# Academich/translation-transformer

Hardware: AMD Instinct MI355X
Metric: reactions/sec (SMILES decoded), greedy speculative (higher is better)
Workload: dtype f32

## Files before the change

### include/ttx.h

```cpp
#ifndef TTX_H
#define TTX_H

#include <stdint.h>

#ifdef __cplusplus
extern "C" {
#endif

#define TTX_ABI_VERSION 4

typedef enum ttx_status {
  TTX_OK = 0,
  TTX_ERR_INVALID = -1,
  TTX_ERR_HIP = -2,
  TTX_ERR_NO_DEVICE = -3,
  TTX_ERR_REFERENCE = -4,
  TTX_ERR_NOMEM = -5,
  TTX_ERR_ROW_REPLAY = -6,
  TTX_ERR_MAX_STEPS = -7
} ttx_status;

typedef struct ttx_config {
  int32_t vocab_size;
  int32_t src_vocab_size;
// ... 83 lines not shown
typedef struct ttx_gen_stats {
  int64_t model_calls;
  int64_t accepted_tokens;
  int64_t produced_tokens;
  int64_t verified_positions;
  int64_t kv_prefix_positions;
  int64_t src_positions;
  double  encode_ms, decode_ms;
  int64_t src_tokens_padded;
  int64_t status;
} ttx_gen_stats;

int ttx_greedy_speculative_generate(ttx_session* s, const int64_t* d_src, int B, int Ls,
                                    const ttx_gen_params* p, int64_t* d_out, ttx_gen_stats* stats,
                                    void* stream);

int ttx_greedy_generate(ttx_session* s, const int64_t* d_src, int B, int Ls, const ttx_gen_params* p,
                        int64_t* d_out, ttx_gen_stats* stats, void* stream);

int ttx_nucleus_mask(ttx_session* s, const float* d_logits, int rows, int V, float nucleus, int n_best, float fill,
                     float* d_out, void* stream);
int ttx_accepted_lengths(ttx_session* s, const float* d_logits, const int64_t* d_drafts, int R, int D, int V, float nucleus,
                         int n_best, int32_t* d_n_ok, void* stream);
int ttx_ragged_topk(ttx_session* s, const float* d_score, const int32_t* d_offsets, int G, int max_group, int k,
                    float* d_top, int64_t* d_idx, void* stream);
typedef struct ttx_beam_params {
  int32_t max_len;
  int32_t n_best;
  int32_t draft_len;
  int32_t n_drafts;
  int32_t smart_drafts_mode;
  int32_t pad_token, bos_token, eos_token, replace_token;
  int32_t max_steps;
} ttx_beam_params;

typedef struct ttx_beam_stats {
  int64_t model_calls;
  int64_t input_lines;
  int64_t running_rows;
  int64_t accepted_tokens;
  int64_t produced_non_pad_tokens;
  int64_t verified_positions;
  int64_t executed_positions;
  int64_t kv_prefix_positions;
  int64_t running_candidates;
  int64_t src_tokens_padded;
  double  encode_ms, decode_ms;
  int32_t out_width;
  int32_t status;
} ttx_beam_stats;

int ttx_beam_speculative_generate(ttx_session* s, const int64_t* d_src, int B, int Ls, const ttx_beam_params* p,
                                  int64_t* d_out, ttx_beam_stats* stats, void* stream);
int ttx_beam_speculative_generate_many(ttx_session** sessions, int n_sessions, int n_batches, const int64_t* const* d_src,
                                       const int* B, const int* Ls, const ttx_beam_params* p, int64_t* const* d_out,
                                       ttx_beam_stats* stats, void* stream);

int ttx_beam_speculative_generate_pool(ttx_session** sessions, int n_sessions, const int64_t* d_src, int R_total, int Ls_all,
                                       const int32_t* h_len, const int32_t* h_batch_of, int n_batches, const int32_t* h_given_ls,
                                       int capacity, const ttx_beam_params* p, int64_t* d_out, int16_t* d_trace_len,
                                       int32_t* d_summary, int trace_cap, ttx_beam_stats* stats, void* stream);

typedef struct ttx_beam_search_params {
  int32_t max_len, beam_size;
  int32_t pad_token, bos_token, eos_token;
} ttx_beam_search_params;
typedef struct ttx_beam_search_stats {
  int64_t model_calls;
  int64_t running_rows;
  int32_t out_width;
  int32_t pad_;
} ttx_beam_search_stats;
int ttx_beam_generate(ttx_session* s, const int64_t* d_src, int B, int Ls, const ttx_beam_search_params* p, int64_t* d_out,
                      ttx_beam_search_stats* stats, void* stream);

int ttx_greedy_speculative_generate_many(ttx_session** sessions, int n_sessions, int n_batches,
                                         const int64_t* const* d_src, const int* B, const int* Ls,
                                         const ttx_gen_params* p, int64_t* const* d_out, ttx_gen_stats* stats,
                                         void* stream);

int ttx_greedy_speculative_generate_rows(ttx_session** sessions, int n_sessions, int n_batches,
                                         const int64_t* const* d_src, const int* B, const int* Ls,
                                         const ttx_gen_params* p, int64_t* const* d_out, int16_t* const* d_traj,
                                         int32_t* const* d_fin_step, ttx_gen_stats* stats, void* stream);

int ttx_greedy_speculative_generate_pool(ttx_session** sessions, int n_sessions, const int64_t* d_src, int R_total, int Ls_all,
                                         const int32_t* h_len, int capacity, const ttx_gen_params* p, int64_t* d_out,
                                         int16_t* d_traj, int32_t* d_fin_step, ttx_gen_stats* stats, void* stream);

typedef struct ttx_tokenizer ttx_tokenizer;
int  ttx_tokenizer_create(const char* const* tokens, const int32_t* ids, int n, ttx_tokenizer** out);
void ttx_tokenizer_destroy(ttx_tokenizer* t);
int  ttx_tokenizer_encode(const ttx_tokenizer* t, const char* line, int32_t* out, int cap);
int  ttx_tokenizer_encode_batch(const ttx_tokenizer* t, const char* const* lines, int B, int64_t* out, int cap_cols);
int  ttx_tokenizer_decode(const ttx_tokenizer* t, const int64_t* ids, int n, char* out, int cap);

int ttx_debug_step_snapshot(ttx_session* s, int32_t* info, float* h_logits, int32_t* h_act, int32_t* h_front,
                            int32_t* h_gen);

int ttx_last_kernel_profile(ttx_session* s, double* gemm_ms, int64_t* gemm_launches, double* empty_pair_ms);

int ttx_debug_gemm_bench(ttx_session* s, int M, int N, int K, int splits, int variant, int reps, double* us_per_launch,
                         double* max_abs_diff);

int ttx_debug_gemm(ttx_session* s, const float* d_x, int ldx, const float* d_w, int ldw, const float* d_bias, float* d_y, int ldy,
                   const int32_t* d_m, int m_max, int N, int K, int relu, int splits, int64_t slab_stride, int variant, int tiling,
                   int32_t* kernel_id, void* stream);
int ttx_debug_gemm_act(ttx_session* s, const float* d_x, int ldx, const float* d_w, int ldw, const float* d_bias, float* d_y, int ldy,
                       const int32_t* d_m, int m_max, int N, int K, int activation, int splits, int64_t slab_stride, int variant,
                       int tiling, int32_t* kernel_id, void* stream);

int ttx_debug_finish_ln(ttx_session* s, const float* d_slabs, int n_slabs, int64_t slab_stride, const float* d_bias,
                        const float* d_resid, const float* d_g1, const float* d_b1, const float* d_g2, const float* d_b2,
                        const uint8_t* d_row_valid, float* d_y, const int32_t* d_m, int m_max, int d, float eps, void* stream);

int ttx_debug_attn(ttx_session* s, const float* d_q, int ldq, const float* d_k, const float* d_v, int ldkv, float* d_out, int H,
                   float scale, int L, int Lk, const int32_t* d_tok, int pad, const uint8_t* d_key_pad, const int32_t* d_mem_row,
                   const int32_t* d_act_idx, const int32_t* d_front, const int32_t* d_src_of, const int32_t* d_src_len,
                   const float* d_kcache, const float* d_vcache, int64_t cache_seq_stride, const int32_t* d_cache_slot, int gen_ld,
                   int N, int D, int mode, int groups, int n_active, int max_keys, int kernel, int32_t* kernel_id, void* stream);

int ttx_debug_attn_hd(ttx_session* s, const float* d_q, int ldq, const float* d_k, const float* d_v, int ldkv, float* d_out, int H,
                      int head_dim, float scale, int L, int Lk, const int32_t* d_tok, int pad, const uint8_t* d_key_pad,
                      const int32_t* d_mem_row, const int32_t* d_act_idx, const int32_t* d_front, const int32_t* d_src_of,
                      const int32_t* d_src_len, const float* d_kcache, const float* d_vcache, int64_t cache_seq_stride,
                      const int32_t* d_cache_slot, int gen_ld, int N, int D, int mode, int groups, int n_active, int max_keys,
                      int kernel, int32_t* kernel_id, void* stream);

int ttx_debug_attn_as(ttx_session* s, const float* d_q, int ldq, const float* d_k, const float* d_v, int ldkv, float* d_out, int H,
                      int head_dim, float scale, int L, int Lk, const int32_t* d_tok, int pad, const uint8_t* d_key_pad,
                      const int32_t* d_mem_row, const int32_t* d_act_idx, const int32_t* d_front, const int32_t* d_src_of,
                      const int32_t* d_src_len, const float* d_kcache, const float* d_vcache, int64_t cache_seq_stride,
                      const int32_t* d_cache_slot, int gen_ld, int N, int D, int mode, int groups, int n_active, int max_keys,
                      int kernel, int32_t* kernel_id, int sel_N, int sel_D, void* stream);

int ttx_debug_argmax(ttx_session* s, const float* d_logits, int V, int32_t* d_pred, const int32_t* d_m, int m_max, void* stream);

int ttx_debug_embed(ttx_session* s, const float* d_table, int V, const float* d_pe, int pe_rows, int d, float* d_x,
                    const int32_t* d_tok, int rows, int L, const int32_t* d_act_idx, const int32_t* d_front, const int32_t* d_gen,
                    int gen_ld, const int32_t* d_drafts, int B, int N, int D, int n_active, int step, void* stream);

typedef struct ttx_debug_accept_args {
  int32_t* d_act_idx; int32_t* d_front; int32_t* d_gen; const int32_t* d_drafts; const int32_t* d_pred; int32_t* d_rec;
  int64_t* d_out; int32_t* d_haspad;
  int16_t* d_traj; int32_t* d_fin_step;
  int32_t* d_rstep; int32_t* d_row_of; int64_t* d_pool_out; int16_t* d_pool_traj; int32_t* d_pool_fin_step;
  int32_t gen_ld, traj_ld, pool_rows, row_rule, pool;
  int32_t B, N, D, Ls, max_len, pad, bos, eos;
  int32_t greedy;
  int32_t threads;
} ttx_debug_accept_args;

int ttx_debug_accept(ttx_session* s, const ttx_debug_accept_args* a, int64_t* state, void* stream);

int ttx_debug_kvcopy(ttx_session* s, const int32_t* d_rec, int n_copy, const float* d_qkv, int64_t qkv_layer_stride, float* d_kcache,
                     float* d_vcache, int64_t cache_layer_stride, int64_t cache_seq_stride, int N, int D, int d, int B, int Ld,
                     void* stream);

int ttx_debug_kvcopy_split(ttx_session* s, const int32_t* d_rec, int n_copy, const float* d_qkv, int64_t qkv_layer_stride,
                           float* d_kcache, float* d_vcache, int64_t cache_layer_stride, int64_t cache_seq_stride, int N, int D, int d,
                           int B, int Ld, const int32_t* d_pos2, const float* d_qkv_probe, int64_t probe_layer_stride, void* stream);

int ttx_debug_probe_split(ttx_session* s, const int32_t* d_act_idx, const int32_t* d_pred_probe, const int32_t* d_drafts, int B, int N,
                          int D, int n_active, int32_t* d_act2, int32_t* d_pos2, int32_t* result, void* stream);

int ttx_debug_merge_pred(ttx_session* s, const int32_t* d_pos2, const int32_t* d_pred_probe, const int32_t* d_pred2, int32_t* d_pred,
                         int B, int N, int D, int n_active, void* stream);

int ttx_debug_probe_split_select(ttx_session* s, const int32_t* d_act_idx, const int32_t* d_pred_probe, const int32_t* d_drafts, int B,
                                 int N, int D, int n_active, int32_t* d_act2, int32_t* d_pos2, int32_t* d_draft_mask, int32_t* d_row_base,
                                 int32_t* d_row_map, int32_t* result, void* stream);
int ttx_debug_merge_pred_select(ttx_session* s, const int32_t* d_pos2, const int32_t* d_pred_probe, const int32_t* d_pred2,
                                int32_t* d_pred, int B, int N, int D, int n_active, const int32_t* d_row_base,
                                const int32_t* d_draft_mask, void* stream);
int ttx_debug_kvcopy_select(ttx_session* s, const int32_t* d_rec, int n_copy, const float* d_qkv, int64_t qkv_layer_stride,
                            float* d_kcache, float* d_vcache, int64_t cache_layer_stride, int64_t cache_seq_stride, int N, int D, int d,
                            int B, int Ld, const int32_t* d_pos2, const float* d_qkv_probe, int64_t probe_layer_stride,
                            const int32_t* d_row_base, const int32_t* d_draft_mask, void* stream);
int ttx_debug_embed_select(ttx_session* s, const float* d_table, int V, const float* d_pe, int pe_rows, int d, float* d_x,
                           const int32_t* d_act_idx, const int32_t* d_front, const int32_t* d_gen, int gen_ld, const int32_t* d_drafts,
                           int B, int N, int D, int n_active, const int32_t* d_row_map, int m_rows, void* stream);
int ttx_debug_attn_select(ttx_session* s, const float* d_q, int ldq, const float* d_k, const float* d_v, int ldkv, float* d_out, int H,
                          float scale, int Lk, const int32_t* d_tok, int pad, const uint8_t* d_key_pad, const int32_t* d_act_idx,
                          const int32_t* d_front, const int32_t* d_src_of, const int32_t* d_src_len, const float* d_kcache,
                          const float* d_vcache, int64_t cache_seq_stride, const int32_t* d_cache_slot, int gen_ld, int N, int D, int mode,
                          int groups, int n_active, int max_keys, int kernel, int32_t* kernel_id, const int32_t* d_row_base,
                          const int32_t* d_draft_mask, void* stream);

int ttx_pool_last_counters(ttx_session* s, int64_t* counters);

int ttx_attn_staged_key_limit(int head_dim, int q_per_group);

int ttx_debug_attn_kernels_seen(ttx_session* s);

int ttx_debug_attn_probs(ttx_session* s, const float* d_q, int ldq, const float* d_k, int ldkv, const uint8_t* d_key_pad,
                         const int32_t* d_mem_row, const int32_t* d_length, int R, int Rm, int H, int head_dim, int T, int Ls,
                         float scale, float* d_heads, float* d_mean, int32_t* d_align, void* stream);

#ifdef __cplusplus
}
#endif
#endif
```

### translation-transformer_amd/_native.py

```python
from __future__ import annotations

import ctypes as C
import os
import subprocess
from pathlib import Path

PKG_DIR = Path(__file__).resolve().parent
CSRC = PKG_DIR / "csrc"
INCLUDE = PKG_DIR.parent / "include"
LIB_PATH = PKG_DIR / "libttx_hip.so"
UNITS = [CSRC / "ttx_api.hip", CSRC / "ttx_gemm.hip", CSRC / "ttx_attn.hip"]
HEADERS = [CSRC / "ttx_internal.h", CSRC / "ttx_common.hip.h", CSRC / "ttx_loop_kernels.hip.h", CSRC / "ttx_metrics.hip.h",
           CSRC / "ttx_score.hip.h", CSRC / "ttx_alternatives.hip.h", CSRC / "ttx_attn_probs.hip.h", CSRC / "ttx_select.h",
           CSRC / "ttx_tokenizer.h", INCLUDE / "ttx.h"]
SOURCES = UNITS + HEADERS
OBJ_DIR = CSRC / "build"

TTX_OK, TTX_ERR_INVALID, TTX_ERR_HIP, TTX_ERR_NO_DEVICE, TTX_ERR_REFERENCE, TTX_ERR_NOMEM = 0, -1, -2, -3, -4, -5
TTX_ERR_ROW_REPLAY = -6
TTX_ERR_MAX_STEPS = -7
TTX_ACT_NONE, TTX_ACT_RELU, TTX_ACT_GELU = 0, 1, 2
ACTIVATIONS = {"relu": TTX_ACT_RELU, "gelu": TTX_ACT_GELU}


def activation_code(activation: str) -> int:
    if activation not in ACTIVATIONS:
        raise ValueError(f"activation must be 'relu' or 'gelu' (the exact erf GELU), got {activation!r}")
    return ACTIVATIONS[activation]


class TtxError(RuntimeError):
    def __init__(self, code: int, msg: str):
        super().__init__(f"libttx_hip error {code}: {msg}")
        self.code = code


class ReferenceError_(RuntimeError):
    """Raised where the reference implementation itself raises on the same input."""


class Config(C.Structure):
    _fields_ = [("vocab_size", C.c_int32), ("src_vocab_size", C.c_int32), ("embedding_dim", C.c_int32),
                ("num_heads", C.c_int32), ("feedforward_dim", C.c_int32), ("num_encoder_layers", C.c_int32),
                ("num_decoder_layers", C.c_int32), ("pad_token", C.c_int32), ("max_positions", C.c_int32),
                ("layer_norm_eps", C.c_float)]


class Tensor(C.Structure):
    _fields_ = [("name", C.c_char_p), ("data", C.POINTER(C.c_float)), ("numel", C.c_int64)]


class GenParams(C.Structure):
    _fields_ = [("max_len", C.c_int32), ("draft_len", C.c_int32), ("n_drafts", C.c_int32), ("pad_token", C.c_int32),
                ("bos_token", C.c_int32), ("eos_token", C.c_int32), ("replace_token", C.c_int32),
                ("want_logits", C.c_int32)]


class BeamParams(C.Structure):
    _fields_ = [("max_len", C.c_int32), ("n_best", C.c_int32), ("draft_len", C.c_int32), ("n_drafts", C.c_int32),
                ("smart_drafts_mode", C.c_int32), ("pad_token", C.c_int32), ("bos_token", C.c_int32),
                ("eos_token", C.c_int32), ("replace_token", C.c_int32), ("max_steps", C.c_int32)]


class BeamStats(C.Structure):
    _fields_ = [("model_calls", C.c_int64), ("input_lines", C.c_int64), ("running_rows", C.c_int64),
                ("accepted_tokens", C.c_int64), ("produced_non_pad_tokens", C.c_int64), ("verified_positions", C.c_int64),
                ("executed_positions", C.c_int64), ("kv_prefix_positions", C.c_int64), ("running_candidates", C.c_int64),
                ("src_tokens_padded", C.c_int64), ("encode_ms", C.c_double), ("decode_ms", C.c_double),
                ("out_width", C.c_int32), ("status", C.c_int32)]


class BeamSearchParams(C.Structure):
    _fields_ = [("max_len", C.c_int32), ("beam_size", C.c_int32), ("pad_token", C.c_int32), ("bos_token", C.c_int32),
                ("eos_token", C.c_int32)]


class BeamSearchStats(C.Structure):
    _fields_ = [("model_calls", C.c_int64), ("running_rows", C.c_int64), ("out_width", C.c_int32), ("pad_", C.c_int32)]


class GenStats(C.Structure):
    _fields_ = [("model_calls", C.c_int64), ("accepted_tokens", C.c_int64), ("produced_tokens", C.c_int64),
                ("verified_positions", C.c_int64), ("kv_prefix_positions", C.c_int64), ("src_positions", C.c_int64),
                ("encode_ms", C.c_double), ("decode_ms", C.c_double), ("src_tokens_padded", C.c_int64),
                ("status", C.c_int64)]


class DebugAcceptArgs(C.Structure):
    _fields_ = [(n, C.c_void_p) for n in ("d_act_idx", "d_front", "d_gen", "d_drafts", "d_pred", "d_rec", "d_out", "d_haspad",
                                          "d_traj", "d_fin_step", "d_rstep", "d_row_of", "d_pool_out", "d_pool_traj",
                                          "d_pool_fin_step")] + \
               [(n, C.c_int32) for n in ("gen_ld", "traj_ld", "pool_rows", "row_rule", "pool", "B", "N", "D", "Ls", "max_len",
                                         "pad", "bos", "eos", "greedy", "threads")]


DEBUG_ACCEPT_STATE_WORDS = 17


_VP, _I, _I64P = C.c_void_p, C.c_int, C.c_void_p
SYMBOLS = {
    "ttx_abi_version": (C.c_int, []),
    "ttx_last_error": (C.c_char_p, []),
    "ttx_device_count": (C.c_int, []),
    "ttx_model_create": (C.c_int, [C.POINTER(Config), C.POINTER(Tensor), _I, _I, C.POINTER(_VP)]),
    "ttx_model_destroy": (None, [_VP]),
    "ttx_model_create_empty": (C.c_int, [C.POINTER(Config), _I, C.POINTER(_VP)]),
    "ttx_model_blob": (C.c_int, [_VP, C.POINTER(_VP), C.POINTER(C.c_int64)]),
    "ttx_model_set_activation": (C.c_int, [_VP, _I]),
    "ttx_model_activation": (C.c_int, [_VP]),
    "ttx_session_create": (C.c_int, [_VP, C.POINTER(_VP)]),
    "ttx_session_destroy": (None, [_VP]),
    "ttx_encode_src": (C.c_int, [_VP, _VP, _I, _I, _VP, _VP]),
    "ttx_decode_tgt": (C.c_int, [_VP, _VP, _I, _I, _VP, _VP, _VP, _I, _I, _VP, _VP]),
    "ttx_forward": (C.c_int, [_VP, _VP, _I, _I, _VP, _I, _VP, _VP]),
    "ttx_token_metrics": (C.c_int, [_VP, _VP, _VP, _I, _I, _I, _I, _VP, _VP, _VP, _VP]),
    "ttx_teacher_forced_eval": (C.c_int, [_VP, _VP, _I, _I, _VP, _I, _I, _VP, _VP, _VP, _VP, _VP]),
    "ttx_hypothesis_logprobs": (C.c_int, [_VP, _VP, _VP, _I, _I, _I, _I, _I, _VP, _VP, _VP, _VP, _VP]),
    "ttx_score_hypotheses": (C.c_int, [_VP, _VP, _I, _I, _VP, _I, _I, _I, _I, _VP, _VP, _VP, _VP, _VP, _VP]),
    "ttx_hypothesis_alternatives": (C.c_int, [_VP, _VP, _VP, _I, _I, _I, _I, _I, _I, _VP, _VP, _VP, _VP, _VP, _VP, _VP]),
    "ttx_score_alternatives": (C.c_int, [_VP, _VP, _I, _I, _VP, _I, _I, _I, _I, _I, _VP, _VP, _VP, _VP, _VP, _VP, _VP, _VP]),
    "ttx_attention_maps": (C.c_int, [_VP, _VP, _I, _I, _VP, _I, _I, _I, _I, _I, _VP, _VP, _VP, _VP, _VP]),
    "ttx_attn_probs_key_limit": (C.c_int, [_I]),
    "ttx_debug_attn_probs": (C.c_int, [_VP, _VP, _I, _VP, _I, _VP, _VP, _VP, _I, _I, _I, _I, _I, _I, C.c_float, _VP, _VP, _VP, _VP]),
    "ttx_make_drafts": (C.c_int, [_VP, _VP, _I, _I, _I, _I, _I, _I, _I, _I, _I, _VP, _VP]),
    "ttx_greedy_speculative_generate": (C.c_int, [_VP, _VP, _I, _I, C.POINTER(GenParams), _VP, C.POINTER(GenStats), _VP]),
    "ttx_greedy_generate": (C.c_int, [_VP, _VP, _I, _I, C.POINTER(GenParams), _VP, C.POINTER(GenStats), _VP]),
    "ttx_greedy_speculative_generate_many": (C.c_int, [C.POINTER(_VP), _I, _I, C.POINTER(_VP), C.POINTER(C.c_int),
                                                      C.POINTER(C.c_int), C.POINTER(GenParams), C.POINTER(_VP),
                                                      C.POINTER(GenStats), _VP]),
    "ttx_greedy_speculative_generate_rows": (C.c_int, [C.POINTER(_VP), _I, _I, C.POINTER(_VP), C.POINTER(C.c_int),
                                                      C.POINTER(C.c_int), C.POINTER(GenParams), C.POINTER(_VP),
                                                      C.POINTER(_VP), C.POINTER(_VP), C.POINTER(GenStats), _VP]),
    "ttx_greedy_speculative_generate_pool": (C.c_int, [C.POINTER(_VP), _I, _VP, _I, _I, C.POINTER(C.c_int32), _I,
                                                      C.POINTER(GenParams), _VP, _VP, _VP, C.POINTER(GenStats), _VP]),
    "ttx_beam_speculative_generate": (C.c_int, [_VP, _VP, _I, _I, C.POINTER(BeamParams), _VP, C.POINTER(BeamStats), _VP]),
    "ttx_beam_speculative_generate_many": (C.c_int, [C.POINTER(_VP), _I, _I, C.POINTER(_VP), C.POINTER(C.c_int),
                                                    C.POINTER(C.c_int), C.POINTER(BeamParams), C.POINTER(_VP),
                                                    C.POINTER(BeamStats), _VP]),
    "ttx_beam_speculative_generate_pool": (C.c_int, [C.POINTER(_VP), _I, _VP, _I, _I, C.POINTER(C.c_int32), C.POINTER(C.c_int32), _I,
                                                    C.POINTER(C.c_int32), _I, C.POINTER(BeamParams), _VP, _VP, _VP, _I,
                                                    C.POINTER(BeamStats), _VP]),
    "ttx_beam_generate": (C.c_int, [_VP, _VP, _I, _I, C.POINTER(BeamSearchParams), _VP, C.POINTER(BeamSearchStats), _VP]),
    "ttx_nucleus_mask": (C.c_int, [_VP, _VP, _I, _I, C.c_float, _I, C.c_float, _VP, _VP]),
    "ttx_accepted_lengths": (C.c_int, [_VP, _VP, _VP, _I, _I, _I, C.c_float, _I, _VP, _VP]),
    "ttx_ragged_topk": (C.c_int, [_VP, _VP, _VP, _I, _I, _I, _VP, _VP, _VP]),
    "ttx_tokenizer_create": (C.c_int, [C.POINTER(C.c_char_p), C.POINTER(C.c_int32), _I, C.POINTER(_VP)]),
    "ttx_tokenizer_destroy": (None, [_VP]),
    "ttx_tokenizer_encode": (C.c_int, [_VP, C.c_char_p, _VP, _I]),
    "ttx_tokenizer_encode_batch": (C.c_int, [_VP, C.POINTER(C.c_char_p), _I, _VP, _I]),
    "ttx_tokenizer_decode": (C.c_int, [_VP, _VP, _I, _VP, _I]),
    "ttx_debug_step_snapshot": (C.c_int, [_VP, C.POINTER(C.c_int32), _VP, _VP, _VP, _VP]),
    "ttx_debug_gemm_bench": (C.c_int, [_VP, _I, _I, _I, _I, _I, _I, C.POINTER(C.c_double), C.POINTER(C.c_double)]),
    "ttx_debug_gemm": (C.c_int, [_VP, _VP, _I, _VP, _I, _VP, _VP, _I, _VP, _I, _I, _I, _I, _I, C.c_int64, _I, _I,
                                 C.POINTER(C.c_int32), _VP]),
    "ttx_debug_gemm_act": (C.c_int, [_VP, _VP, _I, _VP, _I, _VP, _VP, _I, _VP, _I, _I, _I, _I, _I, C.c_int64, _I, _I,
                                     C.POINTER(C.c_int32), _VP]),
    "ttx_debug_finish_ln": (C.c_int, [_VP, _VP, _I, C.c_int64, _VP, _VP, _VP, _VP, _VP, _VP, _VP, _VP, _VP, _I, _I, C.c_float, _VP]),
    "ttx_debug_attn": (C.c_int, [_VP, _VP, _I, _VP, _VP, _I, _VP, _I, C.c_float, _I, _I, _VP, _I, _VP, _VP, _VP, _VP, _VP, _VP, _VP, _VP,
                                 C.c_int64, _VP, _I, _I, _I, _I, _I, _I, _I, _I, C.POINTER(C.c_int32), _VP]),
    "ttx_debug_attn_hd": (C.c_int, [_VP, _VP, _I, _VP, _VP, _I, _VP, _I, _I, C.c_float, _I, _I, _VP, _I, _VP, _VP, _VP, _VP, _VP, _VP, _VP,
                                    _VP, C.c_int64, _VP, _I, _I, _I, _I, _I, _I, _I, _I, C.POINTER(C.c_int32), _VP]),
    "ttx_debug_attn_as": (C.c_int, [_VP, _VP, _I, _VP, _VP, _I, _VP, _I, _I, C.c_float, _I, _I, _VP, _I, _VP, _VP, _VP, _VP, _VP, _VP, _VP,
                                    _VP, C.c_int64, _VP, _I, _I, _I, _I, _I, _I, _I, _I, C.POINTER(C.c_int32), _I, _I, _VP]),
    "ttx_debug_argmax": (C.c_int, [_VP, _VP, _I, _VP, _VP, _I, _VP]),
    "ttx_debug_embed": (C.c_int, [_VP, _VP, _I, _VP, _I, _I, _VP, _VP, _I, _I, _VP, _VP, _VP, _I, _VP, _I, _I, _I, _I, _I, _VP]),
    "ttx_debug_accept": (C.c_int, [_VP, C.POINTER(DebugAcceptArgs), C.POINTER(C.c_int64), _VP]),
    "ttx_debug_kvcopy": (C.c_int, [_VP, _VP, _I, _VP, C.c_int64, _VP, _VP, C.c_int64, C.c_int64, _I, _I, _I, _I, _I, _VP]),
    "ttx_debug_kvcopy_split": (C.c_int, [_VP, _VP, _I, _VP, C.c_int64, _VP, _VP, C.c_int64, C.c_int64, _I, _I, _I, _I, _I, _VP, _VP,
                                         C.c_int64, _VP]),
    "ttx_debug_probe_split": (C.c_int, [_VP, _VP, _VP, _VP, _I, _I, _I, _I, _VP, _VP, C.POINTER(C.c_int32), _VP]),
    "ttx_debug_merge_pred": (C.c_int, [_VP, _VP, _VP, _VP, _VP, _I, _I, _I, _I, _VP]),
    "ttx_debug_probe_split_select": (C.c_int, [_VP, _VP, _VP, _VP, _I, _I, _I, _I, _VP, _VP, _VP, _VP, _VP, C.POINTER(C.c_int32), _VP]),
    "ttx_debug_merge_pred_select": (C.c_int, [_VP, _VP, _VP, _VP, _VP, _I, _I, _I, _I, _VP, _VP, _VP]),
    "ttx_debug_kvcopy_select": (C.c_int, [_VP, _VP, _I, _VP, C.c_int64, _VP, _VP, C.c_int64, C.c_int64, _I, _I, _I, _I, _I, _VP, _VP,
                                          C.c_int64, _VP, _VP, _VP]),
    "ttx_debug_embed_select": (C.c_int, [_VP, _VP, _I, _VP, _I, _I, _VP, _VP, _VP, _VP, _I, _VP, _I, _I, _I, _I, _VP, _I, _VP]),
    "ttx_debug_attn_select": (C.c_int, [_VP, _VP, _I, _VP, _VP, _I, _VP, _I, C.c_float, _I, _VP, _I, _VP, _VP, _VP, _VP, _VP, _VP, _VP,
                                        C.c_int64, _VP, _I, _I, _I, _I, _I, _I, _I, _I, C.POINTER(C.c_int32), _VP, _VP, _VP]),
    "ttx_pool_last_counters": (C.c_int, [_VP, C.POINTER(C.c_int64)]),
    "ttx_attn_staged_key_limit": (C.c_int, [_I, _I]),
    "ttx_debug_attn_kernels_seen": (C.c_int, [_VP]),
    "ttx_last_kernel_profile": (C.c_int, [_VP, C.POINTER(C.c_double), C.POINTER(C.c_int64), C.POINTER(C.c_double)]),
}

_lib = None


def hipcc_path() -> str:
    for cand in (os.environ.get("HIPCC"), "/opt/rocm/bin/hipcc", "hipcc"):
        if cand and (os.path.isabs(cand) and os.path.exists(cand) or not os.path.isabs(cand)):
            return cand
    return "hipcc"


def needs_build() -> bool:
    if not LIB_PATH.exists():
        return True
    t = LIB_PATH.stat().st_mtime
    return any(src.stat().st_mtime > t for src in SOURCES)


def build(force: bool = False, verbose: bool = False) -> Path:
    if not force and not needs_build():
        return LIB_PATH
    OBJ_DIR.mkdir(exist_ok=True)
    flags = ["--offload-arch=gfx950", "-O3", "-std=c++17", "-fPIC", f"-I{INCLUDE}"] + os.environ.get("TTX_HIPCC_FLAGS", "").split()
    newest_header = max(h.stat().st_mtime for h in HEADERS)
    jobs, objs = [], []
    for unit in UNITS:
        obj = OBJ_DIR / (unit.stem + ".o")
        objs.append(str(obj))
        if not force and obj.exists() and obj.stat().st_mtime > max(unit.stat().st_mtime, newest_header) \
                and not os.environ.get("TTX_HIPCC_FLAGS"):
            continue
        cmd = [hipcc_path(), *flags, "-c", str(unit), "-o", str(obj)]
        if verbose:
            print(" ".join(cmd))
        jobs.append((cmd, subprocess.Popen(cmd)))
    for cmd, proc in jobs:
        if proc.wait() != 0:
            raise subprocess.CalledProcessError(proc.returncode, cmd)
    cmd = [hipcc_path(), "--offload-arch=gfx950", "-shared", "-fPIC", "-o", str(LIB_PATH), *objs]
    if verbose:
        print(" ".join(cmd))
    subprocess.run(cmd, check=True)
    return LIB_PATH


def lib():
    global _lib
    if _lib is not None:
        return _lib
    if needs_build():
        build()
    handle = C.CDLL(str(LIB_PATH))
    for name, (res, args) in SYMBOLS.items():
        fn = getattr(handle, name)
        fn.restype = res
        fn.argtypes = args
    if handle.ttx_abi_version() != 4:
        raise RuntimeError("libttx_hip.so ABI version mismatch")
    _lib = handle
    return _lib


def check(code: int) -> None:
    if code == TTX_OK:
        return
    msg = lib().ttx_last_error().decode("utf-8", "replace")
    if code == TTX_ERR_REFERENCE:
        raise ReferenceError_(msg)
    if code == TTX_ERR_MAX_STEPS:
        raise RuntimeError("beam-speculative loop exceeded max_steps (non-terminating input)")
    raise TtxError(code, msg)
```

### translation-transformer_amd/csrc/ttx_api.hip

```cpp
#include "ttx_internal.h"
#include "ttx_loop_kernels.hip.h"
#include "ttx_metrics.hip.h"
#include "ttx_score.hip.h"
#include "ttx_alternatives.hip.h"
#include "ttx_attn_probs.hip.h"
#include "ttx_tokenizer.h"

#include <algorithm>
#include <chrono>
#include <cmath>
#include <cstdio>
#include <cstdlib>
#include <cstring>
#include <mutex>
#include <type_traits>

using namespace ttx;

static thread_local std::string g_err;

int ttx::fail(int code, const std::string& msg) {
  g_err = msg;
  return code;
}
// ... 131 lines not shown
  *bytes = (int64_t)(m->blob_floats * sizeof(float));
  return TTX_OK;
}

extern "C" int ttx_model_create(const ttx_config* cfg, const ttx_tensor* tensors, int n_tensors, int device,
                                ttx_model** out) {
  if (!tensors || n_tensors <= 0) return fail(TTX_ERR_INVALID, "no tensors given");
  ttx_model* m = nullptr;
  TTX_TRY(model_alloc(cfg, device, &m));
  std::vector<float> host(m->blob_floats, 0.f);
  std::map<std::string, const ttx_tensor*> given;
  for (int i = 0; i < n_tensors; ++i) {
    if (!tensors[i].name || !tensors[i].data) { ttx_model_destroy(m); return fail(TTX_ERR_INVALID, "tensor with null name/data"); }
    std::string nm = tensors[i].name;
    if (nm.rfind("model.", 0) == 0) nm = nm.substr(6);
    given[nm] = &tensors[i];
  }
  for (auto& kv : m->index) {
    const std::string& nm = kv.first;
    const bool derived = nm.rfind("derived.", 0) == 0;
    auto it = given.find(nm);
    if (it == given.end()) {
      if (derived || nm == "positional_encoding.pe") continue;
      ttx_model_destroy(m);
      return fail(TTX_ERR_INVALID, "missing tensor: " + nm);
    }
    if ((size_t)it->second->numel != kv.second.second) {
      ttx_model_destroy(m);
      return fail(TTX_ERR_INVALID, "tensor " + nm + " has " + std::to_string(it->second->numel) + " elements, expected " +
                                       std::to_string(kv.second.second));
    }
    std::memcpy(host.data() + kv.second.first, it->second->data, kv.second.second * sizeof(float));
  }
  const ttx_config& c = m->cfg;
  const size_t d = c.embedding_dim;
  if (given.find("positional_encoding.pe") == given.end()) {
    float* pe = host.data() + m->pe;
    const float cst = (float)(-std::log(10000.0) / (double)d);
    for (int p = 0; p < c.max_positions; ++p)
      for (size_t i = 0; i < d; i += 2) {
        const float div = expf((float)i * cst);
        const float arg = (float)p * div;
        pe[(size_t)(p + 1) * d + i] = sinf(arg);
        pe[(size_t)(p + 1) * d + i + 1] = cosf(arg);
      }
  }
  for (int l = 0; l < c.num_decoder_layers; ++l) {
    std::memcpy(host.data() + m->cross_kv_w + (size_t)l * 2 * d * d, host.data() + m->dec[l].ca_in_w + d * d, 2 * d * d * sizeof(float));
    std::memcpy(host.data() + m->cross_kv_b + (size_t)l * 2 * d, host.data() + m->dec[l].ca_in_b + d, 2 * d * sizeof(float));
  }
  if (hipMemcpy(m->blob, host.data(), host.size() * sizeof(float), hipMemcpyHostToDevice) != hipSuccess) {
    ttx_model_destroy(m);
    return fail(TTX_ERR_HIP, "hipMemcpy of the weight blob failed");
  }
  *out = m;
  return TTX_OK;
}

extern "C" void ttx_model_destroy(ttx_model* m) {
  if (!m) return;
  if (m->blob) (void)hipFree(m->blob);
  delete m;
}

static std::mutex g_retired_mu;
static std::vector<void*> g_retired;

static void release_retired() {
  std::vector<void*> v;
  {
    std::lock_guard<std::mutex> lk(g_retired_mu);
    v.swap(g_retired);
  }
  if (v.empty()) return;
  (void)hipDeviceSynchronize();
  for (void* p : v) (void)hipFree(p);
}

static std::mutex g_stream_mu;
static std::map<int, std::vector<std::pair<int, hipStream_t>>> g_free_streams;
static std::map<hipStream_t, int> g_stream_index;
static int g_streams_made = 0;

static int ensure_own_stream(ttx_session* s) {
  if (s->own_stream) return TTX_OK;
  std::lock_guard<std::mutex> lock(g_stream_mu);
  auto& idle = g_free_streams[s->m->device];
  if (!idle.empty()) {
    auto it = std::min_element(idle.begin(), idle.end());
    s->own_stream = it->second;
    idle.erase(it);
    return TTX_OK;
  }
  HIP_TRY(hipStreamCreateWithFlags(&s->own_stream, hipStreamNonBlocking));
  g_stream_index[s->own_stream] = g_streams_made++;
  return TTX_OK;
}

static void release_own_stream(ttx_session* s) {
  if (!s->own_stream) return;
  std::lock_guard<std::mutex> lock(g_stream_mu);
  g_free_streams[s->m->device].push_back({g_stream_index[s->own_stream], s->own_stream});
  s->own_stream = nullptr;
}

static int ensure(Buf& b, size_t bytes, hipStream_t st) {
  (void)st;
  if (bytes <= b.cap) return TTX_OK;
  if (b.owner_gen) ++*b.owner_gen;
  if (b.p) {
    std::lock_guard<std::mutex> lk(g_retired_mu);
    g_retired.push_back(b.p);
    b.p = nullptr;
    b.cap = 0;
  }
  size_t want = bytes + bytes / 8 + 256;
  if (hipMalloc(&b.p, want) != hipSuccess) return fail(TTX_ERR_NOMEM, "hipMalloc failed for " + std::to_string(want) + " bytes");
  b.cap = want;
  static const bool poison = getenv("TTX_POISON_WORKSPACES") != nullptr && atoi(getenv("TTX_POISON_WORKSPACES")) != 0;
  if (poison) {
    if (hipMemset(b.p, 0xFF, want) != hipSuccess) return fail(TTX_ERR_HIP, "hipMemset (poison) failed");
    (void)hipDeviceSynchronize();
  }
  return TTX_OK;
}

extern "C" int ttx_session_create(ttx_model* m, ttx_session** out) {
  if (!m || !out) return fail(TTX_ERR_INVALID, "null argument");
  HIP_TRY(hipSetDevice(m->device));
  ttx_session* s = new ttx_session();
  s->m = m;
  if (hipHostMalloc((void**)&s->host_info, sizeof(HostInfo), hipHostMallocMapped) != hipSuccess ||
      hipHostMalloc((void**)&s->probe_info, sizeof(ProbeInfo), hipHostMallocMapped) != hipSuccess ||
      hipHostMalloc((void**)&s->host_state, sizeof(DecState), hipHostMallocDefault) != hipSuccess) {
    if (s->host_info) (void)hipHostFree(s->host_info);
    if (s->probe_info) (void)hipHostFree(s->probe_info);
    if (s->host_state) (void)hipHostFree(s->host_state);
    delete s;
    return fail(TTX_ERR_NOMEM, "hipHostMalloc failed");
  }
  std::memset(s->host_info, 0, sizeof(HostInfo));
  std::memset(s->probe_info, 0, sizeof(ProbeInfo));
  HIP_TRY(hipEventCreate(&s->ev_a));
  HIP_TRY(hipEventCreate(&s->ev_b));
  HIP_TRY(hipEventCreate(&s->ev_c));
  HIP_TRY(hipEventCreateWithFlags(&s->ev_done, hipEventDisableTiming));
  s->use_graphs = getenv("TTX_NO_GRAPH") == nullptr;
  const char* pf = getenv("TTX_PROFILE_GEMM");
  s->profile = pf && pf[0] == '1';
  if (const char* e = getenv("TTX_SMALL_ROWS")) s->small_rows = std::max(0, atoi(e));
  if (const char* e = getenv("TTX_FFN2_SLAB_ROWS")) s->ffn2_slab_rows = std::max(0, atoi(e));
  if (const char* e = getenv("TTX_QKV_SMALL_ROWS")) s->qkv_small_rows = std::max(0, atoi(e));
  if (const char* e = getenv("TTX_ATTN_FALLBACK")) s->attn_fallback = atoi(e) != 0;
  if (const char* e = getenv("TTX_ATTN_ROW")) s->attn_row = atoi(e) != 0 ? 1 : 0;
  s->host_timing = getenv("TTX_HOST_TIMING") != nullptr;
  m->n_sessions++;
  *out = s;
  return TTX_OK;
}

extern "C" void ttx_session_destroy(ttx_session* s) {
  if (!s) return;
  if (s->host_timing && s->host_launches)
    fprintf(stderr, "[ttx host timing] hipGraphLaunch: %lld launches, %.1f us each\n", s->host_launches,
            s->host_launch_us / (double)s->host_launches);
  if (s->host_timing && s->host_captures)
    fprintf(stderr, "[ttx host timing] graphs captured: %lld, %.1f us each\n", s->host_captures,
            s->host_capture_us / (double)s->host_captures);
  if (s->dead) {
    delete s;
    return;
  }
  release_retired();
  (void)hipDeviceSynchronize();
  for (Buf* b : s->all)
    if (b->p) (void)hipFree(b->p);
  if (s->host_info) (void)hipHostFree(s->host_info);
  if (s->probe_info) (void)hipHostFree(s->probe_info);
  if (s->beam_host) (void)hipHostFree(s->beam_host);
  if (s->bp_host) (void)hipHostFree(s->bp_host);
  s->drop_graphs();
  release_own_stream(s);
  if (s->ev_done) (void)hipEventDestroy(s->ev_done);
  if (s->host_state) (void)hipHostFree(s->host_state);
  for (auto& e : s->ev_pool) { (void)hipEventDestroy(e.first); (void)hipEventDestroy(e.second); }
  if (s->ev_a) (void)hipEventDestroy(s->ev_a);
  if (s->ev_b) (void)hipEventDestroy(s->ev_b);
  if (s->ev_c) (void)hipEventDestroy(s->ev_c);
  delete s;
}

static int variant_for_rows(const ttx_session* s, long long rows, bool step) {
  if (!step) return GV_BIG;
  if (rows < s->qkv_small_rows) return GV_SMALL;
  if (rows < s->small_rows) return GV_MID;
  return rows < s->ffn2_slab_rows ? GV_BIG_FFN2_SLABS : GV_BIG;
}
static int variant_qkv(int v) { return v == GV_SMALL ? GV_SMALL : GV_BIG; }
static int variant_dd(int v) { return (v == GV_SMALL || v == GV_MID) ? GV_SMALL : GV_BIG; }
static int variant_ffn1(int v) { return v == GV_SMALL ? GV_SMALL : GV_BIG; }
static int variant_ffn2(int v) { return v == GV_BIG ? GV_BIG : GV_SMALL; }

static int gemm_ln(ttx_session* s, hipStream_t st, const float* X, int ldx, int K, const float* W, const float* bias,
                   const float* resid, const float* g1, const float* b1, const float* g2, const float* b2,
                   const uint8_t* row_valid, float* Y, const int* m_ptr, int Mmax, int variant) {
  const int d = s->m->cfg.embedding_dim;
  const int S = gemm_splits(d, K, m_ptr != nullptr, variant);
  const long long stride = (long long)Mmax * d;
  TTX_TRY(ensure(s->slab, sizeof(float) * (size_t)S * stride, st));
  TTX_TRY(launch_gemm(s, st, X, ldx, W, K, nullptr, s->slab.as<float>(), d, m_ptr, Mmax, d, K, false, S, stride, variant));
  return launch_finish(s, st, s->slab.as<float>(), S, stride, bias, resid, g1, b1, g2, b2, row_valid, Y, m_ptr, Mmax);
}

static int ffn_half(ttx_session* s, hipStream_t st, const LayerW& w, const float* x, size_t n_w, size_t n_b, const float* g2,
                    const float* b2, const uint8_t* row_valid, float* Y, const int* m_ptr, int Mmax, int v_ffn1, int v_ffn2) {
  const ttx_model* m = s->m;
  const int d = m->cfg.embedding_dim, F = m->cfg.feedforward_dim;
  float* hb = s->hbuf.as<float>();
  TTX_TRY(launch_gemm(s, st, x, d, m->p(w.l1_w), d, m->p(w.l1_b), hb, F, m_ptr, Mmax, F, d, m->activation, 0, 0, v_ffn1));
  return gemm_ln(s, st, hb, F, F, m->p(w.l2_w), m->p(w.l2_b), x, m->p(n_w), m->p(n_b), g2, b2, row_valid, Y, m_ptr, Mmax, v_ffn2);
}

static int ensure_acts(ttx_session* s, hipStream_t st, size_t M, int qkv_layers) {
  const ttx_config& c = s->m->cfg;
  const size_t d = c.embedding_dim, F = c.feedforward_dim;
  TTX_TRY(ensure(s->x, M * d * 4, st));
  TTX_TRY(ensure(s->x1, M * d * 4, st));
  TTX_TRY(ensure(s->x2, M * d * 4, st));
  TTX_TRY(ensure(s->xf, M * d * 4, st));
  TTX_TRY(ensure(s->ao, M * d * 4, st));
  TTX_TRY(ensure(s->q2, M * d * 4, st));
  TTX_TRY(ensure(s->hbuf, M * F * 4, st));
  TTX_TRY(ensure(s->qkv, (size_t)qkv_layers * M * 3 * d * 4, st));
  return TTX_OK;
}

static int run_encoder(ttx_session* s, hipStream_t st, const int* tok, const uint8_t* valid, int B, int Ls, float* memory,
                       float* qkv_buf = nullptr) {
  const ttx_model* m = s->m;
  const ttx_config& c = m->cfg;
  const int d = c.embedding_dim, H = c.num_heads;
  const int M = B * Ls;
  const int gv = variant_for_rows(s, M, false);
  TTX_TRY(ensure_acts(s, st, (size_t)M, 1));
  float* x = s->x.as<float>();
  float* x1 = s->x1.as<float>();
  float* qkv = qkv_buf ? qkv_buf : s->qkv.as<float>();
  float* ao = s->ao.as<float>();
  EmbedArgs e{};
  e.table = m->p(m->src_emb); e.pe = m->p(m->pe); e.X = x; e.d = d; e.V = c.src_vocab_size; e.tok = tok; e.rows = M; e.L = Ls;
  hipLaunchKernelGGL((k_embed<false>), dim3(cdiv(M, 4)), dim3(256), 0, st, e);
  HIP_TRY(hipGetLastError());
  for (int l = 0; l < c.num_encoder_layers; ++l) {
    const LayerW& w = m->enc[l];
    const bool last = (l == c.num_encoder_layers - 1);
    TTX_TRY(launch_gemm(s, st, x, d, m->p(w.sa_in_w), d, m->p(w.sa_in_b), qkv, 3 * d, nullptr, M, 3 * d, d, false, 0, 0, gv));
    AttnArgs a{};
    a.q = qkv; a.ldq = 3 * d; a.k = qkv + d; a.v = qkv + 2 * d; a.ldkv = 3 * d; a.out = ao; a.d = d;
    a.scale = 1.0f / sqrtf((float)(d / H)); a.L = Ls; a.tok = tok; a.pad = c.pad_token;
    TTX_TRY(launch_attn(ATT_ENC, s, st, a, B, H, Ls, Ls));
    TTX_TRY(gemm_ln(s, st, ao, d, d, m->p(w.sa_out_w), m->p(w.sa_out_b), x, m->p(w.n1_w), m->p(w.n1_b), nullptr, nullptr,
                    nullptr, x1, nullptr, M, gv));
    TTX_TRY(ffn_half(s, st, w, x1, w.n2_w, w.n2_b, last ? m->p(m->enc_norm_w) : nullptr, last ? m->p(m->enc_norm_b) : nullptr,
                     last ? valid : nullptr, last ? memory : x, nullptr, M, gv, gv));
  }
  return TTX_OK;
}

static int prepare_tokens(hipStream_t st, const int64_t* d_in, int* out, uint8_t* valid, int n, int pad) {
  hipLaunchKernelGGL(k_prepare_tokens, dim3(cdiv(n, 256)), dim3(256), 0, st, d_in, out, valid, n, pad);
  HIP_TRY(hipGetLastError());
  return TTX_OK;
}

extern "C" int ttx_encode_src(ttx_session* s, const int64_t* d_src, int B, int Ls, float* d_memory, void* stream) {
  if (!s || !d_src || !d_memory || B <= 0 || Ls <= 0) return fail(TTX_ERR_INVALID, "bad argument to ttx_encode_src");
  if (Ls > s->m->cfg.max_positions) return fail(TTX_ERR_INVALID, "source longer than the positional table");
  hipStream_t st = (hipStream_t)stream;
  HIP_TRY(hipSetDevice(s->m->device));
  TTX_TRY(ensure(s->tok_src, (size_t)B * Ls * 4, st));
  TTX_TRY(ensure(s->src_valid, (size_t)B * Ls, st));
  TTX_TRY(prepare_tokens(st, d_src, s->tok_src.as<int>(), s->src_valid.as<uint8_t>(), B * Ls, s->m->cfg.pad_token));
  return run_encoder(s, st, s->tok_src.as<int>(), s->src_valid.as<uint8_t>(), B, Ls, d_memory);
}

struct StackRows {
  const int* m_ptr;
  int Mmax;
  int v_qkv, v_dd, v_ffn1, v_ffn2;
  float* qkv;
  long long qkv_layer;
};

template <class SelfAttn, class CrossAttn>
static int run_decoder_stack(ttx_session* s, hipStream_t st, const StackRows& r, SelfAttn&& self_attn, CrossAttn&& cross_attn,
                             float* logits, int stop_layer = -1) {
  const ttx_model* m = s->m;
  const ttx_config& c = m->cfg;
  const int d = c.embedding_dim, V = c.vocab_size, Ld = c.num_decoder_layers;
  float* x = s->x.as<float>();
  float* x1 = s->x1.as<float>();
  float* x2 = s->x2.as<float>();
  float* xf = s->xf.as<float>();
  float* ao = s->ao.as<float>();
  float* q2 = s->q2.as<float>();
  for (int l = 0; l < Ld; ++l) {
// ... 385 lines not shown
                                  void* stream) {
  if (!s) return session_required("ttx_attention_maps");
  if (!d_src || !d_hyp || B <= 0 || N <= 0 || Ls <= 0) return fail(TTX_ERR_INVALID, "bad argument to ttx_attention_maps");
  if (!d_heads && !d_mean && !d_align) return fail(TTX_ERR_INVALID, "ttx_attention_maps: no output requested (heads, mean and alignment are all null)");
  if (ld_hyp < W) return fail(TTX_ERR_INVALID, "ttx_attention_maps: row stride ld_hyp smaller than W");
  const ttx_config& c = s->m->cfg;
  if (layer == -1) layer = c.num_decoder_layers - 1;
  if (layer < 0 || layer >= c.num_decoder_layers)
    return fail(TTX_ERR_INVALID, "ttx_attention_maps: layer must be -1 or in [0, " + std::to_string(c.num_decoder_layers) + ")");
  TTX_TRY(check_score_shapes(s, (long long)B * N, W, 1, "ttx_attention_maps"));
  if (Ls > c.max_positions) return fail(TTX_ERR_INVALID, "source longer than the positional table");
  const int limit = attn_probs_key_limit(c.embedding_dim / c.num_heads);
  if (Ls > limit)
    return fail(TTX_ERR_INVALID, "ttx_attention_maps: source longer than " + std::to_string(limit) + " keys (ttx_attn_probs_key_limit)");
  hipStream_t st = (hipStream_t)stream;
  HIP_TRY(hipSetDevice(s->m->device));
  const int R = B * N, T = W - 1, d = c.embedding_dim;
  if (!d_length) {
    TTX_TRY(ensure(s->am_length, (size_t)R * 4, st));
    d_length = s->am_length.as<int32_t>();
  }
  TTX_TRY(ensure(s->memory, (size_t)B * Ls * d * 4, st));
  TTX_TRY(ensure(s->mem_pad_tmp, (size_t)B * Ls, st));
  TTX_TRY(ensure(s->sc_src_of, (size_t)R * 4, st));
  TTX_TRY(ttx_encode_src(s, d_src, B, Ls, s->memory.as<float>(), stream));
  hipLaunchKernelGGL(k_invert_mask, dim3(cdiv(B * Ls, 256)), dim3(256), 0, st, s->src_valid.as<uint8_t>(),
                     s->mem_pad_tmp.as<uint8_t>(), B * Ls);
  HIP_TRY(hipGetLastError());
  hipLaunchKernelGGL(k_score_src_of, dim3(cdiv(R, 256)), dim3(256), 0, st, s->sc_src_of.as<int>(), R, N);
  HIP_TRY(hipGetLastError());
  TTX_TRY(ensure(s->tok_tgt, (size_t)R * T * 4, st));
  hipLaunchKernelGGL(k_prepare_tokens_2d, dim3(cdiv(R * T, 256)), dim3(256), 0, st, d_hyp, ld_hyp, s->tok_tgt.as<int>(),
                     (uint8_t*)nullptr, R, T, c.pad_token);
  HIP_TRY(hipGetLastError());
  hipLaunchKernelGGL(k_hyp_length, dim3(cdiv(R, 4)), dim3(256), 0, st, d_hyp, ld_hyp, R, W, c.pad_token, eos, d_length);
  HIP_TRY(hipGetLastError());
  const AttnTap tap{layer, d_length, d_heads, d_mean, d_align};
  return run_decoder_full(s, st, s->tok_tgt.as<int>(), R, T, s->memory.as<float>(), s->mem_pad_tmp.as<uint8_t>(),
                          s->sc_src_of.as<int>(), B, Ls, nullptr, &tap);
}

static int clamp_draft_len(int draft_len, int lo, int hi) { return std::min(std::max(lo, draft_len), hi); }

template <typename OutT>
static int launch_make_drafts(hipStream_t st, const int* src32, int src_ld, int off, int B, int L, int N, int D, int eos,
                              int pad, int repl, OutT* out) {
  const int need = N + D - 1;
  const int Lp = L > need ? L : need;
  const size_t lds = sizeof(int) * (size_t)(Lp + 1);
  if (lds > 60 * 1024) return fail(TTX_ERR_INVALID, "make_drafts: padded source row too long");
  hipLaunchKernelGGL((k_make_drafts<OutT>), dim3(B), dim3(64), lds, st, src32, src_ld, off, L, N, D, eos, pad, repl, out);
  HIP_TRY(hipGetLastError());
  return TTX_OK;
}

extern "C" int ttx_make_drafts(ttx_session* s, const int64_t* d_src, int B, int L, int draft_len, int n_drafts,
                               int min_draft_len, int max_draft_len, int eos_token, int pad_token, int replace_token,
                               int64_t* d_drafts, void* stream) {
  if (!s || !d_src || !d_drafts || B <= 0 || L <= 0) return fail(TTX_ERR_INVALID, "bad argument to ttx_make_drafts");
  if (n_drafts <= 0) return fail(TTX_ERR_REFERENCE, "The number of drafts must be greater than 0");
  if (min_draft_len > max_draft_len) return fail(TTX_ERR_REFERENCE, "The minimum draft length must not be greater than the maximum draft length");
  if (pad_token == replace_token || eos_token == replace_token || eos_token == pad_token)
    return fail(TTX_ERR_REFERENCE, "pad, eos and replace tokens must be pairwise different");
  hipStream_t st = (hipStream_t)stream;
  HIP_TRY(hipSetDevice(s->m->device));
  const int D = clamp_draft_len(draft_len, min_draft_len, max_draft_len);
  if (D <= 0) return fail(TTX_ERR_INVALID, "draft length must be positive");
  TTX_TRY(ensure(s->src32, (size_t)B * L * 4, st));
  TTX_TRY(prepare_tokens(st, d_src, s->src32.as<int>(), nullptr, B * L, pad_token));
  return launch_make_drafts<int64_t>(st, s->src32.as<int>(), L, 0, B, L, n_drafts, D, eos_token, pad_token, replace_token, d_drafts);
}

struct StepCtx {
  int B, Ls, N, D, Lc, gen_ld, max_len;
  ttx_gen_params p;
  const float* kcache = nullptr;
  const float* vcache = nullptr;
  const int* src_of = nullptr;
  const int* src_len = nullptr;
  const int* cache_slot = nullptr;
  bool want_argmax = true;
  int variant = GV_BIG;
  DecState* st_ov = nullptr;
  const int* act_ov = nullptr;
  float* qkv_ov = nullptr;
  int* pred_ov = nullptr;
  int sel_N = 0, sel_D = 0;
  const int* row_base = nullptr; const int* draft_mask = nullptr; const int* row_map = nullptr;
};

static int run_step(ttx_session* s, hipStream_t st, const StepCtx& k, int kcap) {
  const ttx_model* m = s->m;
  const ttx_config& c = m->cfg;
  const int d = c.embedding_dim, H = c.num_heads, V = c.vocab_size, Ld = c.num_decoder_layers;
  const int D1 = k.D + 1;
  const int RPS = step_rps(k.N, k.D);
  const int Mmax = k.B * RPS;
  DecState* dst = k.st_ov ? k.st_ov : s->state.as<DecState>();
  const int* act = k.act_ov ? k.act_ov : s->act_idx.as<int>();
  const int* m_ptr = &dst->m_rows;
  float* ao = s->ao.as<float>();
  float* logits = s->logits.as<float>();
  const float scale = 1.0f / sqrtf((float)(d / H));
  const long long cache_seq = (long long)k.Lc * d;
  const long long cache_layer = (long long)k.B * cache_seq;

  struct AttnSel {
    ttx_session* s;
    AttnSel(ttx_session* s_, int N, int D) : s(s_) { s->attn_sel_N = N; s->attn_sel_D = D; }
    ~AttnSel() { s->attn_sel_N = 0; s->attn_sel_D = 0; }
  } attn_sel(s, k.sel_N, k.sel_D);
  EmbedArgs e{};
  e.table = m->p(m->tgt_emb); e.pe = m->p(m->pe); e.X = s->x.as<float>(); e.d = d; e.V = c.vocab_size;
  e.st = dst; e.act_idx = act; e.front = s->front.as<int>(); e.gen = s->gen.as<int>(); e.gen_ld = k.gen_ld;
  e.drafts = s->drafts.as<int>(); e.N = k.N; e.D = k.D; e.row_map = k.row_map;
  hipLaunchKernelGGL((k_embed<true>), dim3(cdiv(Mmax, 4)), dim3(256), 0, st, e);
  HIP_TRY(hipGetLastError());

  const StackRows rows{m_ptr, Mmax, variant_qkv(k.variant), variant_dd(k.variant), variant_ffn1(k.variant), variant_ffn2(k.variant),
                       k.qkv_ov ? k.qkv_ov : s->qkv.as<float>(), (long long)Mmax * 3 * d};
  TTX_TRY(run_decoder_stack(s, st, rows,
      [&](int l, float* qkv) -> int {
        AttnArgs a{};
        a.q = qkv; a.ldq = 3 * d; a.k = qkv + d; a.v = qkv + 2 * d; a.ldkv = 3 * d; a.out = ao; a.d = d; a.scale = scale;
        a.tok = s->gen.as<int>(); a.pad = c.pad_token; a.st = dst; a.act_idx = act; a.front = s->front.as<int>();
        a.kcache = (k.kcache ? k.kcache : s->kcache.as<float>()) + (size_t)l * cache_layer;
        a.vcache = (k.vcache ? k.vcache : s->vcache.as<float>()) + (size_t)l * cache_layer;
        a.cache_seq_stride = cache_seq; a.gen_ld = k.gen_ld; a.N = k.N; a.D = k.D; a.cache_slot = k.cache_slot;
        a.row_base = k.row_base; a.draft_mask = k.draft_mask;
        return launch_attn(ATT_STEP_SELF, s, st, a, k.B, H, RPS, kcap, k.N, D1);
      },
      [&](int l) -> int {
        AttnArgs ca{};
        ca.q = s->q2.as<float>(); ca.ldq = d; ca.k = s->memkv.as<float>() + (size_t)l * 2 * d; ca.v = ca.k + d; ca.ldkv = Ld * 2 * d;
        ca.out = ao; ca.d = d; ca.scale = scale; ca.Lk = k.Ls; ca.key_pad = s->src_valid.as<uint8_t>();
        ca.st = dst; ca.act_idx = act; ca.front = s->front.as<int>(); ca.N = k.N; ca.D = k.D;
        ca.src_of = k.src_of; ca.src_len = k.src_len; ca.row_base = k.row_base; ca.draft_mask = k.draft_mask;
        return launch_attn(ATT_STEP_CROSS, s, st, ca, k.B, H, RPS, k.Ls, k.N, D1);
      },
      logits));
  if (k.want_argmax) {
    hipLaunchKernelGGL(k_argmax, dim3(cdiv(Mmax, 4)), dim3(256), 0, st, logits, V, k.pred_ov ? k.pred_ov : s->pred.as<int>(), m_ptr, Mmax);
    HIP_TRY(hipGetLastError());
  }
  return TTX_OK;
}

struct GenCtx {
  StepCtx k;
  LoopArgs la;
  KvCopyArgs kc;
};

static int launch_accept_and_commit(ttx_session* s, hipStream_t st, const GenCtx& g, bool greedy) {
  if (greedy) hipLaunchKernelGGL(k_greedy_accept, dim3(1), dim3(256), 0, st, g.la);
  else hipLaunchKernelGGL(k_accept, dim3(1), dim3(g.k.B > 256 ? ACCEPT_THREADS : 256), 0, st, g.la);
  HIP_TRY(hipGetLastError());
  hipLaunchKernelGGL(k_kvcopy, dim3(g.k.B, s->m->cfg.num_decoder_layers), dim3(256), 0, st, g.kc);
  HIP_TRY(hipGetLastError());
  return TTX_OK;
}

static bool watchdog_expired(std::chrono::steady_clock::time_point since) {
  static const int limit_s = [] { const char* e = getenv("TTX_WATCHDOG_SECONDS"); return e && atoi(e) > 0 ? atoi(e) : 120; }();
  return std::chrono::steady_clock::now() - since > std::chrono::seconds(limit_s);
}

static int session_hung(ttx_session* s) {
  s->dead = true;
  return fail(TTX_ERR_HIP, "verify step did not publish its result within the watchdog time; the session is unusable "
                           "(its stream was NOT synchronised) - exit the process or continue in a fresh child process");
}

static int session_alive(const ttx_session* s) {
  if (s && s->dead) return fail(TTX_ERR_HIP, "this session hung in an earlier call and is unusable");
  return TTX_OK;
}

struct Progress {
  unsigned idle_spins = 0;
  std::chrono::steady_clock::time_point last_progress = std::chrono::steady_clock::now();
  bool stalled() { return (++idle_spins & 0xffff) == 0 && watchdog_expired(last_progress); }
  void advanced() { idle_spins = 0; last_progress = std::chrono::steady_clock::now(); }
};

static int key_capacity(int width, int max_len) { return std::min(max_len, ((width + 63) / 64) * 64); }

template <class Enqueue>
static int graph_replay(ttx_session* s, hipStream_t st, GraphCache& cache, const GraphKey& key, Enqueue&& enqueue) {
  if (!s->use_graphs || s->profile) return enqueue();
  const auto now = [s] { return s->host_timing ? std::chrono::steady_clock::now() : std::chrono::steady_clock::time_point(); };
  const auto us_since = [&](std::chrono::steady_clock::time_point t0) { return std::chrono::duration<double, std::micro>(now() - t0).count(); };
  s->graphs_current();
  auto it = cache.map.find(key);
  if (it == cache.map.end()) {
    if (cache.warmed.insert(key).second) return enqueue();
    hipGraph_t graph = nullptr;
    hipGraphExec_t exec = nullptr;
    const auto t0 = now();
    HIP_TRY(hipStreamBeginCapture(st, hipStreamCaptureModeThreadLocal));
    const int rc = enqueue();
    hipError_t e = hipStreamEndCapture(st, &graph);
    if (rc != TTX_OK) { if (graph) (void)hipGraphDestroy(graph); return rc; }
    if (e != hipSuccess) return fail(TTX_ERR_HIP, std::string("hipStreamEndCapture: ") + hipGetErrorString(e));
    e = hipGraphInstantiate(&exec, graph, nullptr, nullptr, 0);
    (void)hipGraphDestroy(graph);
    if (e != hipSuccess) return fail(TTX_ERR_HIP, std::string("hipGraphInstantiate: ") + hipGetErrorString(e));
    if (cache.map.size() > cache.limit) s->drop_graphs();
    it = cache.map.emplace(key, exec).first;
    if (s->host_timing) { s->host_captures += 1; s->host_capture_us += us_since(t0); }
  }
  const auto t0 = now();
  HIP_TRY(hipGraphLaunch(it->second, st));
  if (s->host_timing) { s->host_launches += 1; s->host_launch_us += us_since(t0); }
  return TTX_OK;
}

struct EventGuard {
  hipEvent_t e = nullptr;
  ~EventGuard() { if (e) (void)hipEventDestroy(e); }
};

struct GenJob {
  ttx_session* s = nullptr;
  hipStream_t st = nullptr;
  GenCtx g{};
  bool greedy = false;
  int64_t* d_out = nullptr;
  int16_t* d_traj = nullptr;
  int32_t* d_fin = nullptr;
  ttx_gen_stats* stats = nullptr;
  int launched = 0;
  int phase = 0;
  int batch = -1;
  Progress progress;
};

static int gen_validate(const ttx_session* s, const int64_t* d_src, int B, int Ls, const ttx_gen_params* p, const int64_t* d_out,
                        bool greedy) {
  if (!s || !d_src || !p || !d_out || B <= 0 || Ls <= 1) return fail(TTX_ERR_INVALID, "bad argument to a generate call");
  const ttx_config& c = s->m->cfg;
  if (!greedy) {
    if (p->n_drafts <= 0) return fail(TTX_ERR_REFERENCE, "The number of drafts must be greater than 0");
    if (p->max_len < 1) return fail(TTX_ERR_REFERENCE, "The minimum draft length must not be greater than the maximum draft length");
    if (p->pad_token == p->replace_token || p->eos_token == p->replace_token || p->eos_token == p->pad_token)
      return fail(TTX_ERR_REFERENCE, "pad, eos and replace tokens must be pairwise different");
    if (p->draft_len <= 0) return fail(TTX_ERR_REFERENCE, "Number of speculative tokens must be a positive integer.");
    if (p->draft_len > p->max_len) return fail(TTX_ERR_REFERENCE, "draft_len beyond max_len: the reference's scatter shapes disagree");
  } else if (p->max_len < 1) {
    return fail(TTX_ERR_INVALID, "max_len must be positive");
  }
  if (p->pad_token != c.pad_token) return fail(TTX_ERR_INVALID, "generator pad token differs from the model's");
  const int D = greedy ? 0 : p->draft_len;
  if (p->max_len + D + 2 > c.max_positions) return fail(TTX_ERR_INVALID, "max_len + draft_len exceeds the positional table");
  return TTX_OK;
}

static int gen_start(GenJob& j, ttx_session* s, hipStream_t st, const int64_t* d_src, int B, int Ls, const ttx_gen_params* p,
                     int64_t* d_out, ttx_gen_stats* stats, bool greedy, int16_t* d_traj = nullptr, int32_t* d_fin = nullptr) {
  const ttx_model* m = s->m;
  const ttx_config& c = m->cfg;
  const int d = c.embedding_dim, Ld = c.num_decoder_layers, V = c.vocab_size;
  const int N = greedy ? 1 : p->n_drafts, D = greedy ? 0 : p->draft_len, D1 = D + 1;
  const int max_len = p->max_len;
  j.s = s; j.st = st; j.greedy = greedy; j.d_out = d_out; j.stats = stats; j.launched = 0;
  j.d_traj = d_traj; j.d_fin = d_fin;
  const bool row_rule = d_traj != nullptr;
  s->snap_step = 0;
  GenCtx& g = j.g;
  g = GenCtx{};
  g.k.B = B; g.k.Ls = Ls; g.k.N = N; g.k.D = D; g.k.max_len = max_len; g.k.p = *p;
  g.k.Lc = max_len + D1;
  g.k.gen_ld = max_len + D + 2;
  const size_t Mmax = (size_t)B * step_rps(N, D);

  TTX_TRY(ensure(s->tok_src, (size_t)B * Ls * 4, st));
  TTX_TRY(ensure(s->src_valid, (size_t)B * Ls, st));
  TTX_TRY(ensure(s->memory, (size_t)B * Ls * d * 4, st));
  TTX_TRY(ensure(s->memkv, (size_t)B * Ls * Ld * 2 * d * 4, st));
  TTX_TRY(ensure(s->drafts, (size_t)B * N * std::max(D, 1) * 4, st));
  TTX_TRY(ensure(s->gen, (size_t)B * g.k.gen_ld * 4, st));
  TTX_TRY(ensure(s->front, (size_t)B * 4, st));
  TTX_TRY(ensure(s->act_idx, (size_t)B * 4, st));
  TTX_TRY(ensure(s->haspad, (size_t)B * 4, st));
  if (row_rule) {
    TTX_TRY(ensure(s->traj, (size_t)B * (max_len + 1) * 2, st));
    TTX_TRY(ensure(s->fin_step, (size_t)B * 4, st));
  }
  TTX_TRY(ensure(s->rec, (size_t)B * sizeof(CopyRec), st));
  TTX_TRY(ensure(s->pred, Mmax * 4, st));
  TTX_TRY(ensure(s->state, sizeof(DecState), st));
  TTX_TRY(ensure(s->logits, Mmax * V * 4, st));
  TTX_TRY(ensure(s->outbuf, (size_t)B * max_len * 8, st));
  TTX_TRY(ensure(s->kcache, (size_t)Ld * B * g.k.Lc * d * 4, st));
  TTX_TRY(ensure(s->vcache, (size_t)Ld * B * g.k.Lc * d * 4, st));
  const size_t Macts = std::max(Mmax, (size_t)B * Ls);
  TTX_TRY(ensure_acts(s, st, Macts, 1));
  TTX_TRY(ensure(s->qkv, std::max((size_t)Ld * Mmax, (size_t)B * Ls) * 3 * d * 4, st));
  TTX_TRY(ensure(s->slab, sizeof(float) * 16 * Macts * d, st));
  s->graphs_current();

  s->ev_used = 0;
  HIP_TRY(hipEventRecord(s->ev_a, st));
  TTX_TRY(prepare_tokens(st, d_src, s->tok_src.as<int>(), s->src_valid.as<uint8_t>(), B * Ls, c.pad_token));
  TTX_TRY(run_encoder(s, st, s->tok_src.as<int>(), s->src_valid.as<uint8_t>(), B, Ls, s->memory.as<float>()));
  const int gv = variant_for_rows(s, (long long)B * Ls, false);
  TTX_TRY(launch_gemm(s, st, s->memory.as<float>(), d, m->p(m->cross_kv_w), d, m->p(m->cross_kv_b), s->memkv.as<float>(),
                      Ld * 2 * d, nullptr, B * Ls, Ld * 2 * d, d, false, 0, 0, gv));
  if (!greedy)
    TTX_TRY(launch_make_drafts<int>(st, s->tok_src.as<int>(), Ls, 1, B, Ls - 1, N, D, p->eos_token, p->pad_token,
                                    p->replace_token, s->drafts.as<int>()));

  g.la.st = s->state.as<DecState>(); g.la.act_idx = s->act_idx.as<int>(); g.la.front = s->front.as<int>();
  g.la.gen = s->gen.as<int>(); g.la.gen_ld = g.k.gen_ld; g.la.drafts = s->drafts.as<int>(); g.la.pred = s->pred.as<int>();
  g.la.rec = s->rec.as<CopyRec>(); g.la.out = s->outbuf.as<int64_t>(); g.la.haspad = s->haspad.as<int>();
  HostInfo* dev_info = nullptr;
  HIP_TRY(hipHostGetDevicePointer((void**)&dev_info, (void*)s->host_info, 0));
  g.la.host = dev_info;
  g.la.B = B; g.la.N = N; g.la.D = D; g.la.Ls = Ls; g.la.max_len = max_len; g.la.pad = p->pad_token; g.la.bos = p->bos_token;
  g.la.eos = p->eos_token;
  g.la.row_rule = row_rule ? 1 : 0; g.la.traj = row_rule ? s->traj.as<short>() : nullptr; g.la.traj_ld = max_len + 1;
  g.la.fin_step = row_rule ? s->fin_step.as<int>() : nullptr;
  g.kc.st = s->state.as<DecState>(); g.kc.rec = s->rec.as<CopyRec>(); g.kc.qkv = s->qkv.as<float>();
  g.kc.qkv_layer_stride = (long long)Mmax * 3 * d;
  g.kc.kcache = s->kcache.as<float>(); g.kc.vcache = s->vcache.as<float>();
  g.kc.cache_seq_stride = (long long)g.k.Lc * d; g.kc.cache_layer_stride = (long long)B * g.k.Lc * d;
  g.kc.N = N; g.kc.D = D; g.kc.d = d;

  s->host_info->stop = 0;
  s->host_info->steps_done = 0;
  s->host_info->width = 1;
  s->host_info->n_active = B;
  hipLaunchKernelGGL(k_loop_init, dim3(64), dim3(256), 0, st, g.la);
  HIP_TRY(hipGetLastError());
  HIP_TRY(hipEventRecord(s->ev_b, st));
  j.phase = 1;
  return TTX_OK;
}

static int gen_launch_step(GenJob& j, int width_bound) {
  ttx_session* s = j.s;
  StepCtx k = j.g.k;
  const int live = j.greedy ? k.B : std::max(1, (int)((volatile HostInfo*)s->host_info)->n_active);
  k.variant = variant_for_rows(s, (long long)live * step_rps(k.N, k.D), true);
  const int kcap = key_capacity(std::max(width_bound, 1), k.max_len);
  const auto enqueue = [&]() -> int {
    TTX_TRY(run_step(s, j.st, k, kcap));
    return launch_accept_and_commit(s, j.st, j.g, j.greedy);
  };
  if (k.p.want_logits > 0 && k.p.want_logits == j.launched + 1) {
    TTX_TRY(run_step(s, j.st, k, kcap));
    const ttx_config& c = s->m->cfg;
    const size_t Mmax = (size_t)k.B * step_rps(k.N, k.D);
    TTX_TRY(ensure(s->snap_logits, Mmax * c.vocab_size * 4, j.st));
    TTX_TRY(ensure(s->snap_act, (size_t)k.B * 4, j.st));
    TTX_TRY(ensure(s->snap_front, (size_t)k.B * 4, j.st));
    TTX_TRY(ensure(s->snap_gen, (size_t)k.B * k.gen_ld * 4, j.st));
    TTX_TRY(ensure(s->snap_state, sizeof(DecState), j.st));
    HIP_TRY(hipMemcpyAsync(s->snap_logits.p, s->logits.p, Mmax * c.vocab_size * 4, hipMemcpyDeviceToDevice, j.st));
    HIP_TRY(hipMemcpyAsync(s->snap_act.p, s->act_idx.p, (size_t)k.B * 4, hipMemcpyDeviceToDevice, j.st));
    HIP_TRY(hipMemcpyAsync(s->snap_front.p, s->front.p, (size_t)k.B * 4, hipMemcpyDeviceToDevice, j.st));
    HIP_TRY(hipMemcpyAsync(s->snap_gen.p, s->gen.p, (size_t)k.B * k.gen_ld * 4, hipMemcpyDeviceToDevice, j.st));
    HIP_TRY(hipMemcpyAsync(s->snap_state.p, s->state.p, sizeof(DecState), hipMemcpyDeviceToDevice, j.st));
    s->snap_B = k.B; s->snap_rps = step_rps(k.N, k.D); s->snap_gen_ld = k.gen_ld; s->snap_step = j.launched + 1;
    TTX_TRY(launch_accept_and_commit(s, j.st, j.g, j.greedy));
  } else {
    const int site = j.greedy ? GS_STEP_GREEDY : (j.g.la.row_rule ? GS_STEP_ROW_RULE : GS_STEP_SPECULATIVE);
    TTX_TRY(graph_replay(s, j.st, s->step_graphs, GraphKey{site, k.B, k.Ls, k.N, k.D, k.max_len, kcap, k.variant, 0}, enqueue));
  }
  ++j.launched;
  return TTX_OK;
}

static int gen_finish_enqueue(GenJob& j) {
  ttx_session* s = j.s;
  const StepCtx& k = j.g.k;
  if (j.greedy) {
    hipLaunchKernelGGL(k_gen_to_out, dim3(cdiv(k.B * k.max_len, 256)), dim3(256), 0, j.st, s->gen.as<int>(), k.gen_ld, j.d_out,
                       k.B, k.max_len);
    HIP_TRY(hipGetLastError());
  } else {
    HIP_TRY(hipMemcpyAsync(j.d_out, s->outbuf.as<int64_t>(), (size_t)k.B * k.max_len * 8, hipMemcpyDeviceToDevice, j.st));
    if (j.d_traj) {
      HIP_TRY(hipMemcpyAsync(j.d_traj, s->traj.p, (size_t)k.B * (k.max_len + 1) * 2, hipMemcpyDeviceToDevice, j.st));
      HIP_TRY(hipMemcpyAsync(j.d_fin, s->fin_step.p, (size_t)k.B * 4, hipMemcpyDeviceToDevice, j.st));
    }
  }
  HIP_TRY(hipEventRecord(s->ev_c, j.st));
  HIP_TRY(hipMemcpyAsync(s->host_state, s->state.as<DecState>(), sizeof(DecState), hipMemcpyDeviceToHost, j.st));
  HIP_TRY(hipEventRecord(s->ev_done, j.st));
  j.phase = 2;
  return TTX_OK;
}

static void collect_gemm_profile(ttx_session* s, hipStream_t st) {
  if (!s->profile) return;
  s->prof_launches += (long long)s->ev_used;
  for (size_t i = 0; i < s->ev_used; ++i) {
    float ms = 0.f;
    if (hipEventElapsedTime(&ms, s->ev_pool[i].first, s->ev_pool[i].second) == hipSuccess) s->prof_ms += ms;
  }
  s->ev_used = 0;
  if (s->prof_empty_pair_ms < 0 && s->ev_pool.size() >= 32) {
    unsigned long long* d_ticks = nullptr;
    if (hipMalloc(&d_ticks, 32 * sizeof(unsigned long long)) == hipSuccess) {
      for (int i = 0; i < 32; ++i) {
        (void)hipEventRecord(s->ev_pool[i].first, st);
        hipLaunchKernelGGL(k_spin, dim3(1), dim3(64), 0, st, d_ticks + i, 2000);
        (void)hipEventRecord(s->ev_pool[i].second, st);
      }
      (void)hipStreamSynchronize(st);
      unsigned long long h_ticks[32];
      std::vector<double> over;
      if (hipMemcpy(h_ticks, d_ticks, sizeof(h_ticks), hipMemcpyDeviceToHost) == hipSuccess)
        for (int i = 0; i < 32; ++i) {
          float ms = 0.f;
          if (hipEventElapsedTime(&ms, s->ev_pool[i].first, s->ev_pool[i].second) == hipSuccess)
            over.push_back((double)ms - (double)h_ticks[i] * 1e-5);
        }
      (void)hipFree(d_ticks);
      if (!over.empty()) {
        std::sort(over.begin(), over.end());
        s->prof_empty_pair_ms = std::max(0.0, over[over.size() / 2]);
      }
    }
  }
}

static int gen_finish_collect(GenJob& j) {
  ttx_session* s = j.s;
  const DecState& hs = *s->host_state;
  if (j.stats) {
    j.stats->model_calls = hs.steps;
    j.stats->accepted_tokens = hs.accepted;
    j.stats->produced_tokens = hs.produced;
    j.stats->verified_positions = hs.verified_positions;
    j.stats->kv_prefix_positions = hs.kv_prefix_positions;
    j.stats->src_positions = hs.src_positions;
    j.stats->src_tokens_padded = (long long)j.g.k.B * j.g.k.Ls;
    float ms = 0.f;
    HIP_TRY(hipEventElapsedTime(&ms, s->ev_a, s->ev_b));
    j.stats->encode_ms = ms;
    HIP_TRY(hipEventElapsedTime(&ms, s->ev_b, s->ev_c));
    j.stats->decode_ms = ms;
  }
  collect_gemm_profile(s, j.st);
  j.phase = 0;
  if (j.stats) j.stats->status = hs.error == 3 ? TTX_ERR_ROW_REPLAY : (hs.error ? TTX_ERR_REFERENCE : TTX_OK);
  if (hs.error == 3)
    return fail(TTX_ERR_ROW_REPLAY, "a row emitted PAD inside its sequence: what the reference does next depends on the other rows "
                                    "of its batch, so the batch must be decoded as given (ttx_greedy_speculative_generate_many)");
  if (hs.error == 2)
    return fail(TTX_ERR_REFERENCE, "the model emitted PAD inside a sequence and a whole column became PAD: the reference's draft "
                                   "scatter raises 'index out of range' here (speculative_decoding.py:97,111-115)");
  if (hs.error) return fail(TTX_ERR_REFERENCE, "a row finished at a width beyond max_len: shape mismatch in the reference (speculative_decoding.py:158)");
  return TTX_OK;
}

static int generate_common(ttx_session* s, const int64_t* d_src, int B, int Ls, const ttx_gen_params* p, int64_t* d_out,
                           ttx_gen_stats* stats, void* stream, bool greedy) {
  TTX_TRY(gen_validate(s, d_src, B, Ls, p, d_out, greedy));
  TTX_TRY(session_alive(s));
  HIP_TRY(hipSetDevice(s->m->device));
  release_retired();
  TTX_TRY(ensure_own_stream(s));
  HIP_TRY(hipEventRecord(s->ev_done, (hipStream_t)stream));
  HIP_TRY(hipStreamWaitEvent(s->own_stream, s->ev_done, 0));
  hipStream_t st = s->own_stream;
  GenJob j;
  TTX_TRY(gen_start(j, s, st, d_src, B, Ls, p, d_out, stats, greedy));
  const int D1 = j.g.k.D + 1;
  volatile HostInfo* hi = s->host_info;
  HIP_TRY(hipStreamSynchronize(st));
  while (!hi->stop) {
    if (j.launched > p->max_len + 2) return fail(TTX_ERR_HIP, "decode loop failed to terminate");
    TTX_TRY(gen_launch_step(j, hi->width + D1));
    const int want = j.launched;
    Progress wait;
    while (hi->steps_done < want && !hi->stop) {
      if (wait.stalled()) return session_hung(s);
      __builtin_ia32_pause();
    }
  }
  TTX_TRY(gen_finish_enqueue(j));
  HIP_TRY(hipStreamSynchronize(st));
  return gen_finish_collect(j);
}

extern "C" int ttx_greedy_speculative_generate(ttx_session* s, const int64_t* d_src, int B, int Ls,
                                               const ttx_gen_params* p, int64_t* d_out, ttx_gen_stats* stats,
                                               void* stream) {
  return generate_common(s, d_src, B, Ls, p, d_out, stats, stream, false);
}

extern "C" int ttx_greedy_generate(ttx_session* s, const int64_t* d_src, int B, int Ls, const ttx_gen_params* p,
                                   int64_t* d_out, ttx_gen_stats* stats, void* stream) {
  return generate_common(s, d_src, B, Ls, p, d_out, stats, stream, true);
}

struct PoolJob {
  ttx_session* s = nullptr;
  hipStream_t st = nullptr;
  GenCtx g{};
  int C = 0, Ls_cap = 0;
  int launched = 0;
  int phase = 0;
  int admits = 0;
  int quota_end = -1;
  PoolIo io{};
  Progress progress;
  long long admitted_rows = 0, src_tokens_padded = 0;
  bool two_phase = true;
  long long min_rows = 800;
  GenCtx g2{};
  ProbeInfo* dev_probe = nullptr;
  int probes = 0;
  bool probe_pending = false;
  long long slot_steps = 0, matched_slot_steps = 0, split_steps = 0, skipped_draft_passes = 0;
  bool draft_select = false;
  long long drafts_matched = 0;
  long long rows_executed = 0;
  long long unsplit_rows = 0;
};

static int pool_start(PoolJob& j, ttx_session* s, hipStream_t st, int C, int Ls_cap, const ttx_gen_params* p, int64_t* d_out,
                      int16_t* d_traj, int32_t* d_fin) {
  const ttx_model* m = s->m;
  const ttx_config& c = m->cfg;
  const int d = c.embedding_dim, Ld = c.num_decoder_layers, V = c.vocab_size;
  const int N = p->n_drafts, D = p->draft_len, D1 = D + 1, max_len = p->max_len;
  j.s = s; j.st = st; j.C = C; j.Ls_cap = Ls_cap; j.launched = 0; j.admits = 0; j.admitted_rows = 0; j.src_tokens_padded = 0;
  s->snap_step = 0;
  GenCtx& g = j.g;
  g = GenCtx{};
  g.k.B = C; g.k.Ls = Ls_cap; g.k.N = N; g.k.D = D; g.k.max_len = max_len; g.k.p = *p;
  g.k.Lc = max_len + D1;
  g.k.gen_ld = max_len + D + 2;
  const size_t Mmax = (size_t)C * step_rps(N, D);
  const size_t kv_row = (size_t)Ld * 2 * d;
  TTX_TRY(ensure(s->tok_src, (size_t)C * Ls_cap * 4, st));
  TTX_TRY(ensure(s->valid_new, (size_t)C * Ls_cap, st));
  TTX_TRY(ensure(s->src_valid, (size_t)C * Ls_cap, st));
  TTX_TRY(ensure(s->memory, (size_t)C * Ls_cap * d * 4, st));
  TTX_TRY(ensure(s->memkv_new, (size_t)C * Ls_cap * kv_row * 4, st));
  TTX_TRY(ensure(s->memkv, (size_t)C * Ls_cap * kv_row * 4, st));
  TTX_TRY(ensure(s->drafts, (size_t)C * N * D * 4, st));
  TTX_TRY(ensure(s->drafts_new, (size_t)C * N * D * 4, st));
  TTX_TRY(ensure(s->gen, (size_t)C * g.k.gen_ld * 4, st));
  for (Buf* b : {&s->front, &s->act_idx, &s->haspad, &s->rstep, &s->row_of, &s->src_len, &s->new_slot}) TTX_TRY(ensure(*b, (size_t)C * 4, st));
  TTX_TRY(ensure(s->rec, (size_t)C * sizeof(CopyRec), st));
  TTX_TRY(ensure(s->pred, Mmax * 4, st));
  TTX_TRY(ensure(s->state, sizeof(DecState), st));
  TTX_TRY(ensure(s->pool_io, sizeof(PoolIo), st));
  TTX_TRY(ensure(s->logits, Mmax * V * 4, st));
  TTX_TRY(ensure(s->kcache, (size_t)Ld * C * g.k.Lc * d * 4, st));
  TTX_TRY(ensure(s->vcache, (size_t)Ld * C * g.k.Lc * d * 4, st));
  const size_t Macts = std::max(Mmax, (size_t)C * Ls_cap);
  TTX_TRY(ensure_acts(s, st, Macts, 1));
  TTX_TRY(ensure(s->qkv, std::max((size_t)Ld * Mmax, (size_t)C * Ls_cap) * 3 * d * 4, st));
  TTX_TRY(ensure(s->slab, sizeof(float) * 16 * Macts * d, st));
  j.two_phase = true; j.min_rows = 800; j.probes = 0; j.probe_pending = false;
  j.slot_steps = j.matched_slot_steps = j.split_steps = j.skipped_draft_passes = 0;
  j.drafts_matched = j.rows_executed = j.unsplit_rows = 0;
  if (const char* e = getenv("TTX_TWO_PHASE")) j.two_phase = atoi(e) != 0;
  if (const char* e = getenv("TTX_TWO_PHASE_MIN_ROWS")) j.min_rows = std::max(0, atoi(e));
  j.draft_select = j.two_phase && d == c.num_heads * ATT_DH && c.num_heads % 4 == 0 && !s->attn_fallback && N <= 32 && D >= 1;
  if (const char* e = getenv("TTX_DRAFT_SELECT")) j.draft_select = j.draft_select && atoi(e) != 0;
  if (j.draft_select) {
    for (Buf* b : {&s->draft_mask, &s->row_base}) TTX_TRY(ensure(*b, (size_t)C * 4, st));
    TTX_TRY(ensure(s->row_map, Mmax * 4, st));
  }
  if (j.two_phase) {
    TTX_TRY(ensure(s->qkv_probe, (size_t)Ld * C * 3 * d * 4, st));
    for (Buf* b : {&s->pred_probe, &s->act2, &s->pos2}) TTX_TRY(ensure(*b, (size_t)C * 4, st));
    TTX_TRY(ensure(s->pred_draft, Mmax * 4, st));
    TTX_TRY(ensure(s->state2, 3 * sizeof(DecState), st));
  }
  s->graphs_current();

  s->ev_used = 0;
  HIP_TRY(hipEventRecord(s->ev_a, st));
  if (j.two_phase) {
    HIP_TRY(hipMemsetAsync(s->state2.p, 0, 3 * sizeof(DecState), st));
    s->probe_info->matches = 0; s->probe_info->probes_done = 0; s->probe_info->rows = 0;
    HIP_TRY(hipHostGetDevicePointer((void**)&j.dev_probe, (void*)s->probe_info, 0));
  }
  j.io = PoolIo{d_out, d_traj, d_fin, max_len + 1, 0};
  HIP_TRY(hipMemcpyAsync(s->pool_io.p, &j.io, sizeof(j.io), hipMemcpyHostToDevice, st));
  g.la.st = s->state.as<DecState>(); g.la.act_idx = s->act_idx.as<int>(); g.la.front = s->front.as<int>();
  g.la.gen = s->gen.as<int>(); g.la.gen_ld = g.k.gen_ld; g.la.drafts = s->drafts.as<int>(); g.la.pred = s->pred.as<int>();
  g.la.rec = s->rec.as<CopyRec>(); g.la.out = nullptr; g.la.haspad = s->haspad.as<int>();
  HostInfo* dev_info = nullptr;
  HIP_TRY(hipHostGetDevicePointer((void**)&dev_info, (void*)s->host_info, 0));
  g.la.host = dev_info;
  g.la.B = C; g.la.N = N; g.la.D = D; g.la.Ls = Ls_cap; g.la.max_len = max_len; g.la.pad = p->pad_token; g.la.bos = p->bos_token;
  g.la.eos = p->eos_token;
  g.la.row_rule = 1; g.la.traj = nullptr; g.la.traj_ld = max_len + 1; g.la.fin_step = nullptr;
  g.la.pool = 1; g.la.rstep = s->rstep.as<int>(); g.la.row_of = s->row_of.as<int>(); g.la.io = s->pool_io.as<PoolIo>();
  g.k.src_len = s->src_len.as<int>();
  g.kc.st = s->state.as<DecState>(); g.kc.rec = s->rec.as<CopyRec>(); g.kc.qkv = s->qkv.as<float>();
  g.kc.qkv_layer_stride = (long long)Mmax * 3 * d;
  g.kc.kcache = s->kcache.as<float>(); g.kc.vcache = s->vcache.as<float>();
  g.kc.cache_seq_stride = (long long)g.k.Lc * d; g.kc.cache_layer_stride = (long long)C * g.k.Lc * d;
  g.kc.N = N; g.kc.D = D; g.kc.d = d;
  j.g2 = g;
  if (j.two_phase) {
    j.g2.la.exec_rows = reinterpret_cast<const int*>(s->state2.as<DecState>() + 2);
    j.g2.kc.pos2 = s->pos2.as<int>(); j.g2.kc.qkv_probe = s->qkv_probe.as<float>(); j.g2.kc.probe_layer_stride = (long long)C * 3 * d;
    if (j.draft_select) { j.g2.kc.row_base = s->row_base.as<int>(); j.g2.kc.draft_mask = s->draft_mask.as<int>(); }
  }
  s->host_info->stop = 0; s->host_info->steps_done = 0; s->host_info->width = 1; s->host_info->n_active = 0;
  hipLaunchKernelGGL(k_pool_init, dim3(4), dim3(256), 0, st, g.la);
  HIP_TRY(hipGetLastError());
  j.phase = 1;
  return TTX_OK;
}

static int pool_admit(PoolJob& j, const int64_t* d_src_rows, int ld_src, int R, int Ls_new, int first_row, int64_t* d_out,
                      int16_t* d_traj, int32_t* d_fin) {
  ttx_session* s = j.s;
  hipStream_t st = j.st;
  const ttx_model* m = s->m;
  const ttx_config& c = m->cfg;
  const StepCtx& k = j.g.k;
  const int d = c.embedding_dim, Ld = c.num_decoder_layers;
  const int kv_row = Ld * 2 * d;
  hipLaunchKernelGGL(k_prepare_tokens_2d, dim3(cdiv(R * Ls_new, 256)), dim3(256), 0, st, d_src_rows, ld_src, s->tok_src.as<int>(),
                     s->valid_new.as<uint8_t>(), R, Ls_new, c.pad_token);
  HIP_TRY(hipGetLastError());
  TTX_TRY(run_encoder(s, st, s->tok_src.as<int>(), s->valid_new.as<uint8_t>(), R, Ls_new, s->memory.as<float>()));
  const int gv = variant_for_rows(s, (long long)R * Ls_new, false);
  TTX_TRY(launch_gemm(s, st, s->memory.as<float>(), d, m->p(m->cross_kv_w), d, m->p(m->cross_kv_b), s->memkv_new.as<float>(),
                      kv_row, nullptr, R * Ls_new, kv_row, d, false, 0, 0, gv));
  TTX_TRY(launch_make_drafts<int>(st, s->tok_src.as<int>(), Ls_new, 1, R, Ls_new - 1, k.N, k.D, k.p.eos_token, k.p.pad_token,
                                  k.p.replace_token, s->drafts_new.as<int>()));
  PoolAdmitArgs a{};
  a.st = s->state.as<DecState>(); a.act_idx = s->act_idx.as<int>(); a.front = s->front.as<int>(); a.haspad = s->haspad.as<int>();
  a.rstep = s->rstep.as<int>(); a.row_of = s->row_of.as<int>(); a.src_len = s->src_len.as<int>(); a.new_slot = s->new_slot.as<int>();
  a.host = j.g.la.host; a.B = j.C; a.N = k.N; a.D = k.D; a.R = R; a.first_row = first_row; a.Ls_new = Ls_new;
  hipLaunchKernelGGL(k_pool_admit, dim3(1), dim3(256), (size_t)j.C * 4, st, a);
  HIP_TRY(hipGetLastError());
  PoolFillArgs f{};
  f.new_slot = s->new_slot.as<int>(); f.R = R; f.gen = s->gen.as<int>(); f.gen_ld = k.gen_ld; f.bos = k.p.bos_token; f.pad = k.p.pad_token;
  f.drafts = s->drafts.as<int>(); f.drafts_new = s->drafts_new.as<int>(); f.nd = k.N * k.D;
  f.src_valid = s->src_valid.as<uint8_t>(); f.valid_new = s->valid_new.as<uint8_t>(); f.Ls_cap = j.Ls_cap; f.Ls_new = Ls_new;
  f.memkv = s->memkv.as<float>(); f.memkv_new = s->memkv_new.as<float>(); f.kv_row = kv_row;
  f.out_rows = d_out; f.traj_rows = d_traj; f.fin_rows = d_fin; f.max_len = k.max_len; f.traj_ld = k.max_len + 1; f.first_row = first_row;
  hipLaunchKernelGGL(k_pool_fill, dim3(R, 1 + Ls_new), dim3(256), 0, st, f);
  HIP_TRY(hipGetLastError());
  ++j.admits;
  j.admitted_rows += R;
  j.src_tokens_padded += (long long)R * Ls_new;
  return TTX_OK;
}

static GraphKey pool_key(const StepCtx& k, int variant, int phase) {
  return GraphKey{GS_STEP_POOL, k.B, k.Ls, k.N, k.D, k.max_len, k.max_len, variant, phase};
}

static int pool_launch_step(PoolJob& j, int n_live) {
  ttx_session* s = j.s;
  StepCtx k = j.g.k;
  const int kcap = k.max_len;
  const long long rows = (long long)n_live * step_rps(k.N, k.D);
  if (!j.two_phase || rows < j.min_rows) {
    k.variant = variant_for_rows(s, rows, true);
    TTX_TRY(graph_replay(s, j.st, s->step_graphs, pool_key(k, k.variant, 0), [&]() -> int {
      TTX_TRY(run_step(s, j.st, k, kcap));
      return launch_accept_and_commit(s, j.st, j.g, false);
    }));
    ++j.launched;
    j.rows_executed += rows; j.unsplit_rows += rows;
    return TTX_OK;
  }
  DecState* st2 = s->state2.as<DecState>();
  StepCtx kp = k;
  kp.N = 1; kp.D = 0; kp.sel_N = k.N; kp.sel_D = k.D;
  kp.st_ov = st2; kp.qkv_ov = s->qkv_probe.as<float>(); kp.pred_ov = s->pred_probe.as<int>();
  kp.variant = variant_for_rows(s, n_live, true);
  TTX_TRY(graph_replay(s, j.st, s->step_graphs, pool_key(k, kp.variant, j.draft_select ? 4 : 1), [&]() -> int {
    hipLaunchKernelGGL(k_probe_begin, dim3(1), dim3(64), 0, j.st, s->state.as<DecState>(), st2);
    HIP_TRY(hipGetLastError());
    TTX_TRY(run_step(s, j.st, kp, kcap));
    ProbeSplitArgs ps{};
    ps.st = s->state.as<DecState>(); ps.act_idx = s->act_idx.as<int>(); ps.pred_probe = s->pred_probe.as<int>();
    ps.drafts = s->drafts.as<int>(); ps.N = k.N; ps.D = k.D; ps.act2 = s->act2.as<int>(); ps.pos2 = s->pos2.as<int>();
    ps.st2 = st2 + 1; ps.exec_rows = reinterpret_cast<int*>(st2 + 2);
    ps.host = j.dev_probe;
    if (j.draft_select) { ps.draft_mask = s->draft_mask.as<int>(); ps.row_base = s->row_base.as<int>(); ps.row_map = s->row_map.as<int>(); }
    hipLaunchKernelGGL(k_probe_split, dim3(1), dim3(k.B > 256 ? ACCEPT_THREADS : 256), 0, j.st, ps);
    HIP_TRY(hipGetLastError());
    return TTX_OK;
  }));
  ++j.probes;
  j.probe_pending = true;
  j.split_steps += 1; j.slot_steps += n_live; j.rows_executed += n_live;
  return TTX_OK;
}

static int pool_launch_drafts(PoolJob& j) {
  ttx_session* s = j.s;
  StepCtx k = j.g.k;
  const int kcap = k.max_len;
  const int matches = ((volatile ProbeInfo*)s->probe_info)->matches;
  if (matches < 0 || matches > k.B) return fail(TTX_ERR_HIP, "slot pool: the probe published a match count outside the pool");
  const int RPS = step_rps(k.N, k.D);
  const long long rows = j.draft_select ? ((volatile ProbeInfo*)s->probe_info)->rows : (long long)matches * RPS;
  if (rows < (long long)matches * (matches ? 1 + k.D : 0) || rows > (long long)matches * RPS)
    return fail(TTX_ERR_HIP, "slot pool: the probe published a row count outside its matches' rows");
  DecState* st2 = s->state2.as<DecState>();
  k.st_ov = st2 + 1; k.act_ov = s->act2.as<int>(); k.pred_ov = s->pred_draft.as<int>();
  if (j.draft_select) { k.row_base = s->row_base.as<int>(); k.draft_mask = s->draft_mask.as<int>(); k.row_map = s->row_map.as<int>(); }
  k.variant = matches ? variant_for_rows(s, rows, true) : 0;
  j.matched_slot_steps += matches; j.skipped_draft_passes += matches ? 0 : 1;
  j.rows_executed += rows; j.drafts_matched += (rows - matches) / k.D;
  const int phase = j.draft_select ? (matches ? 5 : 6) : (matches ? 2 : 3);
  TTX_TRY(graph_replay(s, j.st, s->step_graphs, pool_key(k, k.variant, phase), [&]() -> int {
    if (matches) TTX_TRY(run_step(s, j.st, k, kcap));
    MergePredArgs mp{};
    mp.st = s->state.as<DecState>(); mp.pos2 = s->pos2.as<int>(); mp.pred_probe = s->pred_probe.as<int>();
    mp.pred2 = s->pred_draft.as<int>(); mp.pred = s->pred.as<int>(); mp.RPS = RPS;
    mp.row_base = k.row_base; mp.draft_mask = k.draft_mask; mp.D = k.D;
    hipLaunchKernelGGL(k_merge_pred, dim3(cdiv(k.B * RPS, 256)), dim3(256), 0, j.st, mp);
    HIP_TRY(hipGetLastError());
    return launch_accept_and_commit(s, j.st, j.g2, false);
  }));
  j.probe_pending = false;
  ++j.launched;
  return TTX_OK;
}

extern "C" int ttx_greedy_speculative_generate_pool(ttx_session** sessions, int n_sessions, const int64_t* d_src, int R_total,
                                                    int Ls_all, const int32_t* h_len, int capacity, const ttx_gen_params* p,
                                                    int64_t* d_out, int16_t* d_traj, int32_t* d_fin_step, ttx_gen_stats* stats,
                                                    void* stream) {
  if (!sessions || n_sessions <= 0 || !d_src || R_total < 0 || !h_len || capacity <= 0 || capacity > 4096 || !p || !d_out || !d_traj ||
      !d_fin_step)
    return fail(TTX_ERR_INVALID, "bad argument to ttx_greedy_speculative_generate_pool");
  if (R_total == 0) return TTX_OK;
  if (p->max_len > 32000) return fail(TTX_ERR_INVALID, "max_len too large for the int16 trace");
  int len_max = 0;
  for (int i = 0; i < R_total; ++i) len_max = std::max(len_max, (int)h_len[i]);
  if (len_max > Ls_all) return fail(TTX_ERR_INVALID, "row length beyond the source matrix width");
  int Ls_cap = std::min(std::max(192, ((len_max + 63) / 64) * 64), sessions[0]->m->cfg.max_positions);
  Ls_cap = std::max(Ls_cap, std::max(2, len_max));
  TTX_TRY(gen_validate(sessions[0], d_src, capacity, Ls_cap, p, d_out, false));
  HIP_TRY(hipSetDevice(sessions[0]->m->device));
  release_retired();
  for (int i = 0; i < n_sessions; ++i) TTX_TRY(session_alive(sessions[i]));
  EventGuard ready_guard;
  HIP_TRY(hipEventCreateWithFlags(&ready_guard.e, hipEventDisableTiming));
  hipEvent_t ready = ready_guard.e;
  HIP_TRY(hipEventRecord(ready, (hipStream_t)stream));
  bool hung = false;
  const int n_jobs = std::min(n_sessions, cdiv(R_total, std::max(1, std::min(capacity / 2, 32))));
  const int C = std::min(capacity, std::max(1, cdiv(R_total, n_jobs)));
  std::vector<PoolJob> jobs(n_jobs);
  int rc_final = TTX_OK;
  std::fill(std::begin(sessions[0]->pool_counters), std::end(sessions[0]->pool_counters), 0LL);
  for (int i = 0; i < n_jobs && rc_final == TTX_OK; ++i) {
    ttx_session* s = sessions[i];
    TTX_TRY(ensure_own_stream(s));
    HIP_TRY(hipStreamWaitEvent(s->own_stream, ready, 0));
    rc_final = pool_start(jobs[i], s, s->own_stream, C, Ls_cap, p, d_out, d_traj, d_fin_step);
  }
  sessions[0]->pool_counters[6] = jobs[0].draft_select ? 1 : 0;
  const int min_admit = std::max(1, C / 4);
  const bool serial = sessions[0]->profile;
  int cursor = 0, done = 0;
  while (done < n_jobs && rc_final == TTX_OK) {
    bool progressed = false;
    int only = -1;
    if (serial)
      for (int i = n_jobs - 1; i >= 0; --i)
        if (jobs[i].phase != 3) only = i;
    for (int i = 0; i < n_jobs && rc_final == TTX_OK; ++i) {
      if (serial && i != only) continue;
      PoolJob& j = jobs[i];
      ttx_session* s = j.s;
      volatile HostInfo* hi = s->host_info;
      if (j.phase == 1) {
        if (j.probe_pending) {
          if (((volatile ProbeInfo*)s->probe_info)->probes_done < j.probes) {
            if (j.progress.stalled()) {
              rc_final = session_hung(s);
              hung = true;
              break;
            }
            continue;
          }
          j.progress.advanced();
          rc_final = pool_launch_drafts(j);
          progressed = true;
          continue;
        }
        if (j.launched > 0 && hi->steps_done < j.launched) {
          if (j.progress.stalled()) {
            rc_final = session_hung(s);
            hung = true;
            break;
          }
          continue;
        }
        j.progress.advanced();
        int n_act = (j.launched == 0) ? 0 : hi->n_active;
        const int free_slots = C - n_act;
        if (serial && j.quota_end < 0) j.quota_end = cursor + cdiv(R_total - cursor, n_jobs - i);
        const int list_end = serial ? j.quota_end : R_total;
        if (cursor < list_end && (n_act == 0 || free_slots >= min_admit)) {
          int n_running = 0;
          for (const PoolJob& o : jobs) n_running += (o.phase == 1);
          const int remaining = list_end - cursor;
          int share = std::max(1, cdiv(remaining, std::max(1, serial ? 1 : n_running)));
          if (!serial && j.launched == 0 && (long long)n_jobs * C >= R_total) share = std::max(1, cdiv(remaining, n_jobs - i));
          const int take = std::min({free_slots, remaining, share});
          int Ls_new = 2;
          for (int r = cursor; r < cursor + take; ++r) Ls_new = std::max(Ls_new, (int)h_len[r]);
          rc_final = pool_admit(j, d_src + (size_t)cursor * Ls_all, Ls_all, take, Ls_new, cursor, d_out, d_traj, d_fin_step);
          if (rc_final != TTX_OK) break;
          cursor += take;
          n_act += take;
        }
        if (n_act == 0) {
          if (hipEventRecord(s->ev_c, j.st) != hipSuccess ||
              hipMemcpyAsync(s->host_state, s->state.as<DecState>(), sizeof(DecState), hipMemcpyDeviceToHost, j.st) != hipSuccess ||
              hipEventRecord(s->ev_done, j.st) != hipSuccess) {
            rc_final = fail(TTX_ERR_HIP, "slot pool: enqueueing the final state read-back failed");
            break;
          }
          j.phase = 2;
        } else {
          if (j.launched > (long long)(p->max_len + 2) * (R_total + 1)) { rc_final = fail(TTX_ERR_HIP, "decode loop failed to terminate"); break; }
          rc_final = pool_launch_step(j, n_act);
        }
        progressed = true;
      } else if (j.phase == 2) {
        if (hipEventQuery(s->ev_done) == hipSuccess) {
          const DecState& hs = *s->host_state;
          if (stats) {
            stats->model_calls += hs.steps;
            stats->accepted_tokens += hs.accepted;
            stats->produced_tokens += hs.produced;
            stats->verified_positions += hs.verified_positions;
            stats->kv_prefix_positions += hs.kv_prefix_positions;
            stats->src_positions += hs.src_positions;
            stats->src_tokens_padded += j.src_tokens_padded;
            collect_gemm_profile(s, j.st);
            float ms = 0.f;
            if (hipEventElapsedTime(&ms, s->ev_a, s->ev_c) == hipSuccess) stats->decode_ms += ms;
          }
          if (getenv("TTX_TWO_PHASE_STATS"))
            fprintf(stderr, "[ttx two-phase] pool %d: %d steps, %lld split (%lld without a draft pass), %lld slot-steps probed, %lld matched, "
                            "%lld draft rows executed, %lld drafts matched\n",
                    i, j.launched, j.split_steps, j.skipped_draft_passes, j.slot_steps, j.matched_slot_steps,
                    j.rows_executed - j.slot_steps - j.unsplit_rows, j.drafts_matched);
          {
            long long* pc = sessions[0]->pool_counters;
            pc[0] += j.launched; pc[1] += j.split_steps; pc[2] += j.slot_steps; pc[3] += j.matched_slot_steps;
            pc[4] += j.drafts_matched; pc[5] += j.rows_executed;
          }
          if (hs.error == 3 && rc_final == TTX_OK)
            rc_final = fail(TTX_ERR_ROW_REPLAY, "a row emitted PAD inside its sequence: decode the batches as given");
          else if (hs.error && rc_final == TTX_OK)
            rc_final = fail(TTX_ERR_HIP, "slot pool bookkeeping failed (admitted more rows than free slots)");
          j.phase = 3;
          ++done;
          progressed = true;
        }
      }
    }
    if (!progressed) __builtin_ia32_pause();
  }
  if (hung) {
    for (int i = 0; i < n_jobs; ++i) jobs[i].s->dead = true;
  } else {
    for (int i = 0; i < n_jobs; ++i)
      if (jobs[i].s && jobs[i].s->own_stream) (void)hipStreamSynchronize(jobs[i].s->own_stream);
  }
  if (stats) stats->status = rc_final;
  return rc_final;
}

static int generate_many_impl(ttx_session** sessions, int n_sessions, int n_batches, const int64_t* const* d_src, const int* B,
                              const int* Ls, const ttx_gen_params* p, int64_t* const* d_out, int16_t* const* d_traj,
                              int32_t* const* d_fin, ttx_gen_stats* stats, void* stream) {
  if (!sessions || n_sessions <= 0 || n_batches < 0 || !d_src || !B || !Ls || !p || !d_out)
    return fail(TTX_ERR_INVALID, "bad argument to ttx_greedy_speculative_generate_many");
  if (d_traj)
    for (int i = 0; i < n_batches; ++i)
      if (!d_traj[i] || !d_fin || !d_fin[i]) return fail(TTX_ERR_INVALID, "missing trace buffer for a batch");
  for (int i = 0; i < n_batches; ++i) TTX_TRY(gen_validate(sessions[0], d_src[i], B[i], Ls[i], p, d_out[i], false));
  if (sessions[0]->profile) n_sessions = 1;
  HIP_TRY(hipSetDevice(sessions[0]->m->device));
  release_retired();
  hipStream_t caller = (hipStream_t)stream;
  for (int i = 0; i < n_sessions; ++i) TTX_TRY(session_alive(sessions[i]));
  EventGuard ready_guard;
  HIP_TRY(hipEventCreateWithFlags(&ready_guard.e, hipEventDisableTiming));
  hipEvent_t ready = ready_guard.e;
  HIP_TRY(hipEventRecord(ready, caller));
  bool hung = false;
  std::vector<GenJob> jobs(n_sessions);
  for (int i = 0; i < n_sessions; ++i) {
    TTX_TRY(ensure_own_stream(sessions[i]));
    HIP_TRY(hipStreamWaitEvent(sessions[i]->own_stream, ready, 0));
  }
  const int D1 = p->draft_len + 1;
  int next = 0, done = 0, rc_final = TTX_OK;
  while (done < n_batches) {
    bool progressed = false;
    for (int i = 0; i < n_sessions; ++i) {
      GenJob& j = jobs[i];
      ttx_session* s = sessions[i];
      if (j.phase == 0) {
        if (next < n_batches) {
          j.batch = next++;
          int rc = gen_start(j, s, s->own_stream, d_src[j.batch], B[j.batch], Ls[j.batch], p, d_out[j.batch],
                             stats ? &stats[j.batch] : nullptr, false, d_traj ? d_traj[j.batch] : nullptr,
                             d_traj ? d_fin[j.batch] : nullptr);
          if (rc != TTX_OK) { rc_final = rc; done = n_batches; break; }
          progressed = true;
        }
        continue;
      }
      volatile HostInfo* hi = s->host_info;
      if (j.phase == 1) {
        if (hi->stop) {
          if (j.launched == 0 && hipStreamQuery(s->own_stream) != hipSuccess) continue;
          int rc = gen_finish_enqueue(j);
          if (rc != TTX_OK) { rc_final = rc; done = n_batches; break; }
          progressed = true;
        } else if (hi->steps_done >= j.launched && (j.launched > 0 || hipStreamQuery(s->own_stream) == hipSuccess)) {
          if (j.launched > p->max_len + 2) { rc_final = fail(TTX_ERR_HIP, "decode loop failed to terminate"); done = n_batches; break; }
          int rc = gen_launch_step(j, hi->width + D1);
          if (rc != TTX_OK) { rc_final = rc; done = n_batches; break; }
          progressed = true;
          j.progress.advanced();
        } else if (j.launched > 0 && j.progress.stalled()) {
          rc_final = session_hung(s);
          hung = true;
          done = n_batches;
          break;
        }
      } else if (j.phase == 2) {
        if (hipEventQuery(s->ev_done) == hipSuccess) {
          int rc = gen_finish_collect(j);
          if (rc != TTX_OK && rc_final == TTX_OK) rc_final = rc;
          ++done;
          progressed = true;
        }
      }
    }
    if (!progressed) __builtin_ia32_pause();
  }
  if (hung) {
    for (int i = 0; i < n_sessions; ++i) sessions[i]->dead = true;
  } else {
    for (int i = 0; i < n_sessions; ++i) (void)hipStreamSynchronize(sessions[i]->own_stream);
  }
  return rc_final;
}

extern "C" int ttx_greedy_speculative_generate_many(ttx_session** sessions, int n_sessions, int n_batches,
                                                    const int64_t* const* d_src, const int* B, const int* Ls,
                                                    const ttx_gen_params* p, int64_t* const* d_out, ttx_gen_stats* stats,
                                                    void* stream) {
  return generate_many_impl(sessions, n_sessions, n_batches, d_src, B, Ls, p, d_out, nullptr, nullptr, stats, stream);
}

extern "C" int ttx_greedy_speculative_generate_rows(ttx_session** sessions, int n_sessions, int n_batches,
                                                    const int64_t* const* d_src, const int* B, const int* Ls,
// ... 1117 lines not shown
  HIP_TRY(hipSetDevice(s->m->device));
  if (d_m) {
    int32_t m = -1;
    HIP_TRY(hipStreamSynchronize(st));
    HIP_TRY(hipMemcpy(&m, d_m, 4, hipMemcpyDeviceToHost));
    if (m < 0 || m > m_max) return fail(TTX_ERR_INVALID, "ttx_debug_argmax: the live row count on the device is outside [0, m_max]");
  }
  hipLaunchKernelGGL(k_argmax, dim3(cdiv(m_max, 4)), dim3(256), 0, st, d_logits, V, d_pred, d_m, m_max);
  HIP_TRY(hipGetLastError());
  return TTX_OK;
}

static int embed_debug(ttx_session* s, const float* d_table, int V, const float* d_pe, int pe_rows, int d, float* d_x,
                       const int32_t* d_tok, int rows, int L, const int32_t* d_act_idx, const int32_t* d_front,
                       const int32_t* d_gen, int gen_ld, const int32_t* d_drafts, int B, int N, int D, int n_active, int step,
                       const int32_t* d_row_map, int m_rows, void* stream) {
  hipStream_t st = reinterpret_cast<hipStream_t>(stream);
  if (!s || !d_table || !d_pe || !d_x) return fail(TTX_ERR_INVALID, "null argument to ttx_debug_embed");
  if (!dbg_model_d(d)) return fail(TTX_ERR_INVALID, "ttx_debug_embed: d must be 64, 128, 256, 512 or 1024");
  if (V < 1 || pe_rows < 1) return fail(TTX_ERR_INVALID, "ttx_debug_embed: V and pe_rows must be positive");
  if (!dbg_aligned16(d_table) || !dbg_aligned16(d_pe) || !dbg_aligned16(d_x))
    return fail(TTX_ERR_INVALID, "ttx_debug_embed: float operands must be 16-byte aligned");
  HIP_TRY(hipSetDevice(s->m->device));
  EmbedArgs e{};
  e.table = d_table; e.pe = d_pe; e.X = d_x; e.d = d; e.V = V;
  if (!step) {
    if (!d_tok || rows < 1 || L < 1) return fail(TTX_ERR_INVALID, "ttx_debug_embed: full mode needs tokens, rows >= 1 and L >= 1");
    if (pe_rows < L + 1) return fail(TTX_ERR_INVALID, "ttx_debug_embed: the positional table must have L + 1 rows");
    e.tok = d_tok; e.rows = rows; e.L = L;
    hipLaunchKernelGGL((k_embed<false>), dim3(cdiv(rows, 4)), dim3(256), 0, st, e);
    HIP_TRY(hipGetLastError());
    return TTX_OK;
  }
  if (!d_act_idx || !d_front || !d_gen || !d_drafts) return fail(TTX_ERR_INVALID, "ttx_debug_embed: step mode needs act_idx, front, gen and drafts");
  if (B < 1 || N < 1 || D < 1 || gen_ld < 1) return fail(TTX_ERR_INVALID, "ttx_debug_embed: step mode needs B, N, D and gen_ld >= 1");
  if (n_active < 0 || n_active > B) return fail(TTX_ERR_INVALID, "ttx_debug_embed: n_active must lie in [0, B]");
  int max_front = 0;
  TTX_TRY(dbg_check_slots("ttx_debug_embed", d_act_idx, d_front, B, n_active, gen_ld, D, st, &max_front));
  if (n_active > 0 && pe_rows < max_front + D + 2) return fail(TTX_ERR_INVALID, "ttx_debug_embed: the positional table must have front + D + 2 rows");
  const int RPS = step_rps(N, D);
  if (d_row_map) {
    if (m_rows < 0 || m_rows > n_active * RPS) return fail(TTX_ERR_INVALID, "ttx_debug_embed_select: m_rows must lie in [0, n_active * (1 + N*D)]");
    std::vector<int32_t> map((size_t)std::max(m_rows, 1));
    HIP_TRY(hipStreamSynchronize(st));
    if (m_rows > 0) HIP_TRY(hipMemcpy(map.data(), d_row_map, (size_t)m_rows * 4, hipMemcpyDeviceToHost));
    for (int i = 0; i < m_rows; ++i)
      if (map[i] < 0 || map[i] >= n_active * RPS) return fail(TTX_ERR_INVALID, "ttx_debug_embed_select: row_map must hold layout rows of the live slots");
  }
  DecState* dst = nullptr;
  HIP_TRY(hipMalloc((void**)&dst, sizeof(DecState)));
  DecState* hs = reinterpret_cast<DecState*>(s->host_state);
  *hs = DecState{};
  hs->n_active = n_active; hs->r_rows = n_active * N; hs->m_rows = d_row_map ? m_rows : n_active * RPS;
  hipError_t err = hipMemcpyAsync(dst, hs, sizeof(DecState), hipMemcpyHostToDevice, st);
  if (err == hipSuccess) {
    e.st = dst; e.act_idx = d_act_idx; e.front = d_front; e.gen = d_gen; e.gen_ld = gen_ld; e.drafts = d_drafts; e.N = N; e.D = D;
    e.row_map = d_row_map;
    hipLaunchKernelGGL((k_embed<true>), dim3(cdiv(B * RPS, 4)), dim3(256), 0, st, e);
    err = hipGetLastError();
  }
  const hipError_t esync = hipStreamSynchronize(st);
  (void)hipFree(dst);
  HIP_TRY(err);
  HIP_TRY(esync);
  return TTX_OK;
}

extern "C" int ttx_debug_embed(ttx_session* s, const float* d_table, int V, const float* d_pe, int pe_rows, int d, float* d_x,
                               const int32_t* d_tok, int rows, int L, const int32_t* d_act_idx, const int32_t* d_front,
                               const int32_t* d_gen, int gen_ld, const int32_t* d_drafts, int B, int N, int D, int n_active, int step,
                               void* stream) {
  return embed_debug(s, d_table, V, d_pe, pe_rows, d, d_x, d_tok, rows, L, d_act_idx, d_front, d_gen, gen_ld, d_drafts, B, N, D, n_active,
                     step, nullptr, 0, stream);
}

extern "C" int ttx_debug_embed_select(ttx_session* s, const float* d_table, int V, const float* d_pe, int pe_rows, int d, float* d_x,
                                      const int32_t* d_act_idx, const int32_t* d_front, const int32_t* d_gen, int gen_ld,
                                      const int32_t* d_drafts, int B, int N, int D, int n_active, const int32_t* d_row_map, int m_rows,
                                      void* stream) {
  return embed_debug(s, d_table, V, d_pe, pe_rows, d, d_x, nullptr, 0, 0, d_act_idx, d_front, d_gen, gen_ld, d_drafts, B, N, D, n_active, 1,
                     d_row_map, m_rows, stream);
}

extern "C" int ttx_debug_accept(ttx_session* s, const ttx_debug_accept_args* a, int64_t* state, void* stream) {
  hipStream_t st = reinterpret_cast<hipStream_t>(stream);
  if (!s || !a || !state) return fail(TTX_ERR_INVALID, "null argument to ttx_debug_accept");
  if (!a->d_act_idx || !a->d_front || !a->d_gen || !a->d_pred || !a->d_rec)
    return fail(TTX_ERR_INVALID, "ttx_debug_accept: act_idx, front, gen, pred and rec are required");
  const bool greedy = a->greedy != 0;
  if (greedy && (a->row_rule || a->pool || a->N != 1 || a->D != 0))
    return fail(TTX_ERR_INVALID, "ttx_debug_accept: plain greedy runs with N = 1, D = 0 and neither row_rule nor pool");
  if (!greedy && (!a->d_drafts || !a->d_haspad || a->N < 1 || a->D < 1))
    return fail(TTX_ERR_INVALID, "ttx_debug_accept: the speculative step needs drafts, haspad, N >= 1 and D >= 1");
  if (a->pool && !a->row_rule) return fail(TTX_ERR_INVALID, "ttx_debug_accept: pool implies row_rule");
  if (!greedy && !a->pool && !a->d_out) return fail(TTX_ERR_INVALID, "ttx_debug_accept: out is required outside pool mode");
  if (a->row_rule && !a->pool && (!a->d_traj || !a->d_fin_step)) return fail(TTX_ERR_INVALID, "ttx_debug_accept: row_rule needs traj and fin_step");
  if (a->pool && (!a->d_rstep || !a->d_row_of || !a->d_pool_out || !a->d_pool_traj || !a->d_pool_fin_step || a->pool_rows < 1))
    return fail(TTX_ERR_INVALID, "ttx_debug_accept: pool mode needs rstep, row_of and the caller-side out, traj and fin_step rows");
  if (a->row_rule && a->traj_ld < 1) return fail(TTX_ERR_INVALID, "ttx_debug_accept: traj_ld must be positive");
  if (a->B < 1 || a->max_len < 1 || a->gen_ld < 1 || a->Ls < 0) return fail(TTX_ERR_INVALID, "ttx_debug_accept: B, max_len and gen_ld must be positive");
  if (a->threads != 0 && a->threads != 256 && a->threads != ACCEPT_THREADS) return fail(TTX_ERR_INVALID, "ttx_debug_accept: threads is 0, 256 or 1024");
  if (a->threads == 256 && a->B > 256) return fail(TTX_ERR_INVALID, "ttx_debug_accept: 256 threads are never launched for B > 256");
  if (greedy && a->threads == ACCEPT_THREADS) return fail(TTX_ERR_INVALID, "ttx_debug_accept: plain greedy always runs with 256 threads");
  const int n_active = (int)state[0];
  if (state[0] < 0 || state[0] > a->B) return fail(TTX_ERR_INVALID, "ttx_debug_accept: n_active must lie in [0, B]");
  if (a->gen_ld < a->max_len) return fail(TTX_ERR_INVALID, "ttx_debug_accept: gen_ld must cover max_len (finished rows are copied from gen)");
  HIP_TRY(hipSetDevice(s->m->device));
  int max_front = 0;
  if (greedy) {
    if (n_active > 0) {
      int32_t f0 = -1;
      HIP_TRY(hipStreamSynchronize(st));
      HIP_TRY(hipMemcpy(&f0, a->d_front, 4, hipMemcpyDeviceToHost));
      if (f0 < 0 || (long long)f0 + 2 > a->gen_ld) return fail(TTX_ERR_INVALID, "ttx_debug_accept: gen_ld is too small for front + D + 2");
    }
  } else {
    TTX_TRY(dbg_check_slots("ttx_debug_accept", a->d_act_idx, a->d_front, a->B, n_active, a->gen_ld, a->D, st, &max_front));
    if (a->pool && n_active > 0) {
      std::vector<int32_t> row_of((size_t)a->B);
      HIP_TRY(hipMemcpy(row_of.data(), a->d_row_of, (size_t)a->B * 4, hipMemcpyDeviceToHost));
      std::vector<int32_t> act((size_t)n_active);
      HIP_TRY(hipMemcpy(act.data(), a->d_act_idx, (size_t)n_active * 4, hipMemcpyDeviceToHost));
      for (int i = 0; i < n_active; ++i)
        if (row_of[act[i]] < 0 || row_of[act[i]] >= a->pool_rows) return fail(TTX_ERR_INVALID, "ttx_debug_accept: row_of must lie in [0, pool_rows)");
    }
  }
  HostInfo* hinfo = nullptr;
  HostInfo* dev_info = nullptr;
  DecState* dst = nullptr;
  PoolIo* dio = nullptr;
  hipError_t err = hipHostMalloc((void**)&hinfo, sizeof(HostInfo), hipHostMallocMapped);
  if (err == hipSuccess) err = hipHostGetDevicePointer((void**)&dev_info, (void*)hinfo, 0);
  if (err == hipSuccess) err = hipMalloc((void**)&dst, sizeof(DecState));
  if (err == hipSuccess && a->pool) err = hipMalloc((void**)&dio, sizeof(PoolIo));
  DecState* hs = reinterpret_cast<DecState*>(s->host_state);
  PoolIo hio{a->d_pool_out, a->d_pool_traj, a->d_pool_fin_step, a->traj_ld, 0};
  if (err == hipSuccess) {
    *hinfo = HostInfo{-1, -1, -1, -1};
    hs->n_active = n_active; hs->r_rows = (int)state[1]; hs->m_rows = (int)state[2]; hs->stop = (int)state[3];
    hs->width = (int)state[4]; hs->steps = (int)state[5]; hs->error = (int)state[6]; hs->n_copy = (int)state[7];
    hs->accepted = state[8]; hs->produced = state[9]; hs->verified_positions = state[10]; hs->kv_prefix_positions = state[11];
    hs->src_positions = state[12];
    err = hipMemcpyAsync(dst, hs, sizeof(DecState), hipMemcpyHostToDevice, st);
  }
  if (err == hipSuccess && a->pool) err = hipMemcpyAsync(dio, &hio, sizeof(PoolIo), hipMemcpyHostToDevice, st);
  if (err == hipSuccess) {
    LoopArgs la{};
    la.st = dst; la.act_idx = a->d_act_idx; la.front = a->d_front; la.gen = a->d_gen; la.gen_ld = a->gen_ld;
    la.drafts = a->d_drafts; la.pred = a->d_pred; la.rec = reinterpret_cast<CopyRec*>(a->d_rec); la.out = a->d_out;
    la.host = dev_info; la.haspad = a->d_haspad;
    la.row_rule = a->row_rule ? 1 : 0; la.traj = a->d_traj; la.traj_ld = a->traj_ld; la.fin_step = a->d_fin_step;
    la.pool = a->pool ? 1 : 0; la.rstep = a->d_rstep; la.row_of = a->d_row_of; la.io = dio;
    la.B = a->B; la.N = a->N; la.D = a->D; la.Ls = a->Ls; la.max_len = a->max_len; la.pad = a->pad; la.bos = a->bos; la.eos = a->eos;
    if (greedy) hipLaunchKernelGGL(k_greedy_accept, dim3(1), dim3(256), 0, st, la);
    else hipLaunchKernelGGL(k_accept, dim3(1), dim3(a->threads ? a->threads : (a->B > 256 ? ACCEPT_THREADS : 256)), 0, st, la);
    err = hipGetLastError();
  }
  if (err == hipSuccess) err = hipMemcpyAsync(hs, dst, sizeof(DecState), hipMemcpyDeviceToHost, st);
  const hipError_t esync = hipStreamSynchronize(st);
  if (err == hipSuccess && esync == hipSuccess) {
    state[0] = hs->n_active; state[1] = hs->r_rows; state[2] = hs->m_rows; state[3] = hs->stop; state[4] = hs->width;
    state[5] = hs->steps; state[6] = hs->error; state[7] = hs->n_copy;
    state[8] = hs->accepted; state[9] = hs->produced; state[10] = hs->verified_positions; state[11] = hs->kv_prefix_positions;
    state[12] = hs->src_positions;
    state[13] = hinfo->stop; state[14] = hinfo->steps_done; state[15] = hinfo->width; state[16] = hinfo->n_active;
  }
  if (dio) (void)hipFree(dio);
  if (dst) (void)hipFree(dst);
  if (hinfo) (void)hipHostFree(hinfo);
  HIP_TRY(err);
  HIP_TRY(esync);
  return TTX_OK;
}

static int kvcopy_debug(const char* who, ttx_session* s, const int32_t* d_rec, int n_copy, const float* d_qkv, int64_t qkv_layer_stride,
                        float* d_kcache, float* d_vcache, int64_t cache_layer_stride, int64_t cache_seq_stride, int N, int D, int d, int B,
                        int Ld, const int32_t* d_pos2, const float* d_qkv_probe, int64_t probe_layer_stride, hipStream_t st,
                        const int32_t* d_row_base = nullptr, const int32_t* d_draft_mask = nullptr) {
  const std::string w(who);
  if ((d_row_base || d_draft_mask) && !d_pos2) return fail(TTX_ERR_INVALID, w + ": row_base and draft_mask need pos2");
  if (!s || !d_rec || !d_qkv || !d_kcache || !d_vcache) return fail(TTX_ERR_INVALID, "null argument to " + w);
  if (!dbg_model_d(d)) return fail(TTX_ERR_INVALID, w + ": d must be 64, 128, 256, 512 or 1024");
  if (B < 1 || Ld < 1 || N < 1 || D < 0) return fail(TTX_ERR_INVALID, w + ": B, Ld and N must be positive, D >= 0");
  if (n_copy < 0 || n_copy > B) return fail(TTX_ERR_INVALID, w + ": n_copy must lie in [0, B]");
  if (!dbg_aligned16(d_qkv) || !dbg_aligned16(d_kcache) || !dbg_aligned16(d_vcache))
    return fail(TTX_ERR_INVALID, w + ": float operands must be 16-byte aligned");
  const int RPS = step_rps(N, D);
  if ((qkv_layer_stride & 3) || qkv_layer_stride < (int64_t)B * RPS * 3 * d)
    return fail(TTX_ERR_INVALID, w + ": qkv_layer_stride must be a multiple of 4 covering B * (1 + N*D) rows of 3d");
  if ((cache_seq_stride & 3) || cache_seq_stride < d || (cache_layer_stride & 3) || cache_layer_stride < (int64_t)B * cache_seq_stride)
    return fail(TTX_ERR_INVALID, w + ": the cache strides must be multiples of 4, a row's covering d and a layer's B rows");
  if ((d_pos2 != nullptr) != (d_qkv_probe != nullptr)) return fail(TTX_ERR_INVALID, w + ": pos2 and qkv_probe come together");
  if (d_pos2 && (!dbg_aligned16(d_qkv_probe) || (probe_layer_stride & 3) || probe_layer_stride < (int64_t)B * 3 * d))
    return fail(TTX_ERR_INVALID, w + ": qkv_probe must be 16-byte aligned and its layer stride a multiple of 4 covering B rows of 3d");
  HIP_TRY(hipSetDevice(s->m->device));
  if (n_copy > 0) {
    std::vector<CopyRec> rec((size_t)n_copy);
    std::vector<int> pos((size_t)n_copy, 0);
    HIP_TRY(hipStreamSynchronize(st));
    HIP_TRY(hipMemcpy(rec.data(), d_rec, (size_t)n_copy * sizeof(CopyRec), hipMemcpyDeviceToHost));
    if (d_pos2) HIP_TRY(hipMemcpy(pos.data(), d_pos2, (size_t)n_copy * sizeof(int), hipMemcpyDeviceToHost));
    for (int i = 0; i < n_copy; ++i) {
      const CopyRec& r = rec[i];
      if (r.b < 0 || r.b >= B || r.best < 0 || r.best >= N || r.nacc < 0 || r.nacc > D || r.front_old < 0 ||
          ((int64_t)r.front_old + r.nacc + 1) * d > cache_seq_stride)
        return fail(TTX_ERR_INVALID, w + ": a record is outside the operands (b, best, nacc or front_old + nacc + 1 positions)");
      if (d_pos2 && (pos[i] < -1 || pos[i] >= B || (pos[i] < 0 && r.nacc != 0)))
        return fail(TTX_ERR_INVALID, w + ": pos2 must lie in [-1, B), and a slot without a draft pass (-1) accepts nothing");
    }
    if (d_row_base || d_draft_mask) {
      int n_pos = 0, total = 0;
      for (int i = 0; i < n_copy; ++i) n_pos = std::max(n_pos, pos[i] + 1);
      std::vector<int32_t> mask;
      TTX_TRY(dbg_check_select(w, d_row_base, d_draft_mask, n_pos, N, D, st, &mask, &total));
      for (int i = 0; i < n_copy; ++i)
        if (pos[i] >= 0 && rec[i].nacc > 0 && !(((unsigned)mask[pos[i]] >> rec[i].best) & 1u))
          return fail(TTX_ERR_INVALID, w + ": the best draft of a slot that accepted tokens must be a present one");
    }
  }
  DecState* dst = nullptr;
  HIP_TRY(hipMalloc((void**)&dst, sizeof(DecState)));
  DecState* hs = reinterpret_cast<DecState*>(s->host_state);
  *hs = DecState{};
  hs->n_copy = n_copy;
  hipError_t err = hipMemcpyAsync(dst, hs, sizeof(DecState), hipMemcpyHostToDevice, st);
  if (err == hipSuccess) {
    KvCopyArgs kc{};
    kc.st = dst; kc.rec = reinterpret_cast<const CopyRec*>(d_rec); kc.qkv = d_qkv; kc.qkv_layer_stride = (long long)qkv_layer_stride;
    kc.kcache = d_kcache; kc.vcache = d_vcache; kc.cache_layer_stride = (long long)cache_layer_stride;
    kc.cache_seq_stride = (long long)cache_seq_stride; kc.N = N; kc.D = D; kc.d = d;
    kc.pos2 = d_pos2; kc.qkv_probe = d_qkv_probe; kc.probe_layer_stride = (long long)probe_layer_stride;
    kc.row_base = d_row_base; kc.draft_mask = d_draft_mask;
    hipLaunchKernelGGL(k_kvcopy, dim3(B, Ld), dim3(256), 0, st, kc);
    err = hipGetLastError();
  }
  const hipError_t esync = hipStreamSynchronize(st);
  (void)hipFree(dst);
  HIP_TRY(err);
  HIP_TRY(esync);
  return TTX_OK;
}

extern "C" int ttx_debug_kvcopy(ttx_session* s, const int32_t* d_rec, int n_copy, const float* d_qkv, int64_t qkv_layer_stride,
                                float* d_kcache, float* d_vcache, int64_t cache_layer_stride, int64_t cache_seq_stride, int N, int D,
                                int d, int B, int Ld, void* stream) {
  return kvcopy_debug("ttx_debug_kvcopy", s, d_rec, n_copy, d_qkv, qkv_layer_stride, d_kcache, d_vcache, cache_layer_stride,
                      cache_seq_stride, N, D, d, B, Ld, nullptr, nullptr, 0, reinterpret_cast<hipStream_t>(stream));
}

extern "C" int ttx_debug_kvcopy_split(ttx_session* s, const int32_t* d_rec, int n_copy, const float* d_qkv, int64_t qkv_layer_stride,
                                      float* d_kcache, float* d_vcache, int64_t cache_layer_stride, int64_t cache_seq_stride, int N,
                                      int D, int d, int B, int Ld, const int32_t* d_pos2, const float* d_qkv_probe,
                                      int64_t probe_layer_stride, void* stream) {
  return kvcopy_debug("ttx_debug_kvcopy_split", s, d_rec, n_copy, d_qkv, qkv_layer_stride, d_kcache, d_vcache, cache_layer_stride,
                      cache_seq_stride, N, D, d, B, Ld, d_pos2, d_qkv_probe, probe_layer_stride, reinterpret_cast<hipStream_t>(stream));
}

extern "C" int ttx_debug_kvcopy_select(ttx_session* s, const int32_t* d_rec, int n_copy, const float* d_qkv, int64_t qkv_layer_stride,
                                       float* d_kcache, float* d_vcache, int64_t cache_layer_stride, int64_t cache_seq_stride, int N,
                                       int D, int d, int B, int Ld, const int32_t* d_pos2, const float* d_qkv_probe,
                                       int64_t probe_layer_stride, const int32_t* d_row_base, const int32_t* d_draft_mask, void* stream) {
  if ((d_row_base != nullptr) != (d_draft_mask != nullptr))
    return fail(TTX_ERR_INVALID, "ttx_debug_kvcopy_select: row_base and draft_mask come together");
  return kvcopy_debug("ttx_debug_kvcopy_select", s, d_rec, n_copy, d_qkv, qkv_layer_stride, d_kcache, d_vcache, cache_layer_stride,
                      cache_seq_stride, N, D, d, B, Ld, d_pos2, d_qkv_probe, probe_layer_stride, reinterpret_cast<hipStream_t>(stream),
                      d_row_base, d_draft_mask);
}

static int dbg_state_with(hipStream_t st, int n_active, int steps, DecState** out) {
  DecState* dst = nullptr;
  HIP_TRY(hipMalloc((void**)&dst, 2 * sizeof(DecState)));
  DecState h[2] = {};
  h[0].n_active = n_active;
  h[1].steps = steps;
  const hipError_t e = hipMemcpy(dst, h, sizeof(h), hipMemcpyHostToDevice);
  (void)st;
  if (e != hipSuccess) { (void)hipFree(dst); HIP_TRY(e); }
  *out = dst;
  return TTX_OK;
}

static int probe_split_debug(ttx_session* s, const int32_t* d_act_idx, const int32_t* d_pred_probe, const int32_t* d_drafts,
                             int B, int N, int D, int n_active, int32_t* d_act2, int32_t* d_pos2, int32_t* result,
                             int32_t* d_draft_mask, int32_t* d_row_base, int32_t* d_row_map, void* stream) {
  hipStream_t st = reinterpret_cast<hipStream_t>(stream);
  if (!s || !d_act_idx || !d_pred_probe || !d_drafts || !d_act2 || !d_pos2 || !result)
    return fail(TTX_ERR_INVALID, "null argument to ttx_debug_probe_split");
  if (B < 1 || N < 1 || D < 1) return fail(TTX_ERR_INVALID, "ttx_debug_probe_split: B, N and D must be positive");
  if (n_active < 0 || n_active > B) return fail(TTX_ERR_INVALID, "ttx_debug_probe_split: n_active must lie in [0, B]");
  HIP_TRY(hipSetDevice(s->m->device));
  HIP_TRY(hipStreamSynchronize(st));
  if (n_active > 0) {
    std::vector<int> act((size_t)n_active);
    HIP_TRY(hipMemcpy(act.data(), d_act_idx, (size_t)n_active * 4, hipMemcpyDeviceToHost));
    std::vector<char> seen((size_t)B, 0);
    for (int b : act) {
      if (b < 0 || b >= B || seen[b]) return fail(TTX_ERR_INVALID, "ttx_debug_probe_split: act_idx must be distinct rows of [0, B)");
      seen[b] = 1;
    }
  }
  ProbeInfo* hinfo = nullptr;
  if (hipHostMalloc((void**)&hinfo, sizeof(ProbeInfo), hipHostMallocMapped) != hipSuccess) return fail(TTX_ERR_NOMEM, "hipHostMalloc failed");
  hinfo->matches = -1; hinfo->probes_done = -1; hinfo->rows = -1;
  DecState* dst = nullptr;
  int rc = dbg_state_with(st, n_active, result[4], &dst);
  int* d_exec = nullptr;
  hipError_t err = hipSuccess;
  if (rc == TTX_OK) err = hipMalloc((void**)&d_exec, 4);
  if (rc == TTX_OK && err == hipSuccess) {
    ProbeSplitArgs ps{};
    ps.st = dst; ps.act_idx = d_act_idx; ps.pred_probe = d_pred_probe; ps.drafts = d_drafts; ps.N = N; ps.D = D;
    ps.act2 = d_act2; ps.pos2 = d_pos2; ps.st2 = dst + 1; ps.exec_rows = d_exec;
    ps.draft_mask = d_draft_mask; ps.row_base = d_row_base; ps.row_map = d_row_map;
    err = hipHostGetDevicePointer((void**)&ps.host, (void*)hinfo, 0);
    if (err == hipSuccess) {
      hipLaunchKernelGGL(k_probe_split, dim3(1), dim3(B > 256 ? ACCEPT_THREADS : 256), 0, st, ps);
      err = hipGetLastError();
    }
    if (err == hipSuccess) err = hipStreamSynchronize(st);
    DecState h2{};
    int exec = 0;
    if (err == hipSuccess) err = hipMemcpy(&h2, dst + 1, sizeof(DecState), hipMemcpyDeviceToHost);
    if (err == hipSuccess) err = hipMemcpy(&exec, d_exec, 4, hipMemcpyDeviceToHost);
    if (err == hipSuccess) {
// ... 99 lines not shown
```

### translation-transformer_amd/csrc/ttx_internal.h

```cpp
#pragma once
#include "ttx.h"
#include "ttx_common.hip.h"

#include <map>
#include <set>
#include <string>
#include <utility>
#include <vector>

namespace ttx {
struct BeamHost;
struct BeamPoolHost;
}

struct LayerW {
  size_t sa_in_w, sa_in_b, sa_out_w, sa_out_b;
  size_t ca_in_w, ca_in_b, ca_out_w, ca_out_b;
  size_t l1_w, l1_b, l2_w, l2_b;
  size_t n1_w, n1_b, n2_w, n2_b, n3_w, n3_b;
};

struct ttx_model {
  ttx_config cfg;
  int device;
  int activation = TTX_ACT_RELU;
  int n_sessions = 0;

  int n_cu = 256;
  float* blob = nullptr;
  size_t blob_floats = 0;
  std::map<std::string, std::pair<size_t, size_t>> index;
  std::vector<LayerW> enc, dec;
  size_t src_emb, tgt_emb, enc_norm_w, enc_norm_b, dec_norm_w, dec_norm_b, cls_w, cls_b, pe;
  size_t cross_kv_w, cross_kv_b;
  const float* p(size_t off) const { return blob + off; }
};

struct Buf {
  void* p = nullptr;
  size_t cap = 0;
  uint64_t* owner_gen = nullptr;
  template <typename T> T* as() const { return reinterpret_cast<T*>(p); }
};

enum GemmVariant { GV_BIG = 0, GV_SMALL = 1, GV_BIG_FFN2_SLABS = 2, GV_MID = 3 };

enum GemmKernelId { GK_GEMM3 = 1, GK_GEMM_TN = 2, GK_GEMM24_4 = 3, GK_GEMM24_0 = 4, GK_GEMM2_1 = 5, GK_GEMM2_2 = 6, GK_GEMM2_4 = 7,
                    GK_GEMM2_0 = 8, GK_BODY_128x64 = 16 };

enum AttnKernelId { AK_ATTN = 1, AK_ATTN2 = 2, AK_ATTN3 = 3, AK_ATTN3S = 4, AK_ATTN1 = 5 };

enum GraphSite { GS_STEP_SPECULATIVE = 0, GS_STEP_GREEDY = 1, GS_STEP_ROW_RULE = 2, GS_STEP_POOL = 3, GS_BEAM_ITER = 4, GS_BEAM_POOL_ITER = 5 };
typedef std::vector<int> GraphKey;

struct GraphCache {
  std::map<GraphKey, hipGraphExec_t> map;
  std::set<GraphKey> warmed;
  size_t limit;
  explicit GraphCache(size_t limit_) : limit(limit_) {}
  void clear() {
    for (auto& kv : map) (void)hipGraphExecDestroy(kv.second);
    map.clear(); warmed.clear();
  }
};

#define TTX_SESSION_BUFS(X)                                                                                                      \
                                                                      \
  X(x) X(x1) X(x2) X(xf) X(ao) X(q2) X(hbuf) X(slab) X(qkv) X(logits) X(ckv)                                                      \
                                                                                                                    \
  X(tok_src) X(src_valid) X(memory) X(memkv)                                                                                     \
                                                                                                               \
  X(tok_tgt) X(mem_pad_tmp)                                                                                                      \
   \
  X(ev_logits) X(ev_pred) X(ev_nll)                                                                                              \
   \
                                                                                                      \
  X(sc_src_of) X(am_length)                                                                                                                   \
                                                                                                                       \
  X(drafts) X(gen) X(front) X(act_idx) X(rec) X(pred) X(state) X(kcache) X(vcache) X(src32) X(outbuf) X(haspad) X(traj)           \
  X(fin_step)                                                                                                                    \
                                                                                            \
  X(rstep) X(row_of) X(src_len) X(new_slot) X(pool_io) X(memkv_new) X(valid_new) X(drafts_new)                                    \
       \
            \
  X(qkv_probe) X(pred_probe) X(pred_draft) X(act2) X(pos2) X(state2)                                                             \
         \
  X(draft_mask) X(row_base) X(row_map)                                                                                           \
                                        \
  X(snap_logits) X(snap_act) X(snap_front) X(snap_gen) X(snap_state)                                                             \
  X(leaf_score) X(leaf_tok) X(leaf_cnt) X(beam_summary)                                                                          \
                                                                                               \
  X(bs_cand_next) X(bs_len_next) X(bs_fin_next) X(bs_logp_next) X(bs_len) X(bs_fin) X(bs_active) X(bs_logp) X(bs_per_cand)        \
  X(bs_best_n) X(bs_best_slot) X(bs_chosen) X(bs_parent) X(bs_parent_draft) X(bs_mark) X(bs_drafts_src) X(bs_cnt) X(bs_hit)       \
                                                                                 \
  X(t_prev_len) X(t_slot_of) X(t_src_of)                                                                                         \
                                            \
  X(bp_row_of) X(bp_batch) X(bp_cand) X(bp_cand_len) X(bp_tok) X(bp_new_slot) X(bp_io) X(bp_grp) X(bp_src_acc) X(bp_enc_qkv)
#define TTX_DECLARE_BUF(name) Buf name;
#define TTX_REGISTER_BUF(name) all.push_back(&name);

#ifndef TTX_BIG_MIN_TILES
#define TTX_BIG_MIN_TILES 400
#endif
struct ttx_session {
  ttx_model* m;
  std::vector<Buf*> all;
  TTX_SESSION_BUFS(TTX_DECLARE_BUF)
  Buf tk[2], tv[2];
  int snap_B = 0, snap_rps = 0, snap_gen_ld = 0, snap_step = 0;
  ttx::ProbeInfo* probe_info = nullptr;
  long long pool_counters[7] = {};
  ttx::BeamHost* beam_host = nullptr;
  ttx::BeamPoolHost* bp_host = nullptr;
  ttx::HostInfo* host_info = nullptr;
  hipStream_t own_stream = nullptr;
  uint64_t alloc_generation = 0;
  uint64_t graphs_generation = 0;
  bool dead = false;
  bool use_graphs = true;
  GraphCache step_graphs{512};
  GraphCache iter_graphs{256};
  hipEvent_t ev_done = nullptr;
  void drop_graphs() { step_graphs.clear(); iter_graphs.clear(); }
  void graphs_current() { if (graphs_generation != alloc_generation) { drop_graphs(); graphs_generation = alloc_generation; } }
  ttx::DecState* host_state = nullptr;
  bool attr_attn2[2][8] = {};
  bool attr_select = false, attr_step = false, attr_topk = false, attr_pool_select = false;
  bool attr_attn_probs[8] = {};
  int qkv_small_rows = 800;
  int small_rows = 2000;
  int ffn2_slab_rows = 5600;
  int big_min_tiles = TTX_BIG_MIN_TILES;
  int last_gemm_kernel = 0, last_gemm_big_min_tiles = 0;
  int attn_split = -1;
  int attn_row = -1;
  bool attn_fallback = false;
  int attn_force = 0;
  int attn_sel_N = 0, attn_sel_D = 0;
  int last_attn_kernel = 0;
  unsigned attn_kernels_seen = 0;
  bool profile = false;
  std::vector<std::pair<hipEvent_t, hipEvent_t>> ev_pool;
  size_t ev_used = 0;
  double prof_ms = 0;
  double prof_empty_pair_ms = -1;
  long long prof_launches = 0;
  bool host_timing = false;
  double host_launch_us = 0;
  long long host_captures = 0;
  double host_capture_us = 0;
  long long host_launches = 0;
  hipEvent_t ev_a = nullptr, ev_b = nullptr, ev_c = nullptr;
  ttx_session() {
    TTX_SESSION_BUFS(TTX_REGISTER_BUF)
    for (Buf* b : {&tk[0], &tk[1], &tv[0], &tv[1]}) all.push_back(b);
    for (Buf* b : all) b->owner_gen = &alloc_generation;
  }
};

namespace ttx {

int fail(int code, const std::string& msg);

#define HIP_TRY(expr)                                                                                  \
  do {                                                                                                 \
    hipError_t _e = (expr);                                                                            \
    if (_e != hipSuccess)                                                                              \
      return ttx::fail(TTX_ERR_HIP, std::string(#expr) + ": " + hipGetErrorString(_e) + " (" __FILE__ ":" + \
                                        std::to_string(__LINE__) + ")");                               \
  } while (0)

#define TTX_TRY(expr)        \
  do {                       \
    int _r = (expr);         \
    if (_r != TTX_OK) return _r; \
  } while (0)

static inline int cdiv(int a, int b) { return (a + b - 1) / b; }

int gemm_slice_k(int K);
int gemm_splits(int N, int K, bool step, int variant);
int launch_gemm(ttx_session* s, hipStream_t st, const float* X, int ldx, const float* W, int ldw, const float* bias,
                float* Y, int ldy, const int* m_ptr, int Mmax, int N, int K, int act, int splits, long long slab_stride,
                int variant);
int launch_finish(ttx_session* s, hipStream_t st, const float* slabs, int n_slabs, long long slab_stride, const float* bias,
                  const float* resid, const float* g1, const float* b1, const float* g2, const float* b2,
                  const uint8_t* row_valid, float* Y, const int* m_ptr, int Mmax);
int launch_finish_d(hipStream_t st, const float* slabs, int n_slabs, long long slab_stride, const float* bias, const float* resid,
                    const float* g1, const float* b1, const float* g2, const float* b2, const uint8_t* row_valid, float* Y,
                    const int* m_ptr, int Mmax, int d, float eps);
int gemm_debug(ttx_session* s, const float* d_x, int ldx, const float* d_w, int ldw, const float* d_bias, float* d_y, int ldy,
               const int32_t* d_m, int m_max, int N, int K, int act, int splits, long long slab_stride, int variant, int tiling,
               int32_t* kernel_id, hipStream_t st);
int finish_debug(ttx_session* s, const float* d_slabs, int n_slabs, long long slab_stride, const float* d_bias, const float* d_resid,
                 const float* d_g1, const float* d_b1, const float* d_g2, const float* d_b2, const uint8_t* d_row_valid, float* d_y,
                 const int32_t* d_m, int m_max, int d, float eps, hipStream_t st);
int gemm_bench(ttx_session* s, int M, int N, int K, int splits, int variant, int reps, double* us_per_launch, double* max_abs_diff);

int launch_attn(int mode, ttx_session* s, hipStream_t st, const AttnArgs& a, int groups, int H, int q_per_group, int max_keys,
                int N = 1, int D1 = 1);
int attn_debug(ttx_session* s, const AttnArgs& in, int H, int head_dim, int mode, int groups, int n_active, int max_keys, int kernel,
               int32_t* kernel_id, hipStream_t st);
int attn_staged_key_limit(int head_dim, int q_per_group);

}
```

### translation-transformer_amd/csrc/ttx_loop_kernels.hip.h

```cpp
#pragma once
#include "ttx_common.hip.h"
#include "ttx_select.h"

namespace ttx {

struct EmbedArgs {
  const float* table; const float* pe; float* X; int d;
  int V;
  const int* tok; int rows; int L;
  const DecState* st; const int* act_idx; const int* front; const int* gen; int gen_ld;
  const int* drafts; int N; int D;
  const int* row_map;
};

template <bool STEP>
__global__ __launch_bounds__(256) void k_embed(EmbedArgs a) {
  const int row = blockIdx.x * 4 + (threadIdx.x >> 6);
  const int lane = threadIdx.x & 63;
  int tok, pos;
  if constexpr (STEP) {
    if (row >= a.st->m_rows) return;
    const int RPS = step_rps(a.N, a.D);
    const int lrow = a.row_map ? a.row_map[row] : row;
    const int rs = lrow % RPS;
    const int b = a.act_idx[lrow / RPS];
    const int f = a.front[b];
    if (rs == 0) {
      tok = a.gen[(size_t)b * a.gen_ld + f];
      pos = f;
    } else {
      const int n = (rs - 1) / a.D, j = (rs - 1) % a.D;
      tok = a.drafts[((size_t)b * a.N + n) * a.D + j];
      pos = f + 1 + j;
    }
  } else {
    if (row >= a.rows) return;
    tok = a.tok[row];
    pos = row % a.L;
  }
  if ((unsigned)tok >= (unsigned)a.V) tok = 0;
  const float* e = a.table + (size_t)tok * a.d;
  const float* p = a.pe + (size_t)(pos + 1) * a.d;
  float* x = a.X + (size_t)row * a.d;
  for (int c = lane * 4; c < a.d; c += 256) {
    const float4 ev = *reinterpret_cast<const float4*>(e + c);
    const float4 pv = *reinterpret_cast<const float4*>(p + c);
    *reinterpret_cast<float4*>(x + c) = make_float4(ev.x + pv.x, ev.y + pv.y, ev.z + pv.z, ev.w + pv.w);
  }
}

__global__ void k_prepare_tokens(const int64_t* in, int* out, uint8_t* valid, int n, int pad) {
  const int i = blockIdx.x * blockDim.x + threadIdx.x;
  if (i < n) {
    const int t = (int)in[i];
    out[i] = t;
    if (valid) valid[i] = (t != pad) ? 1 : 0;
  }
}

__global__ __launch_bounds__(256) void k_argmax(const float* logits, int V, int* pred, const int* m_ptr, int M) {
  const int rows = m_ptr ? *m_ptr : M;
  const int row = blockIdx.x * 4 + (threadIdx.x >> 6);
  if (row >= rows) return;
  const int lane = threadIdx.x & 63;
  const float* p = logits + (size_t)row * V;
  float best = -INFINITY;
  int bi = 0x7fffffff;
  for (int c = lane; c < V; c += 64) {
    const float v = p[c];
    if (v > best) { best = v; bi = c; }
  }
#pragma unroll
  for (int o = 32; o > 0; o >>= 1) {
    const float ov = __shfl_xor(best, o, 64);
    const int oi = __shfl_xor(bi, o, 64);
    if (ov > best || (ov == best && oi < bi)) { best = ov; bi = oi; }
  }
  if (lane == 0) pred[row] = (bi < V) ? bi : 0;
}

template <typename OutT>
__global__ __launch_bounds__(64) void k_make_drafts(const int* src, int src_ld, int off, int L, int N, int D,
                                                    int eos, int pad, int repl, OutT* out) {
  extern __shared__ int pre[];
  const int b = blockIdx.x;
  const int need = N + D - 1;
  const int Lp = L > need ? L : need;
  const int W = Lp - D + 1;
  const int* s = src + (size_t)b * src_ld + off;
  __shared__ int n_clean;
  if (threadIdx.x == 0) {
    int c = 0;
    pre[0] = 0;
    for (int i = 0; i < Lp; ++i) {
      const int t = (i < L) ? s[i] : pad;
      c += (t == eos || t == pad) ? 1 : 0;
      pre[i + 1] = c;
    }
    int clean = 0;
    for (int w = 0; w < W; ++w) clean += (pre[w + D] - pre[w] == 0) ? 1 : 0;
    n_clean = clean;
  }
  __syncthreads();
  const int take = n_clean > N ? n_clean : N;
  const float ratio = __fdiv_rn((float)(take - 1), (float)(N - 1 > 1 ? N - 1 : 1));
  for (int e = threadIdx.x; e < N * D; e += blockDim.x) {
    const int i = e / D, j = e % D;
    int w = (int)__fmul_rn((float)i, ratio);
    if (w > W - 1) w = W - 1;
    const int p = w + j;
    int t = (p < L) ? s[p] : pad;
    if (t == eos || t == pad) t = repl;
    out[((size_t)b * N + i) * D + e % D] = (OutT)t;
  }
}

struct LoopArgs {
  DecState* st; int* act_idx; int* front; int* gen; int gen_ld;
  const int* drafts; const int* pred;
  CopyRec* rec; int64_t* out; HostInfo* host; int* haspad;
  int row_rule; short* traj; int traj_ld; int* fin_step;
  int pool; int* rstep; int* row_of; const struct PoolIo* io;
  int B, N, D, Ls, max_len, pad, bos, eos;
  const int* exec_rows;
};
struct PoolIo { int64_t* out; short* traj; int* fin_step; int traj_ld; int pad_; };

__global__ void k_loop_init(LoopArgs a) {
  const int tid = blockIdx.x * blockDim.x + threadIdx.x;
  const int total = a.B * a.gen_ld;
  for (int i = tid; i < total; i += gridDim.x * blockDim.x) a.gen[i] = (i % a.gen_ld == 0) ? a.bos : a.pad;
  for (int i = tid; i < a.B * a.max_len; i += gridDim.x * blockDim.x) a.out[i] = a.pad;
  for (int i = tid; i < a.B; i += gridDim.x * blockDim.x) {
    a.act_idx[i] = i; a.front[i] = 0; a.haspad[i] = 0;
    if (a.row_rule) a.fin_step[i] = 0;
  }
  if (a.row_rule)
    for (int i = tid; i < a.B * a.traj_ld; i += gridDim.x * blockDim.x) a.traj[i] = (i % a.traj_ld == 0) ? 0 : -1;
  if (tid == 0) {
    DecState s;
    s.n_active = a.B; s.r_rows = a.B * a.N; s.m_rows = a.B * step_rps(a.N, a.D);
    s.width = 1; s.steps = 0; s.error = 0; s.n_copy = 0;
    s.stop = (1 >= a.max_len) ? 1 : 0;
    if (s.stop) { s.n_active = 0; s.r_rows = 0; s.m_rows = 0; }
    s.accepted = s.produced = s.verified_positions = s.kv_prefix_positions = s.src_positions = 0;
    *a.st = s;
    a.host->width = 1;
    a.host->steps_done = 0;
    a.host->stop = s.stop;
    __threadfence_system();
  }
}

constexpr int ACCEPT_THREADS = 1024;
__global__ __launch_bounds__(ACCEPT_THREADS) void k_accept(LoopArgs a) {
  __shared__ int s_maxfront, s_anyfin, s_suspect, s_nn, s_maxf_new, s_nfin;
  __shared__ int s_finlist[256];
  __shared__ long long s_acc, s_prefix;
  __shared__ int s_scan[ACCEPT_THREADS];
  DecState* st = a.st;
  const int Bc = st->n_active;
  if (Bc == 0) return;
  const int D1 = a.D + 1, RPS = step_rps(a.N, a.D);
  if (threadIdx.x == 0) { s_maxfront = 0; s_anyfin = 0; s_acc = 0; s_prefix = 0; s_suspect = 0; s_nn = 0; s_maxf_new = 0; s_nfin = 0; }
  __syncthreads();
  for (int slot = threadIdx.x; slot < Bc; slot += blockDim.x) {
    const int b = a.act_idx[slot];
    const int f = a.front[b];
    const int* ps = a.pred + (size_t)slot * RPS;
    int best = 0, bacc = -1;
    for (int n = 0; n < a.N; ++n) {
      const int* dr = a.drafts + ((size_t)b * a.N + n) * a.D;
      const int* pr = ps + 1 + n * a.D - 1;
      int acc = a.D;
      for (int j = a.D - 1; j >= 0; --j)
        if (dr[j] != (j == 0 ? ps[0] : pr[j])) acc = j;
      if (acc > bacc) { bacc = acc; best = n; }
    }
    const int* pr = ps + 1 + best * a.D - 1;
    int* g = a.gen + (size_t)b * a.gen_ld;
    bool fin = false, sawpad = false;
    for (int j = 0; j <= bacc; ++j) {
      const int t = (j == 0) ? ps[0] : pr[j];
      g[f + 1 + j] = t;
      fin |= (t == a.eos);
      sawpad |= (t == a.pad);
    }
    if (sawpad) a.haspad[b] = 1;
    a.front[b] = f + bacc + 1;
    int flags = fin ? 1 : 0;
    if (a.row_rule) {
      int it = st->steps + 1;
      short* trow = a.traj + (size_t)b * a.traj_ld;
      int* finp = a.fin_step + b;
      if (a.pool) {
        it = a.rstep[b] + 1;
        a.rstep[b] = it;
        trow = a.io->traj + (size_t)a.row_of[b] * a.traj_ld;
        finp = a.io->fin_step + a.row_of[b];
      }
      if (it < a.traj_ld) trow[it] = (short)(f + bacc + 1);
      if (fin) *finp = it;
      else if (f + D1 + 1 >= a.max_len) flags = 2;
    }
    a.rec[slot] = CopyRec{b, best, bacc, f, flags};
    atomicMax(&s_maxfront, f);
    atomicAdd((unsigned long long*)&s_acc, (unsigned long long)bacc);
    atomicAdd((unsigned long long*)&s_prefix, (unsigned long long)f);
    if (fin) {
      s_anyfin = 1;
      const int k = atomicAdd(&s_nfin, 1);
      if (k < 256) s_finlist[k] = b;
    }
  }
  __syncthreads();
  const int width = s_maxfront + 1 + D1;
  const int wcopy = width < a.max_len ? width : a.max_len;
  int nn_before = 0;
  for (int base = 0; base < Bc; base += blockDim.x) {
    const int slot = base + threadIdx.x;
    const int code = slot < Bc ? a.rec[slot].b : -1;
    const int keep = (slot < Bc && a.rec[slot].flags == 0) ? 1 : 0;
    const unsigned long long mask = __ballot(keep);
    const int lane = threadIdx.x & 63, wave = threadIdx.x >> 6;
    if (lane == 0) s_scan[wave] = __popcll(mask);
    __syncthreads();
    int before = 0, total = 0;
    for (int w = 0; w < (int)(blockDim.x >> 6); ++w) {
      const int c = s_scan[w];
      before += (w < wave) ? c : 0;
      total += c;
    }
    if (keep) {
      a.act_idx[nn_before + before + __popcll(mask & ((1ull << lane) - 1ull))] = code;
      if (a.haspad[code]) s_suspect = 1;
      atomicMax(&s_maxf_new, a.front[code]);
    }
    nn_before += total;
    __syncthreads();
  }
  const int wout = a.row_rule ? a.max_len : wcopy;
  auto copy_row = [&](int b, int first, int stride) {
    const int* g = a.gen + (size_t)b * a.gen_ld;
    int64_t* orow = a.pool ? a.io->out + (size_t)a.row_of[b] * a.max_len : a.out + (size_t)b * a.max_len;
    for (int c = first; c < wout; c += stride) orow[c] = g[c];
  };
  if (s_nfin <= 256) {
    for (int k = threadIdx.x >> 6; k < s_nfin; k += (int)(blockDim.x >> 6)) copy_row(s_finlist[k], threadIdx.x & 63, 64);
  } else {
    for (int slot = 0; slot < Bc; ++slot)
      if (a.rec[slot].flags == 1) copy_row(a.rec[slot].b, threadIdx.x, blockDim.x);
  }
  __syncthreads();
  if (threadIdx.x == 0) {
    const int nn = nn_before;
    st->n_copy = Bc;
    st->steps += 1;
    st->accepted += s_acc;
    st->produced += s_acc + Bc;
    st->verified_positions += a.exec_rows ? (long long)*a.exec_rows : (long long)Bc * RPS;
    st->kv_prefix_positions += s_prefix;
    st->src_positions += (long long)Bc * a.Ls;
    st->width = width;
    if (s_anyfin && width > a.max_len && !a.row_rule) st->error = 1;
    int stop = (nn == 0 || (!a.row_rule && width >= a.max_len)) ? 1 : 0;
    if (a.row_rule && s_suspect) st->error = 3;
    if (!stop && s_suspect && !a.row_rule) {
      const int maxf = s_maxf_new;
      for (int c = 0; c <= maxf && !stop; ++c) {
        bool allpad = true;
        for (int i = 0; i < nn && allpad; ++i) {
          const int b = a.act_idx[i];
          if (a.front[b] >= c && a.gen[(size_t)b * a.gen_ld + c] != a.pad) allpad = false;
        }
        if (allpad) { st->error = 2; stop = 1; }
      }
    }
    st->stop = stop;
    st->n_active = stop ? 0 : nn;
    st->r_rows = stop ? 0 : nn * a.N;
    st->m_rows = stop ? 0 : nn * RPS;
    a.host->width = width;
    a.host->n_active = stop ? 0 : nn;
    a.host->stop = stop;
    __threadfence_system();
    a.host->steps_done = st->steps;
  }
}

__global__ void k_pool_init(LoopArgs a) {
  const int tid = blockIdx.x * blockDim.x + threadIdx.x;
  for (int i = tid; i < a.B; i += gridDim.x * blockDim.x) { a.act_idx[i] = 0; a.front[i] = 0; a.haspad[i] = 0; a.rstep[i] = 0; a.row_of[i] = 0; }
  if (tid == 0) {
    DecState s;
    s.n_active = 0; s.r_rows = 0; s.m_rows = 0; s.width = 1; s.steps = 0; s.error = 0; s.n_copy = 0; s.stop = 0;
    s.accepted = s.produced = s.verified_positions = s.kv_prefix_positions = s.src_positions = 0;
    *a.st = s;
    a.host->width = 1; a.host->steps_done = 0; a.host->stop = 0; a.host->n_active = 0;
    __threadfence_system();
  }
}

struct PoolAdmitArgs {
  DecState* st; int* act_idx; int* front; int* haspad; int* rstep; int* row_of; int* src_len; int* new_slot; HostInfo* host;
  int B, N, D, R, first_row, Ls_new;
};

__global__ __launch_bounds__(256) void k_pool_admit(PoolAdmitArgs a) {
  extern __shared__ int s_used[];
  DecState* st = a.st;
  const int n = st->n_active;
  for (int i = threadIdx.x; i < a.B; i += blockDim.x) s_used[i] = 0;
  __syncthreads();
  for (int i = threadIdx.x; i < n; i += blockDim.x) s_used[a.act_idx[i]] = 1;
  __syncthreads();
  if (threadIdx.x == 0) {
    int got = 0;
    for (int b = 0; b < a.B && got < a.R; ++b) {
      if (s_used[b]) continue;
      a.new_slot[got] = b;
      a.act_idx[n + got] = b;
      a.front[b] = 0; a.haspad[b] = 0; a.rstep[b] = 0;
      a.row_of[b] = a.first_row + got;
      a.src_len[b] = a.Ls_new;
      ++got;
    }
    const int nn = n + got;
    st->n_active = nn; st->r_rows = nn * a.N; st->m_rows = nn * step_rps(a.N, a.D);
    st->stop = 0;
    if (got != a.R) st->error = 4;
    a.host->stop = 0;
    a.host->n_active = nn;
    __threadfence_system();
  }
}

struct PoolFillArgs {
  const int* new_slot; int R;
  int* gen; int gen_ld; int bos; int pad;
  int* drafts; const int* drafts_new; int nd;
  uint8_t* src_valid; const uint8_t* valid_new; int Ls_cap; int Ls_new;
  float* memkv; const float* memkv_new; int kv_row;
  int64_t* out_rows; short* traj_rows; int* fin_rows; int max_len; int traj_ld; int first_row;
};

__global__ __launch_bounds__(256) void k_pool_fill(PoolFillArgs a) {
  const int i = blockIdx.x;
  const int b = a.new_slot[i];
  const int t = threadIdx.x;
  if (blockIdx.y == 0) {
    for (int c = t; c < a.gen_ld; c += blockDim.x) a.gen[(size_t)b * a.gen_ld + c] = (c == 0) ? a.bos : a.pad;
    for (int c = t; c < a.nd; c += blockDim.x) a.drafts[(size_t)b * a.nd + c] = a.drafts_new[(size_t)i * a.nd + c];
    for (int c = t; c < a.Ls_cap; c += blockDim.x)
      a.src_valid[(size_t)b * a.Ls_cap + c] = (c < a.Ls_new) ? a.valid_new[(size_t)i * a.Ls_new + c] : (uint8_t)0;
    const size_t row = (size_t)(a.first_row + i);
    for (int c = t; c < a.max_len; c += blockDim.x) a.out_rows[row * a.max_len + c] = a.pad;
    for (int c = t; c < a.traj_ld; c += blockDim.x) a.traj_rows[row * a.traj_ld + c] = (c == 0) ? 0 : -1;
    if (t == 0) a.fin_rows[row] = 0;
  } else {
    const int key = blockIdx.y - 1;
    const float4* src = reinterpret_cast<const float4*>(a.memkv_new + ((size_t)i * a.Ls_new + key) * a.kv_row);
    float4* dst = reinterpret_cast<float4*>(a.memkv + ((size_t)b * a.Ls_cap + key) * a.kv_row);
    for (int c = t; c < a.kv_row / 4; c += blockDim.x) dst[c] = src[c];
  }
}

__global__ void k_prepare_tokens_2d(const int64_t* in, int ld_in, int* out, uint8_t* valid, int rows, int cols, int pad) {
  const int i = blockIdx.x * blockDim.x + threadIdx.x;
  if (i < rows * cols) {
    const int r = i / cols, c = i - r * cols;
    const int tk = (int)in[(size_t)r * ld_in + c];
    out[i] = tk;
    if (valid) valid[i] = (tk != pad) ? 1 : 0;
  }
}

__global__ __launch_bounds__(256) void k_greedy_accept(LoopArgs a) {
  __shared__ int s_running;
  DecState* st = a.st;
  const int Bc = st->n_active;
  if (Bc == 0) return;
  if (threadIdx.x == 0) s_running = 0;
  __syncthreads();
  const int f = a.front[0];
  for (int b = threadIdx.x; b < Bc; b += blockDim.x) {
    const int t = a.pred[b];
    a.gen[(size_t)b * a.gen_ld + f + 1] = t;
    a.front[b] = f + 1;
    a.rec[b] = CopyRec{b, 0, 0, f, 0};
    if (t != a.eos && t != a.pad) s_running = 1;
  }
  __syncthreads();
  if (threadIdx.x == 0) {
    st->n_copy = Bc;
    st->steps += 1;
    st->produced += Bc;
    st->verified_positions += Bc;
    st->kv_prefix_positions += (long long)Bc * f;
    st->src_positions += (long long)Bc * a.Ls;
    st->width = f + 2;
    const int stop = (!s_running || f + 1 >= a.max_len - 1) ? 1 : 0;
    st->stop = stop;
    if (stop) { st->n_active = 0; st->r_rows = 0; st->m_rows = 0; }
    a.host->width = f + 2;
    a.host->steps_done = st->steps;
    a.host->stop = stop;
    __threadfence_system();
  }
}

__global__ void k_gen_to_out(const int* gen, int gen_ld, int64_t* out, int B, int max_len) {
  const int i = blockIdx.x * blockDim.x + threadIdx.x;
  if (i < B * max_len) out[i] = gen[(size_t)(i / max_len) * gen_ld + (i % max_len)];
}

struct KvCopyArgs {
  const DecState* st; const CopyRec* rec;
  const float* qkv; long long qkv_layer_stride;
  float* kcache; float* vcache; long long cache_layer_stride; long long cache_seq_stride;
  int N, D, d;
  const int* pos2; const float* qkv_probe; long long probe_layer_stride;
  const int* row_base; const int* draft_mask;
};

__global__ __launch_bounds__(256) void k_kvcopy(KvCopyArgs a) {
  const int slot = blockIdx.x, l = blockIdx.y;
  if (slot >= a.st->n_copy) return;
  const CopyRec r = a.rec[slot];
  const int RPS = step_rps(a.N, a.D);
  const float* src = a.qkv + (size_t)l * a.qkv_layer_stride + ((size_t)slot * RPS) * 3 * a.d;
  int nrows = r.nacc + 1;
  int best_row = 1 + r.best * a.D;
  if (a.pos2) {
    const int p = a.pos2[slot];
    if (p >= 0 && a.row_base) {
      src = a.qkv + (size_t)l * a.qkv_layer_stride + (size_t)a.row_base[p] * 3 * a.d;
      best_row = max(step_sel_row((unsigned)a.draft_mask[p], r.best, 0, a.D), 0);
    } else if (p >= 0) src = a.qkv + (size_t)l * a.qkv_layer_stride + ((size_t)p * RPS) * 3 * a.d;
    else { src = a.qkv_probe + (size_t)l * a.probe_layer_stride + (size_t)slot * 3 * a.d; nrows = 1; }
  }
  float* kc = a.kcache + (size_t)l * a.cache_layer_stride + (size_t)r.b * a.cache_seq_stride + (size_t)r.front_old * a.d;
  float* vc = a.vcache + (size_t)l * a.cache_layer_stride + (size_t)r.b * a.cache_seq_stride + (size_t)r.front_old * a.d;
  const int per_row = a.d / 4;
  const int total = nrows * per_row;
  for (int e = threadIdx.x; e < total; e += blockDim.x) {
// ... 1203 lines not shown
```

### translation-transformer_amd/model.py

```python
from __future__ import annotations

import ctypes as C
import os
import math
from typing import NamedTuple

import numpy as np
import torch

from . import _native as N


def reference_pe_table(emb: int, max_len: int = 5000) -> torch.Tensor:
    pe = torch.zeros(max_len, emb)
    position = torch.arange(0, max_len, dtype=torch.float).unsqueeze(1)
    div_term = torch.exp(torch.arange(0, emb, 2).float() * (-math.log(10000.0) / emb))
    pe[:, 0::2] = torch.sin(position * div_term)
    pe[:, 1::2] = torch.cos(position * div_term)
    return torch.vstack((torch.zeros(1, emb), pe)).contiguous()


def _strip(state: dict) -> dict:
    if any(k.startswith("model.") for k in state):
        return {k[len("model."):]: v for k, v in state.items() if k.startswith("model.")}
# ... 88 lines not shown
        arr = (N.Tensor * len(host))()
        keep = []
        for i, (k, v) in enumerate(host.items()):
            name = k.encode()
            keep.append((name, v))
            arr[i] = N.Tensor(name, C.cast(v.data_ptr(), C.POINTER(C.c_float)), v.numel())
        N.check(self._lib.ttx_model_create(C.byref(self.cfg), arr, len(host), dev.index or 0, C.byref(self._model)))
        N.check(self._lib.ttx_model_set_activation(self._model, act))
        N.check(self._lib.ttx_session_create(self._model, C.byref(self._session)))

    def blob_tensor(self) -> torch.Tensor:
        ptr, nbytes = C.c_void_p(), C.c_int64()
        N.check(self._lib.ttx_model_blob(self._model, C.byref(ptr), C.byref(nbytes)))
        with torch.cuda.device(self.device):
            t = torch.as_tensor(_DeviceSpan(int(ptr.value), int(nbytes.value)), device=self.device)
        t._ttx_owner = self
        return t

    def _stream(self) -> C.c_void_p:
        return C.c_void_p(torch.cuda.current_stream(self.device).cuda_stream)

    @property
    def session(self) -> C.c_void_p:
        return self._session

    def new_session(self) -> C.c_void_p:
        s = C.c_void_p()
        had = os.environ.get("TTX_PROFILE_GEMM")
        if self._profile_sessions:
            os.environ["TTX_PROFILE_GEMM"] = "1"
        try:
            N.check(self._lib.ttx_session_create(self._model, C.byref(s)))
        finally:
            if self._profile_sessions:
                if had is None:
                    os.environ.pop("TTX_PROFILE_GEMM", None)
                else:
                    os.environ["TTX_PROFILE_GEMM"] = had
        return s

    def session_pool(self, n: int) -> list:
        pool = getattr(self, "_pool", None)
        if pool is None:
            pool = self._pool = [self._session]
        while len(pool) < n:
            pool.append(self.new_session())
        return pool[:n]

    def kernel_profile(self) -> dict:
        ms, n, e = C.c_double(), C.c_int64(), C.c_double()
        tot_ms, tot_n, over = 0.0, 0, []
        for sess in (getattr(self, "_pool", None) or [self._session]):
            N.check(self._lib.ttx_last_kernel_profile(sess, C.byref(ms), C.byref(n), C.byref(e)))
            tot_ms += ms.value
            tot_n += n.value
            if n.value and e.value > 0:
                over.append(e.value)
        return {"gemm_ms": tot_ms, "launches": tot_n, "pair_overhead_ms": float(np.median(over)) if over else 0.0}

    @staticmethod
    def _ptr(t: torch.Tensor | None):
        return None if t is None else t.data_ptr()

    def debug_gemm(self, x: torch.Tensor, w: torch.Tensor, bias: torch.Tensor | None, y: torch.Tensor, n: int, k: int,
                   m_max: int, m_live: torch.Tensor | None = None, relu: bool = False, splits: int = 0, slab_stride: int = 0,
                   variant: int = 0, tiling: int = 0, activation: int | None = None) -> int:
        kid = C.c_int32(0)
        if activation is not None:
            N.check(self._lib.ttx_debug_gemm_act(self._session, x.data_ptr(), x.stride(0), w.data_ptr(), w.stride(0), self._ptr(bias),
                                                 y.data_ptr(), y.stride(0), self._ptr(m_live), int(m_max), int(n), int(k),
                                                 int(activation), int(splits), int(slab_stride), int(variant), int(tiling),
                                                 C.byref(kid), self._stream()))
            return int(kid.value)
        N.check(self._lib.ttx_debug_gemm(self._session, x.data_ptr(), x.stride(0), w.data_ptr(), w.stride(0), self._ptr(bias),
                                         y.data_ptr(), y.stride(0), self._ptr(m_live), int(m_max), int(n), int(k), int(relu),
                                         int(splits), int(slab_stride), int(variant), int(tiling), C.byref(kid), self._stream()))
        return int(kid.value)

    def debug_finish_ln(self, slabs: torch.Tensor, n_slabs: int, slab_stride: int, bias: torch.Tensor, resid: torch.Tensor,
                        g1: torch.Tensor, b1: torch.Tensor, g2: torch.Tensor | None, b2: torch.Tensor | None,
                        row_valid: torch.Tensor | None, y: torch.Tensor, m_max: int, d: int, eps: float = 1e-5,
                        m_live: torch.Tensor | None = None) -> None:
        N.check(self._lib.ttx_debug_finish_ln(self._session, slabs.data_ptr(), int(n_slabs), int(slab_stride), bias.data_ptr(),
                                              resid.data_ptr(), g1.data_ptr(), b1.data_ptr(), self._ptr(g2), self._ptr(b2),
                                              self._ptr(row_valid), y.data_ptr(), self._ptr(m_live), int(m_max), int(d),
                                              float(eps), self._stream()))

    def debug_attn(self, mode: int, q: torch.Tensor, k: torch.Tensor, v: torch.Tensor, out: torch.Tensor, heads: int, scale: float,
                   groups: int, max_keys: int, L: int = 0, Lk: int = 0, tok: torch.Tensor | None = None, pad: int = 0,
                   key_pad: torch.Tensor | None = None, mem_row: torch.Tensor | None = None, act_idx: torch.Tensor | None = None,
                   front: torch.Tensor | None = None, src_of: torch.Tensor | None = None, src_len: torch.Tensor | None = None,
                   kcache: torch.Tensor | None = None, vcache: torch.Tensor | None = None, cache_seq_stride: int = 0,
                   cache_slot: torch.Tensor | None = None, gen_ld: int = 0, n: int = 1, d: int = 0, n_active: int = 0,
                   kernel: int = 0, head_dim: int = 32, choose_as: tuple | None = None) -> int:
        kid = C.c_int32(0)
        assert k.stride(0) == v.stride(0)
        if choose_as is not None:
            N.check(self._lib.ttx_debug_attn_as(self._session, q.data_ptr(), q.stride(0), k.data_ptr(), v.data_ptr(), k.stride(0),
                                                out.data_ptr(), int(heads), int(head_dim), float(scale), int(L), int(Lk), self._ptr(tok),
                                                int(pad), self._ptr(key_pad), self._ptr(mem_row), self._ptr(act_idx), self._ptr(front),
                                                self._ptr(src_of), self._ptr(src_len), self._ptr(kcache), self._ptr(vcache),
                                                int(cache_seq_stride), self._ptr(cache_slot), int(gen_ld), int(n), int(d), int(mode),
                                                int(groups), int(n_active), int(max_keys), int(kernel), C.byref(kid),
                                                int(choose_as[0]), int(choose_as[1]), self._stream()))
            return int(kid.value)
        N.check(self._lib.ttx_debug_attn_hd(self._session, q.data_ptr(), q.stride(0), k.data_ptr(), v.data_ptr(), k.stride(0),
                                            out.data_ptr(), int(heads), int(head_dim), float(scale), int(L), int(Lk), self._ptr(tok),
                                            int(pad), self._ptr(key_pad), self._ptr(mem_row), self._ptr(act_idx), self._ptr(front),
                                            self._ptr(src_of), self._ptr(src_len), self._ptr(kcache), self._ptr(vcache),
                                            int(cache_seq_stride), self._ptr(cache_slot), int(gen_ld), int(n), int(d), int(mode),
                                            int(groups), int(n_active), int(max_keys), int(kernel), C.byref(kid), self._stream()))
        return int(kid.value)

    def debug_attn_probs(self, q: torch.Tensor, k: torch.Tensor, key_pad: torch.Tensor, length: torch.Tensor, heads: int,
                         head_dim: int, T: int, Ls: int, scale: float, mem_row: torch.Tensor | None = None,
                         out_heads: torch.Tensor | None = None, out_mean: torch.Tensor | None = None,
                         out_align: torch.Tensor | None = None) -> None:
        R, Rm = int(length.numel()), int(key_pad.numel()) // int(Ls)
        N.check(self._lib.ttx_debug_attn_probs(self._session, q.data_ptr(), q.stride(0), k.data_ptr(), k.stride(0), key_pad.data_ptr(),
                                               self._ptr(mem_row), length.data_ptr(), R, Rm, int(heads), int(head_dim), int(T), int(Ls),
                                               float(scale), self._ptr(out_heads), self._ptr(out_mean), self._ptr(out_align),
                                               self._stream()))

    @staticmethod
    def attn_probs_key_limit(head_dim: int) -> int:
        return int(N.lib().ttx_attn_probs_key_limit(int(head_dim)))

    def debug_argmax(self, logits: torch.Tensor, pred: torch.Tensor, m_max: int, m_live: torch.Tensor | None = None) -> None:
        N.check(self._lib.ttx_debug_argmax(self._session, logits.data_ptr(), int(logits.shape[1]), pred.data_ptr(),
                                           self._ptr(m_live), int(m_max), self._stream()))

    def debug_embed(self, table: torch.Tensor, pe: torch.Tensor, x: torch.Tensor, tok: torch.Tensor | None = None, rows: int = 0,
                    L: int = 0, act_idx: torch.Tensor | None = None, front: torch.Tensor | None = None,
                    gen: torch.Tensor | None = None, drafts: torch.Tensor | None = None, B: int = 0, n: int = 1, d: int = 0,
                    n_active: int = 0, step: bool = False) -> None:
        N.check(self._lib.ttx_debug_embed(self._session, table.data_ptr(), int(table.shape[0]), pe.data_ptr(), int(pe.shape[0]),
                                          int(table.shape[1]), x.data_ptr(), self._ptr(tok), int(rows), int(L), self._ptr(act_idx),
                                          self._ptr(front), self._ptr(gen), 0 if gen is None else int(gen.stride(0)),
                                          self._ptr(drafts), int(B), int(n), int(d), int(n_active), int(bool(step)), self._stream()))

    def debug_accept(self, state, *, B: int, n: int, d: int, Ls: int, max_len: int, pad: int, bos: int, eos: int, gen_ld: int,
                     greedy: bool = False, threads: int = 0, row_rule: bool = False, pool: bool = False, traj_ld: int = 0,
                     pool_rows: int = 0, **arrays) -> list:
        a = N.DebugAcceptArgs()
        for name, _ in N.DebugAcceptArgs._fields_[:15]:
            t = arrays.pop(name[2:], None)
            setattr(a, name, None if t is None else t.data_ptr())
        assert not arrays, f"unknown operands {sorted(arrays)}"
        a.gen_ld, a.traj_ld, a.pool_rows, a.row_rule, a.pool = int(gen_ld), int(traj_ld), int(pool_rows), int(row_rule), int(pool)
        a.B, a.N, a.D, a.Ls, a.max_len, a.pad, a.bos, a.eos = int(B), int(n), int(d), int(Ls), int(max_len), int(pad), int(bos), int(eos)
        a.greedy, a.threads = int(greedy), int(threads)
        words = (C.c_int64 * N.DEBUG_ACCEPT_STATE_WORDS)(*[int(v) for v in state], *([0] * (N.DEBUG_ACCEPT_STATE_WORDS - len(state))))
        N.check(self._lib.ttx_debug_accept(self._session, C.byref(a), words, self._stream()))
        return [int(v) for v in words]

    def debug_kvcopy(self, rec: torch.Tensor, n_copy: int, qkv: torch.Tensor, kcache: torch.Tensor, vcache: torch.Tensor,
                     n: int, d: int, width: int, B: int) -> None:
        assert kcache.stride() == vcache.stride()
        N.check(self._lib.ttx_debug_kvcopy(self._session, rec.data_ptr(), int(n_copy), qkv.data_ptr(), int(qkv.stride(0)),
                                           kcache.data_ptr(), vcache.data_ptr(), int(kcache.stride(0)), int(kcache.stride(1)),
                                           int(n), int(d), int(width), int(B), int(qkv.shape[0]), self._stream()))

    def debug_kvcopy_split(self, rec: torch.Tensor, n_copy: int, qkv: torch.Tensor, kcache: torch.Tensor, vcache: torch.Tensor,
                           n: int, d: int, width: int, B: int, pos2: torch.Tensor | None = None,
                           qkv_probe: torch.Tensor | None = None) -> None:
        assert kcache.stride() == vcache.stride()
        N.check(self._lib.ttx_debug_kvcopy_split(self._session, rec.data_ptr(), int(n_copy), qkv.data_ptr(), int(qkv.stride(0)),
                                                 kcache.data_ptr(), vcache.data_ptr(), int(kcache.stride(0)), int(kcache.stride(1)),
                                                 int(n), int(d), int(width), int(B), int(qkv.shape[0]), self._ptr(pos2),
                                                 self._ptr(qkv_probe), 0 if qkv_probe is None else int(qkv_probe.stride(0)),
                                                 self._stream()))

    def debug_probe_split(self, act_idx: torch.Tensor, pred_probe: torch.Tensor, drafts: torch.Tensor, n_active: int,
                          act2: torch.Tensor, pos2: torch.Tensor, probes_before: int = 0) -> list:
        B, n, d = drafts.shape
        words = (C.c_int32 * 7)(0, 0, 0, 0, int(probes_before), 0, 0)
        N.check(self._lib.ttx_debug_probe_split(self._session, act_idx.data_ptr(), pred_probe.data_ptr(), drafts.data_ptr(), int(B),
                                                int(n), int(d), int(n_active), act2.data_ptr(), pos2.data_ptr(), words,
                                                self._stream()))
        return [int(v) for v in words]

    def debug_merge_pred(self, pos2: torch.Tensor, pred_probe: torch.Tensor, pred2: torch.Tensor, pred: torch.Tensor, B: int,
                         n: int, d: int, n_active: int) -> None:
        N.check(self._lib.ttx_debug_merge_pred(self._session, pos2.data_ptr(), pred_probe.data_ptr(), pred2.data_ptr(),
                                               pred.data_ptr(), int(B), int(n), int(d), int(n_active), self._stream()))

    def debug_probe_split_select(self, act_idx: torch.Tensor, pred_probe: torch.Tensor, drafts: torch.Tensor, n_active: int,
                                 act2: torch.Tensor, pos2: torch.Tensor, draft_mask: torch.Tensor, row_base: torch.Tensor,
                                 row_map: torch.Tensor, probes_before: int = 0) -> list:
        B, n, d = drafts.shape
        words = (C.c_int32 * 8)(0, 0, 0, 0, int(probes_before), 0, 0, 0)
        N.check(self._lib.ttx_debug_probe_split_select(self._session, act_idx.data_ptr(), pred_probe.data_ptr(), drafts.data_ptr(),
                                                       int(B), int(n), int(d), int(n_active), act2.data_ptr(), pos2.data_ptr(),
                                                       self._ptr(draft_mask), self._ptr(row_base), self._ptr(row_map), words,
                                                       self._stream()))
        return [int(v) for v in words]

    def debug_merge_pred_select(self, pos2: torch.Tensor, pred_probe: torch.Tensor, pred2: torch.Tensor, pred: torch.Tensor, B: int,
                                n: int, d: int, n_active: int, row_base: torch.Tensor | None, draft_mask: torch.Tensor | None) -> None:
        N.check(self._lib.ttx_debug_merge_pred_select(self._session, pos2.data_ptr(), pred_probe.data_ptr(), pred2.data_ptr(),
                                                      pred.data_ptr(), int(B), int(n), int(d), int(n_active), self._ptr(row_base),
                                                      self._ptr(draft_mask), self._stream()))

    def debug_kvcopy_select(self, rec: torch.Tensor, n_copy: int, qkv: torch.Tensor, kcache: torch.Tensor, vcache: torch.Tensor,
                            n: int, d: int, width: int, B: int, pos2: torch.Tensor | None, qkv_probe: torch.Tensor | None,
                            row_base: torch.Tensor | None, draft_mask: torch.Tensor | None) -> None:
        assert kcache.stride() == vcache.stride()
        N.check(self._lib.ttx_debug_kvcopy_select(self._session, rec.data_ptr(), int(n_copy), qkv.data_ptr(), int(qkv.stride(0)),
                                                  kcache.data_ptr(), vcache.data_ptr(), int(kcache.stride(0)), int(kcache.stride(1)),
                                                  int(n), int(d), int(width), int(B), int(qkv.shape[0]), self._ptr(pos2),
                                                  self._ptr(qkv_probe), 0 if qkv_probe is None else int(qkv_probe.stride(0)),
                                                  self._ptr(row_base), self._ptr(draft_mask), self._stream()))

    def debug_embed_select(self, table: torch.Tensor, pe: torch.Tensor, x: torch.Tensor, act_idx: torch.Tensor, front: torch.Tensor,
                           gen: torch.Tensor, drafts: torch.Tensor, B: int, n: int, d: int, n_active: int,
                           row_map: torch.Tensor | None, m_rows: int) -> None:
        N.check(self._lib.ttx_debug_embed_select(self._session, table.data_ptr(), int(table.shape[0]), pe.data_ptr(), int(pe.shape[0]),
                                                 int(table.shape[1]), x.data_ptr(), act_idx.data_ptr(), front.data_ptr(),
                                                 gen.data_ptr(), int(gen.stride(0)), drafts.data_ptr(), int(B), int(n), int(d),
                                                 int(n_active), self._ptr(row_map), int(m_rows), self._stream()))

    def debug_attn_select(self, mode: int, q: torch.Tensor, k: torch.Tensor, v: torch.Tensor, out: torch.Tensor, heads: int,
                          scale: float, groups: int, max_keys: int, row_base: torch.Tensor | None, draft_mask: torch.Tensor | None,
                          Lk: int = 0, tok: torch.Tensor | None = None, pad: int = 0, key_pad: torch.Tensor | None = None,
                          act_idx: torch.Tensor | None = None, front: torch.Tensor | None = None, src_of: torch.Tensor | None = None,
                          src_len: torch.Tensor | None = None, kcache: torch.Tensor | None = None, vcache: torch.Tensor | None = None,
                          cache_seq_stride: int = 0, cache_slot: torch.Tensor | None = None, gen_ld: int = 0, n: int = 1, d: int = 0,
                          n_active: int = 0, kernel: int = 0, **unused) -> int:
        kid = C.c_int32(0)
        assert k.stride(0) == v.stride(0)
        N.check(self._lib.ttx_debug_attn_select(self._session, q.data_ptr(), q.stride(0), k.data_ptr(), v.data_ptr(), k.stride(0),
                                                out.data_ptr(), int(heads), float(scale), int(Lk), self._ptr(tok), int(pad),
                                                self._ptr(key_pad), self._ptr(act_idx), self._ptr(front), self._ptr(src_of),
                                                self._ptr(src_len), self._ptr(kcache), self._ptr(vcache), int(cache_seq_stride),
                                                self._ptr(cache_slot), int(gen_ld), int(n), int(d), int(mode), int(groups),
                                                int(n_active), int(max_keys), int(kernel), C.byref(kid), self._ptr(row_base),
                                                self._ptr(draft_mask), self._stream()))
        return int(kid.value)

    def attn_kernels_seen(self, session=None) -> set:
        mask = int(self._lib.ttx_debug_attn_kernels_seen(self._session if session is None else session))
        if mask < 0:
            N.check(mask)
        return {k for k in range(1, 32) if mask >> k & 1}

    POOL_COUNTERS = ("steps", "split_steps", "slot_steps_probed", "slots_matched", "drafts_matched", "rows_executed", "draft_select")

    def pool_last_counters(self, session=None) -> dict:
        words = (C.c_int64 * 7)()
        N.check(self._lib.ttx_pool_last_counters(self._session if session is None else session, words))
        return dict(zip(self.POOL_COUNTERS, (int(v) for v in words)))

    @staticmethod
    def attn_staged_key_limit(head_dim: int, q_per_group: int) -> int:
        return int(N.lib().ttx_attn_staged_key_limit(int(head_dim), int(q_per_group)))

    def close(self) -> None:
        if getattr(self, "_score_session", None):
            self._lib.ttx_session_destroy(self._score_session)
            self._score_session = None
        for extra in getattr(self, "_pool", [])[1:]:
            self._lib.ttx_session_destroy(extra)
        self._pool = None
        if getattr(self, "_session", None):
            self._lib.ttx_session_destroy(self._session)
            self._session = None
        if getattr(self, "_model", None):
            self._lib.ttx_model_destroy(self._model)
            self._model = None

    def __del__(self):
        try:
            self.close()
        except Exception:
            pass

    def _tokens(self, t: torch.Tensor) -> torch.Tensor:
        return t.to(self.device, torch.int64).contiguous()

    def check_tokens(self, t: torch.Tensor, vocab: int | None = None) -> None:
        if t.numel() == 0:
            return
        lo, hi = int(t.min()), int(t.max())
        if lo < 0 or hi >= (vocab or self.src_vocab_size):
            raise IndexError("index out of range in self")

    def encode_src(self, src: torch.Tensor, src_pad_mask: torch.Tensor | None = None) -> torch.Tensor:
        src = self._tokens(src)
        self.check_tokens(src)
        B, Ls = src.shape
        mem = torch.empty((B, Ls, self.emb_dim), dtype=torch.float32, device=self.device)
        N.check(self._lib.ttx_encode_src(self._session, src.data_ptr(), B, Ls, mem.data_ptr(), self._stream()))
        return mem

    def decode_tgt(self, tgt: torch.Tensor, memory: torch.Tensor, memory_pad_mask: torch.Tensor,
                   memory_row: torch.Tensor | None = None) -> torch.Tensor:
        tgt = self._tokens(tgt)
        R, Lt = tgt.shape
        memory = memory.to(self.device, torch.float32).contiguous()
        Rm, Ls, _ = memory.shape
        pad = memory_pad_mask.to(self.device, torch.uint8).contiguous()
        row_ptr = None
        if memory_row is not None:
            memory_row = memory_row.to(self.device, torch.int32).contiguous()
            row_ptr = memory_row.data_ptr()
        logits = torch.empty((R, Lt, self.tgt_vocab_size), dtype=torch.float32, device=self.device)
# ... 263 lines not shown
```

Baseline: 23080.

## Spread speculative accept across many blocks with wave-per-slot kernel and chunk pool admission

After: 23970, median of 6. +3.9%, better.

```diff
diff --git a/include/ttx.h b/include/ttx.h
--- a/include/ttx.h
+++ b/include/ttx.h
@@ -259,6 +259,8 @@
 } ttx_debug_accept_args;
 
 int ttx_debug_accept(ttx_session* s, const ttx_debug_accept_args* a, int64_t* state, void* stream);
+
+int ttx_debug_accept_block(ttx_session* s, int32_t* words, int n_words, void* stream);
 
 int ttx_debug_kvcopy(ttx_session* s, const int32_t* d_rec, int n_copy, const float* d_qkv, int64_t qkv_layer_stride, float* d_kcache,
                      float* d_vcache, int64_t cache_layer_stride, int64_t cache_seq_stride, int N, int D, int d, int B, int Ld,
diff --git a/translation-transformer_amd/_native.py b/translation-transformer_amd/_native.py
--- a/translation-transformer_amd/_native.py
+++ b/translation-transformer_amd/_native.py
@@ -94,6 +94,7 @@
                                          "pad", "bos", "eos", "greedy", "threads")]
 
 
+DEBUG_ACCEPT_BLOCK_WORDS = 264
 DEBUG_ACCEPT_STATE_WORDS = 17
 
 
@@ -165,6 +166,7 @@
     "ttx_debug_argmax": (C.c_int, [_VP, _VP, _I, _VP, _VP, _I, _VP]),
     "ttx_debug_embed": (C.c_int, [_VP, _VP, _I, _VP, _I, _I, _VP, _VP, _I, _I, _VP, _VP, _VP, _I, _VP, _I, _I, _I, _I, _I, _VP]),
     "ttx_debug_accept": (C.c_int, [_VP, C.POINTER(DebugAcceptArgs), C.POINTER(C.c_int64), _VP]),
+    "ttx_debug_accept_block": (C.c_int, [_VP, C.POINTER(C.c_int32), _I, _VP]),
     "ttx_debug_kvcopy": (C.c_int, [_VP, _VP, _I, _VP, C.c_int64, _VP, _VP, C.c_int64, C.c_int64, _I, _I, _I, _I, _I, _VP]),
     "ttx_debug_kvcopy_split": (C.c_int, [_VP, _VP, _I, _VP, C.c_int64, _VP, _VP, C.c_int64, C.c_int64, _I, _I, _I, _I, _I, _VP, _VP,
                                          C.c_int64, _VP]),
diff --git a/translation-transformer_amd/csrc/ttx_api.hip b/translation-transformer_amd/csrc/ttx_api.hip
--- a/translation-transformer_amd/csrc/ttx_api.hip
+++ b/translation-transformer_amd/csrc/ttx_api.hip
@@ -307,6 +307,7 @@
   if (const char* e = getenv("TTX_FFN2_SLAB_ROWS")) s->ffn2_slab_rows = std::max(0, atoi(e));
   if (const char* e = getenv("TTX_QKV_SMALL_ROWS")) s->qkv_small_rows = std::max(0, atoi(e));
   if (const char* e = getenv("TTX_ATTN_FALLBACK")) s->attn_fallback = atoi(e) != 0;
+  if (const char* e = getenv("TTX_ACCEPT_SPREAD")) s->accept_spread = atoi(e) != 0;
   if (const char* e = getenv("TTX_ATTN_ROW")) s->attn_row = atoi(e) != 0 ? 1 : 0;
   s->host_timing = getenv("TTX_HOST_TIMING") != nullptr;
   m->n_sessions++;
@@ -998,10 +999,35 @@
   KvCopyArgs kc;
 };
 
+static int launch_accept(hipStream_t st, const LoopArgs& la, int threads) {
+  if (la.blk) {
+    hipLaunchKernelGGL(k_accept_slots, dim3(cdiv(la.B, ACCEPT_SLOT_WAVES)), dim3(ACCEPT_SLOT_WAVES * 64), 0, st, la);
+    HIP_TRY(hipGetLastError());
+    hipLaunchKernelGGL(k_accept_finish, dim3(1), dim3(ACCEPT_THREADS), 0, st, la);
+  } else {
+    hipLaunchKernelGGL(k_accept, dim3(1), dim3(threads ? threads : (la.B > 256 ? ACCEPT_THREADS : 256)), 0, st, la);
+  }
+  HIP_TRY(hipGetLastError());
+  return TTX_OK;
+}
+
+static int accept_blk_for(ttx_session* s, hipStream_t st, int B, AcceptBlk** out) {
+  *out = nullptr;
+  if (!s->accept_spread || B <= 256) return TTX_OK;
+  const void* before = s->accept_blk.p;
+  TTX_TRY(ensure(s->accept_blk, sizeof(AcceptBlk), st));
+  if (s->accept_blk.p != before) HIP_TRY(hipMemsetAsync(s->accept_blk.p, 0, sizeof(AcceptBlk), st));
+  *out = s->accept_blk.as<AcceptBlk>();
+  return TTX_OK;
+}
+
 static int launch_accept_and_commit(ttx_session* s, hipStream_t st, const GenCtx& g, bool greedy) {
-  if (greedy) hipLaunchKernelGGL(k_greedy_accept, dim3(1), dim3(256), 0, st, g.la);
-  else hipLaunchKernelGGL(k_accept, dim3(1), dim3(g.k.B > 256 ? ACCEPT_THREADS : 256), 0, st, g.la);
-  HIP_TRY(hipGetLastError());
+  if (greedy) {
+    hipLaunchKernelGGL(k_greedy_accept, dim3(1), dim3(256), 0, st, g.la);
+    HIP_TRY(hipGetLastError());
+  } else {
+    TTX_TRY(launch_accept(st, g.la, 0));
+  }
   hipLaunchKernelGGL(k_kvcopy, dim3(g.k.B, s->m->cfg.num_decoder_layers), dim3(256), 0, st, g.kc);
   HIP_TRY(hipGetLastError());
   return TTX_OK;
@@ -1144,6 +1170,8 @@
   TTX_TRY(ensure_acts(s, st, Macts, 1));
   TTX_TRY(ensure(s->qkv, std::max((size_t)Ld * Mmax, (size_t)B * Ls) * 3 * d * 4, st));
   TTX_TRY(ensure(s->slab, sizeof(float) * 16 * Macts * d, st));
+  AcceptBlk* blk = nullptr;
+  if (!greedy) TTX_TRY(accept_blk_for(s, st, B, &blk));
   s->graphs_current();
 
   s->ev_used = 0;
@@ -1167,6 +1195,7 @@
   g.la.eos = p->eos_token;
   g.la.row_rule = row_rule ? 1 : 0; g.la.traj = row_rule ? s->traj.as<short>() : nullptr; g.la.traj_ld = max_len + 1;
   g.la.fin_step = row_rule ? s->fin_step.as<int>() : nullptr;
+  g.la.blk = blk;
   g.kc.st = s->state.as<DecState>(); g.kc.rec = s->rec.as<CopyRec>(); g.kc.qkv = s->qkv.as<float>();
   g.kc.qkv_layer_stride = (long long)Mmax * 3 * d;
   g.kc.kcache = s->kcache.as<float>(); g.kc.vcache = s->vcache.as<float>();
@@ -1344,6 +1373,29 @@
   return generate_common(s, d_src, B, Ls, p, d_out, stats, stream, true);
 }
 
+constexpr long long ADMIT_ROWS = 16384;
+static int chunk_width(const int32_t* len, int first, int end) {
+  int w = 2;
+  for (int r = first; r < end; ++r) w = std::max(w, (int)len[r]);
+  return w;
+}
+static void admit_chunks(const int32_t* len, int n, long long budget, std::vector<int>& ends) {
+  ends.clear();
+  if (budget > 0 && (long long)n * chunk_width(len, 0, n) >= budget) {
+    int first = 0, w = 2;
+    for (int r = 0; r < n; ++r) {
+      w = std::max(w, (int)len[r]);
+      if ((long long)(r + 1 - first) * w >= budget) { ends.push_back(r + 1); first = r + 1; w = 2; }
+    }
+    if (first < n) {
+      const bool merge = !ends.empty() && (long long)(n - first) * chunk_width(len, first, n) * 2 < budget;
+      if (merge) ends.back() = n; else ends.push_back(n);
+    }
+  } else {
+    ends.push_back(n);
+  }
+}
+
 struct PoolJob {
   ttx_session* s = nullptr;
   hipStream_t st = nullptr;
@@ -1356,6 +1408,7 @@
   PoolIo io{};
   Progress progress;
   long long admitted_rows = 0, src_tokens_padded = 0;
+  long long admit_rows = 0;
   bool two_phase = true;
   long long min_rows = 800;
   GenCtx g2{};
@@ -1408,6 +1461,8 @@
   j.two_phase = true; j.min_rows = 800; j.probes = 0; j.probe_pending = false;
   j.slot_steps = j.matched_slot_steps = j.split_steps = j.skipped_draft_passes = 0;
   j.drafts_matched = j.rows_executed = j.unsplit_rows = 0;
+  j.admit_rows = ADMIT_ROWS;
+  if (const char* e = getenv("TTX_ADMIT_ROWS")) j.admit_rows = std::max(0, atoi(e));
   if (const char* e = getenv("TTX_TWO_PHASE")) j.two_phase = atoi(e) != 0;
   if (const char* e = getenv("TTX_TWO_PHASE_MIN_ROWS")) j.min_rows = std::max(0, atoi(e));
   j.draft_select = j.two_phase && d == c.num_heads * ATT_DH && c.num_heads % 4 == 0 && !s->attn_fallback && N <= 32 && D >= 1;
@@ -1422,6 +1477,8 @@
     TTX_TRY(ensure(s->pred_draft, Mmax * 4, st));
     TTX_TRY(ensure(s->state2, 3 * sizeof(DecState), st));
   }
+  AcceptBlk* blk = nullptr;
+  TTX_TRY(accept_blk_for(s, st, C, &blk));
   s->graphs_current();
 
   s->ev_used = 0;
@@ -1443,6 +1500,7 @@
   g.la.eos = p->eos_token;
   g.la.row_rule = 1; g.la.traj = nullptr; g.la.traj_ld = max_len + 1; g.la.fin_step = nullptr;
   g.la.pool = 1; g.la.rstep = s->rstep.as<int>(); g.la.row_of = s->row_of.as<int>(); g.la.io = s->pool_io.as<PoolIo>();
+  g.la.blk = blk;
   g.k.src_len = s->src_len.as<int>();
   g.kc.st = s->state.as<DecState>(); g.kc.rec = s->rec.as<CopyRec>(); g.kc.qkv = s->qkv.as<float>();
   g.kc.qkv_layer_stride = (long long)Mmax * 3 * d;
@@ -1602,6 +1660,7 @@
   const int n_jobs = std::min(n_sessions, cdiv(R_total, std::max(1, std::min(capacity / 2, 32))));
   const int C = std::min(capacity, std::max(1, cdiv(R_total, n_jobs)));
   std::vector<PoolJob> jobs(n_jobs);
+  std::vector<int> chunk_ends;
   int rc_final = TTX_OK;
   std::fill(std::begin(sessions[0]->pool_counters), std::end(sessions[0]->pool_counters), 0LL);
   for (int i = 0; i < n_jobs && rc_final == TTX_OK; ++i) {
@@ -1660,9 +1719,14 @@
           int share = std::max(1, cdiv(remaining, std::max(1, serial ? 1 : n_running)));
           if (!serial && j.launched == 0 && (long long)n_jobs * C >= R_total) share = std::max(1, cdiv(remaining, n_jobs - i));
           const int take = std::min({free_slots, remaining, share});
-          int Ls_new = 2;
-          for (int r = cursor; r < cursor + take; ++r) Ls_new = std::max(Ls_new, (int)h_len[r]);
-          rc_final = pool_admit(j, d_src + (size_t)cursor * Ls_all, Ls_all, take, Ls_new, cursor, d_out, d_traj, d_fin_step);
+          admit_chunks(h_len + cursor, take, j.admit_rows, chunk_ends);
+          int r0 = cursor;
+          for (const int end : chunk_ends) {
+            const int r1 = cursor + end;
+            rc_final = pool_admit(j, d_src + (size_t)r0 * Ls_all, Ls_all, r1 - r0, chunk_width(h_len, r0, r1), r0, d_out, d_traj, d_fin_step);
+            if (rc_final != TTX_OK) break;
+            r0 = r1;
+          }
           if (rc_final != TTX_OK) break;
           cursor += take;
           n_act += take;
@@ -3086,9 +3150,11 @@
     la.row_rule = a->row_rule ? 1 : 0; la.traj = a->d_traj; la.traj_ld = a->traj_ld; la.fin_step = a->d_fin_step;
     la.pool = a->pool ? 1 : 0; la.rstep = a->d_rstep; la.row_of = a->d_row_of; la.io = dio;
     la.B = a->B; la.N = a->N; la.D = a->D; la.Ls = a->Ls; la.max_len = a->max_len; la.pad = a->pad; la.bos = a->bos; la.eos = a->eos;
-    if (greedy) hipLaunchKernelGGL(k_greedy_accept, dim3(1), dim3(256), 0, st, la);
-    else hipLaunchKernelGGL(k_accept, dim3(1), dim3(a->threads ? a->threads : (a->B > 256 ? ACCEPT_THREADS : 256)), 0, st, la);
-    err = hipGetLastError();
+    int rc_blk = TTX_OK;
+    if (!greedy && a->threads == 0) rc_blk = accept_blk_for(s, st, a->B, &la.blk);
+    if (rc_blk != TTX_OK) err = hipErrorOutOfMemory;
+    else if (greedy) { hipLaunchKernelGGL(k_greedy_accept, dim3(1), dim3(256), 0, st, la); err = hipGetLastError(); }
+    else if (launch_accept(st, la, a->threads) != TTX_OK) err = hipErrorLaunchFailure;
   }
   if (err == hipSuccess) err = hipMemcpyAsync(hs, dst, sizeof(DecState), hipMemcpyDeviceToHost, st);
   const hipError_t esync = hipStreamSynchronize(st);
@@ -3104,6 +3170,17 @@
   if (hinfo) (void)hipHostFree(hinfo);
   HIP_TRY(err);
   HIP_TRY(esync);
+  return TTX_OK;
+}
+
+extern "C" int ttx_debug_accept_block(ttx_session* s, int32_t* words, int n_words, void* stream) {
+  hipStream_t st = reinterpret_cast<hipStream_t>(stream);
+  if (!s || !words || n_words < 0 || (size_t)n_words * 4 > sizeof(AcceptBlk))
+    return fail(TTX_ERR_INVALID, "ttx_debug_accept_block: words must hold at most the block's int32 words");
+  if (!s->accept_blk.p) return fail(TTX_ERR_INVALID, "ttx_debug_accept_block: this session has not run the accept pair yet");
+  HIP_TRY(hipSetDevice(s->m->device));
+  HIP_TRY(hipStreamSynchronize(st));
+  HIP_TRY(hipMemcpy(words, s->accept_blk.p, (size_t)n_words * 4, hipMemcpyDeviceToHost));
   return TTX_OK;
 }
 
diff --git a/translation-transformer_amd/csrc/ttx_internal.h b/translation-transformer_amd/csrc/ttx_internal.h
--- a/translation-transformer_amd/csrc/ttx_internal.h
+++ b/translation-transformer_amd/csrc/ttx_internal.h
@@ -86,6 +86,8 @@
   X(qkv_probe) X(pred_probe) X(pred_draft) X(act2) X(pos2) X(state2)                                                             \
          \
   X(draft_mask) X(row_base) X(row_map)                                                                                           \
+                           \
+  X(accept_blk)                                                                                                                  \
                                         \
   X(snap_logits) X(snap_act) X(snap_front) X(snap_gen) X(snap_state)                                                             \
   X(leaf_score) X(leaf_tok) X(leaf_cnt) X(beam_summary)                                                                          \
@@ -134,6 +136,7 @@
   int last_gemm_kernel = 0, last_gemm_big_min_tiles = 0;
   int attn_split = -1;
   int attn_row = -1;
+  bool accept_spread = true;
   bool attn_fallback = false;
   int attn_force = 0;
   int attn_sel_N = 0, attn_sel_D = 0;
diff --git a/translation-transformer_amd/csrc/ttx_loop_kernels.hip.h b/translation-transformer_amd/csrc/ttx_loop_kernels.hip.h
--- a/translation-transformer_amd/csrc/ttx_loop_kernels.hip.h
+++ b/translation-transformer_amd/csrc/ttx_loop_kernels.hip.h
@@ -123,8 +123,16 @@
   int pool; int* rstep; int* row_of; const struct PoolIo* io;
   int B, N, D, Ls, max_len, pad, bos, eos;
   const int* exec_rows;
+  struct AcceptBlk* blk;
 };
 struct PoolIo { int64_t* out; short* traj; int* fin_step; int traj_ld; int pad_; };
+
+struct AcceptBlk { int maxfront, nfin, pad_[2]; unsigned long long acc, prefix; int finlist[256]; };
+
+__device__ __forceinline__ void accept_blk_clear(AcceptBlk* k, int t) {
+  if (t < 256) k->finlist[t] = 0;
+  if (t == 0) { k->maxfront = 0; k->nfin = 0; k->pad_[0] = k->pad_[1] = 0; k->acc = 0; k->prefix = 0; }
+}
 
 __global__ void k_loop_init(LoopArgs a) {
   const int tid = blockIdx.x * blockDim.x + threadIdx.x;
@@ -137,6 +145,7 @@
   }
   if (a.row_rule)
     for (int i = tid; i < a.B * a.traj_ld; i += gridDim.x * blockDim.x) a.traj[i] = (i % a.traj_ld == 0) ? 0 : -1;
+  if (a.blk && blockIdx.x == 0) accept_blk_clear(a.blk, threadIdx.x);
   if (tid == 0) {
     DecState s;
     s.n_active = a.B; s.r_rows = a.B * a.N; s.m_rows = a.B * step_rps(a.N, a.D);
@@ -152,69 +161,66 @@
   }
 }
 
+struct SlotStep { int b, f, bacc; bool fin; };
+__device__ __forceinline__ void accept_slot_commit(const LoopArgs& a, const DecState* st, int slot, int b, int f, int best, int bacc,
+                                                   bool fin, bool sawpad) {
+  const int D1 = a.D + 1;
+  if (sawpad) a.haspad[b] = 1;
+  a.front[b] = f + bacc + 1;
+  int flags = fin ? 1 : 0;
+  if (a.row_rule) {
+    int it = st->steps + 1;
+    short* trow = a.traj + (size_t)b * a.traj_ld;
+    int* finp = a.fin_step + b;
+    if (a.pool) {
+      it = a.rstep[b] + 1;
+      a.rstep[b] = it;
+      trow = a.io->traj + (size_t)a.row_of[b] * a.traj_ld;
+      finp = a.io->fin_step + a.row_of[b];
+    }
+    if (it < a.traj_ld) trow[it] = (short)(f + bacc + 1);
+    if (fin) *finp = it;
+    else if (f + D1 + 1 >= a.max_len) flags = 2;
+  }
+  a.rec[slot] = CopyRec{b, best, bacc, f, flags};
+}
+
+__device__ __forceinline__ SlotStep accept_slot(const LoopArgs& a, const DecState* st, int slot) {
+  const int RPS = step_rps(a.N, a.D);
+  const int b = a.act_idx[slot];
+  const int f = a.front[b];
+  const int* ps = a.pred + (size_t)slot * RPS;
+  int best = 0, bacc = -1;
+  for (int n = 0; n < a.N; ++n) {
+    const int* dr = a.drafts + ((size_t)b * a.N + n) * a.D;
+    const int* pr = ps + 1 + n * a.D - 1;
+    int acc = a.D;
+    for (int j = a.D - 1; j >= 0; --j)
+      if (dr[j] != (j == 0 ? ps[0] : pr[j])) acc = j;
+    if (acc > bacc) { bacc = acc; best = n; }
+  }
+  const int* pr = ps + 1 + best * a.D - 1;
+  int* g = a.gen + (size_t)b * a.gen_ld;
+  bool fin = false, sawpad = false;
+  for (int j = 0; j <= bacc; ++j) {
+    const int t = (j == 0) ? ps[0] : pr[j];
+    g[f + 1 + j] = t;
+    fin |= (t == a.eos);
+    sawpad |= (t == a.pad);
+  }
+  accept_slot_commit(a, st, slot, b, f, best, bacc, fin, sawpad);
+  return SlotStep{b, f, bacc, fin};
+}
+
 constexpr int ACCEPT_THREADS = 1024;
-__global__ __launch_bounds__(ACCEPT_THREADS) void k_accept(LoopArgs a) {
-  __shared__ int s_maxfront, s_anyfin, s_suspect, s_nn, s_maxf_new, s_nfin;
-  __shared__ int s_finlist[256];
-  __shared__ long long s_acc, s_prefix;
-  __shared__ int s_scan[ACCEPT_THREADS];
-  DecState* st = a.st;
-  const int Bc = st->n_active;
-  if (Bc == 0) return;
+__device__ __forceinline__ void accept_finish(const LoopArgs& a, DecState* st, int Bc, int maxfront, int nfin, const int* finlist,
+                                              long long acc, long long prefix) {
+  __shared__ int s_suspect, s_maxf_new;
+  __shared__ int s_scan[ACCEPT_THREADS / 64];
   const int D1 = a.D + 1, RPS = step_rps(a.N, a.D);
-  if (threadIdx.x == 0) { s_maxfront = 0; s_anyfin = 0; s_acc = 0; s_prefix = 0; s_suspect = 0; s_nn = 0; s_maxf_new = 0; s_nfin = 0; }
-  __syncthreads();
-  for (int slot = threadIdx.x; slot < Bc; slot += blockDim.x) {
-    const int b = a.act_idx[slot];
-    const int f = a.front[b];
-    const int* ps = a.pred + (size_t)slot * RPS;
-    int best = 0, bacc = -1;
-    for (int n = 0; n < a.N; ++n) {
-      const int* dr = a.drafts + ((size_t)b * a.N + n) * a.D;
-      const int* pr = ps + 1 + n * a.D - 1;
-      int acc = a.D;
-      for (int j = a.D - 1; j >= 0; --j)
-        if (dr[j] != (j == 0 ? ps[0] : pr[j])) acc = j;
-      if (acc > bacc) { bacc = acc; best = n; }
-    }
-    const int* pr = ps + 1 + best * a.D - 1;
-    int* g = a.gen + (size_t)b * a.gen_ld;
-    bool fin = false, sawpad = false;
-    for (int j = 0; j <= bacc; ++j) {
-      const int t = (j == 0) ? ps[0] : pr[j];
-      g[f + 1 + j] = t;
-      fin |= (t == a.eos);
-      sawpad |= (t == a.pad);
-    }
-    if (sawpad) a.haspad[b] = 1;
-    a.front[b] = f + bacc + 1;
-    int flags = fin ? 1 : 0;
-    if (a.row_rule) {
-      int it = st->steps + 1;
-      short* trow = a.traj + (size_t)b * a.traj_ld;
-      int* finp = a.fin_step + b;
-      if (a.pool) {
-        it = a.rstep[b] + 1;
-        a.rstep[b] = it;
-        trow = a.io->traj + (size_t)a.row_of[b] * a.traj_ld;
-        finp = a.io->fin_step + a.row_of[b];
-      }
-      if (it < a.traj_ld) trow[it] = (short)(f + bacc + 1);
-      if (fin) *finp = it;
-      else if (f + D1 + 1 >= a.max_len) flags = 2;
-    }
-    a.rec[slot] = CopyRec{b, best, bacc, f, flags};
-    atomicMax(&s_maxfront, f);
-    atomicAdd((unsigned long long*)&s_acc, (unsigned long long)bacc);
-    atomicAdd((unsigned long long*)&s_prefix, (unsigned long long)f);
-    if (fin) {
-      s_anyfin = 1;
-      const int k = atomicAdd(&s_nfin, 1);
-      if (k < 256) s_finlist[k] = b;
-    }
-  }
-  __syncthreads();
-  const int width = s_maxfront + 1 + D1;
+  if (threadIdx.x == 0) { s_suspect = 0; s_maxf_new = 0; }
+  __syncthreads();
+  const int width = maxfront + 1 + D1;
   const int wcopy = width < a.max_len ? width : a.max_len;
   int nn_before = 0;
   for (int base = 0; base < Bc; base += blockDim.x) {
@@ -245,8 +251,8 @@
     int64_t* orow = a.pool ? a.io->out + (size_t)a.row_of[b] * a.max_len : a.out + (size_t)b * a.max_len;
     for (int c = first; c < wout; c += stride) orow[c] = g[c];
   };
-  if (s_nfin <= 256) {
-    for (int k = threadIdx.x >> 6; k < s_nfin; k += (int)(blockDim.x >> 6)) copy_row(s_finlist[k], threadIdx.x & 63, 64);
+  if (nfin <= 256) {
+    for (int k = threadIdx.x >> 6; k < nfin; k += (int)(blockDim.x >> 6)) copy_row(finlist[k], threadIdx.x & 63, 64);
   } else {
     for (int slot = 0; slot < Bc; ++slot)
       if (a.rec[slot].flags == 1) copy_row(a.rec[slot].b, threadIdx.x, blockDim.x);
@@ -256,13 +262,13 @@
     const int nn = nn_before;
     st->n_copy = Bc;
     st->steps += 1;
-    st->accepted += s_acc;
-    st->produced += s_acc + Bc;
+    st->accepted += acc;
+    st->produced += acc + Bc;
     st->verified_positions += a.exec_rows ? (long long)*a.exec_rows : (long long)Bc * RPS;
-    st->kv_prefix_positions += s_prefix;
+    st->kv_prefix_positions += prefix;
     st->src_positions += (long long)Bc * a.Ls;
     st->width = width;
-    if (s_anyfin && width > a.max_len && !a.row_rule) st->error = 1;
+    if (nfin > 0 && width > a.max_len && !a.row_rule) st->error = 1;
     int stop = (nn == 0 || (!a.row_rule && width >= a.max_len)) ? 1 : 0;
     if (a.row_rule && s_suspect) st->error = 3;
     if (!stop && s_suspect && !a.row_rule) {
@@ -288,9 +294,106 @@
   }
 }
 
+__global__ __launch_bounds__(ACCEPT_THREADS) void k_accept(LoopArgs a) {
+  __shared__ int s_maxfront, s_nfin;
+  __shared__ int s_finlist[256];
+  __shared__ long long s_acc, s_prefix;
+  DecState* st = a.st;
+  const int Bc = st->n_active;
+  if (Bc == 0) return;
+  if (threadIdx.x == 0) { s_maxfront = 0; s_acc = 0; s_prefix = 0; s_nfin = 0; }
+  __syncthreads();
+  for (int slot = threadIdx.x; slot < Bc; slot += blockDim.x) {
+    const SlotStep r = accept_slot(a, st, slot);
+    atomicMax(&s_maxfront, r.f);
+    atomicAdd((unsigned long long*)&s_acc, (unsigned long long)r.bacc);
+    atomicAdd((unsigned long long*)&s_prefix, (unsigned long long)r.f);
+    if (r.fin) {
+      const int k = atomicAdd(&s_nfin, 1);
+      if (k < 256) s_finlist[k] = r.b;
+    }
+  }
+  __syncthreads();
+  accept_finish(a, st, Bc, s_maxfront, s_nfin, s_finlist, s_acc, s_prefix);
+}
+
+__device__ __forceinline__ SlotStep accept_slot_wave(const LoopArgs& a, const DecState* st, int slot, int lane) {
+  const int RPS = step_rps(a.N, a.D), ND = a.N * a.D;
+  const int b = a.act_idx[slot];
+  const int f = a.front[b];
+  const int* ps = a.pred + (size_t)slot * RPS;
+  const int* dr = a.drafts + (size_t)b * ND;
+  int best = 0, bacc = -1, open_acc = a.D;
+  for (int base = 0; base < ND; base += 64) {
+    const int e = base + lane;
+    bool miss = false;
+    if (e < ND) miss = dr[e] != ps[(e % a.D == 0) ? 0 : e];
+    const unsigned long long m = __ballot(miss);
+    for (int n = base / a.D; n < a.N && n * a.D < base + 64; ++n) {
+      const int start = n * a.D, end = start + a.D;
+      const int lo = max(start, base) - base, hi = min(end, base + 64) - base;
+      const unsigned long long bits = (m >> lo) & (hi - lo == 64 ? ~0ull : (1ull << (hi - lo)) - 1ull);
+      if (start >= base) open_acc = a.D;
+      if (bits && open_acc == a.D) open_acc = base + lo - start + (int)__ffsll((long long)bits) - 1;
+      if (end <= base + 64 && open_acc > bacc) { bacc = open_acc; best = n; }
+    }
+  }
+  int* g = a.gen + (size_t)b * a.gen_ld;
+  bool fin = false, sawpad = false;
+  for (int j0 = 0; j0 <= bacc; j0 += 64) {
+    const int j = j0 + lane;
+    int t = -1;
+    if (j <= bacc) { t = ps[j == 0 ? 0 : best * a.D + j]; g[f + 1 + j] = t; }
+    fin |= __ballot(j <= bacc && t == a.eos) != 0;
+    sawpad |= __ballot(j <= bacc && t == a.pad) != 0;
+  }
+  if (lane == 0) accept_slot_commit(a, st, slot, b, f, best, bacc, fin, sawpad);
+  return SlotStep{b, f, bacc, fin};
+}
+
+constexpr int ACCEPT_SLOT_WAVES = 4;
+__global__ __launch_bounds__(ACCEPT_SLOT_WAVES * 64) void k_accept_slots(LoopArgs a) {
+  __shared__ int s_maxfront;
+  __shared__ unsigned long long s_acc, s_prefix;
+  const DecState* st = a.st;
+  const int Bc = st->n_active;
+  if ((int)blockIdx.x * ACCEPT_SLOT_WAVES >= Bc) return;
+  if (threadIdx.x == 0) { s_maxfront = 0; s_acc = 0; s_prefix = 0; }
+  __syncthreads();
+  const int slot = blockIdx.x * ACCEPT_SLOT_WAVES + (threadIdx.x >> 6), lane = threadIdx.x & 63;
+  if (slot < Bc) {
+    const SlotStep r = accept_slot_wave(a, st, slot, lane);
+    if (lane == 0) {
+      atomicMax(&s_maxfront, r.f);
+      atomicAdd(&s_acc, (unsigned long long)r.bacc);
+      atomicAdd(&s_prefix, (unsigned long long)r.f);
+      if (r.fin) {
+        const int k = atomicAdd(&a.blk->nfin, 1);
+        if (k < 256) a.blk->finlist[k] = r.b;
+      }
+    }
+  }
+  __syncthreads();
+  if (threadIdx.x == 0) {
+    atomicMax(&a.blk->maxfront, s_maxfront);
+    atomicAdd(&a.blk->acc, s_acc);
+    atomicAdd(&a.blk->prefix, s_prefix);
+  }
+}
+
+__global__ __launch_bounds__(ACCEPT_THREADS) void k_accept_finish(LoopArgs a) {
+  DecState* st = a.st;
+  const int Bc = st->n_active;
+  if (Bc == 0) return;
+  AcceptBlk* k = a.blk;
+  accept_finish(a, st, Bc, k->maxfront, k->nfin, k->finlist, (long long)k->acc, (long long)k->prefix);
+  accept_blk_clear(k, threadIdx.x);
+}
+
 __global__ void k_pool_init(LoopArgs a) {
   const int tid = blockIdx.x * blockDim.x + threadIdx.x;
   for (int i = tid; i < a.B; i += gridDim.x * blockDim.x) { a.act_idx[i] = 0; a.front[i] = 0; a.haspad[i] = 0; a.rstep[i] = 0; a.row_of[i] = 0; }
+  if (a.blk && blockIdx.x == 0) accept_blk_clear(a.blk, threadIdx.x);
   if (tid == 0) {
     DecState s;
     s.n_active = 0; s.r_rows = 0; s.m_rows = 0; s.width = 1; s.steps = 0; s.error = 0; s.n_copy = 0; s.stop = 0;
diff --git a/translation-transformer_amd/model.py b/translation-transformer_amd/model.py
--- a/translation-transformer_amd/model.py
+++ b/translation-transformer_amd/model.py
@@ -264,6 +264,11 @@
         a.greedy, a.threads = int(greedy), int(threads)
         words = (C.c_int64 * N.DEBUG_ACCEPT_STATE_WORDS)(*[int(v) for v in state], *([0] * (N.DEBUG_ACCEPT_STATE_WORDS - len(state))))
         N.check(self._lib.ttx_debug_accept(self._session, C.byref(a), words, self._stream()))
+        return [int(v) for v in words]
+
+    def debug_accept_block(self) -> list:
+        words = (C.c_int32 * N.DEBUG_ACCEPT_BLOCK_WORDS)()
+        N.check(self._lib.ttx_debug_accept_block(self._session, words, N.DEBUG_ACCEPT_BLOCK_WORDS, self._stream()))
         return [int(v) for v in words]
 
     def debug_kvcopy(self, rec: torch.Tensor, n_copy: int, qkv: torch.Tensor, kcache: torch.Tensor, vcache: torch.Tensor,
```
